# zwyang6/ExCEL

Hardware: AMD Instinct MI355X
Metric: images/sec (CAM+PAR refine, 448x448) (higher is better)
Workload: dtype bf16x3 (fp32 as bf16 hi+lo, fp32 accumulate)

## Files before the change

### excel_amd/_lib.py

```python
import ctypes as C
import os

_HERE = os.path.dirname(os.path.abspath(__file__))
LIB_PATH = os.path.join(_HERE, "csrc", "libexcel_hip.so")

c_f = C.c_void_p
c_i = C.c_int
c_ll = C.c_longlong
c_sz = C.c_size_t


class VitConfig(C.Structure):
    _fields_ = [("width", c_i), ("layers", c_i), ("heads", c_i), ("patch", c_i), ("out_dim", c_i),
                ("n_surgery", c_i), ("pos_grid", c_i)]


class VitBlockWeights(C.Structure):
    _fields_ = [(n, C.c_void_p) for n in (
        "ln1_w", "ln1_b", "in_proj_w", "in_proj_b", "out_proj_w", "out_proj_b",
        "ln2_w", "ln2_b", "fc1_w", "fc1_b", "fc2_w", "fc2_b")]


class VitWeights(C.Structure):
    _fields_ = [(n, C.c_void_p) for n in (
        "conv1_w", "class_emb", "pos_emb", "ln_pre_w", "ln_pre_b", "ln_post_w", "ln_post_b", "proj")] + \
        [("blocks", C.POINTER(VitBlockWeights))]


class DecoderConfig(C.Structure):
    _fields_ = [(n, c_i) for n in ("vit_layers", "vit_width", "embed", "dec_layers", "heads", "num_classes")]


class FuseLayerWeights(C.Structure):
    _fields_ = [(n, C.c_void_p) for n in ("proj_w", "proj_b", "proj2_w", "proj2_b")]


class DecoderBlockWeights(C.Structure):
    _fields_ = VitBlockWeights._fields_


class DecoderWeights(C.Structure):
    _fields_ = [("fuse", C.POINTER(FuseLayerWeights)), ("fuse_w", C.c_void_p), ("fuse_b", C.c_void_p),
                ("blocks", C.POINTER(DecoderBlockWeights)), ("pred_w", C.c_void_p), ("pred_b", C.c_void_p)]


class TextConfig(C.Structure):
    _fields_ = [(n, c_i) for n in ("vocab_size", "context_length", "width", "layers", "heads", "embed_dim")]


class TextWeights(C.Structure):
    _fields_ = [(n, C.c_void_p) for n in ("token_embedding", "positional_embedding", "ln_final_w", "ln_final_b", "text_projection")] + \
        [("blocks", C.POINTER(DecoderBlockWeights))]


class RaggedInfo(C.Structure):
    _fields_ = [("B", C.c_int32), ("total_tiles", C.c_int32), ("total_pix", C.c_int64), ("total_label_pix", C.c_int64),
                ("max_plane_pix", C.c_int64), ("table_ints", C.c_int64)]


class AugParams(C.Structure):
    _fields_ = [("ratio", C.c_double), ("flip", C.c_int32), ("h_pad", C.c_int32), ("w_pad", C.c_int32),
                ("cand_h", C.c_int32 * 10), ("cand_w", C.c_int32 * 10)]


class TrainAugInfo(C.Structure):
    _fields_ = [("B", C.c_int32), ("S", C.c_int32), ("max_h", C.c_int32), ("max_w2", C.c_int32), ("table_ints", C.c_int64),
                ("workspace_bytes", C.c_int64), ("total_label_pix", C.c_int64)]


SIGNATURES = {
    "excel_last_error": (C.c_char_p, []),
    "excel_abi_version": (c_i, []),
    "excel_build_id": (C.c_char_p, []),
    "excel_gemm_f32": (c_i, [c_f, c_f, c_f, c_f, c_f, c_i, c_i, c_i, c_i, c_i, c_i, c_i, c_i, c_i, c_i,
                             c_ll, c_ll, c_ll, c_ll, c_f]),
    "excel_split_bf16": (c_i, [c_f, c_f, c_ll, c_i, c_f]),
    "excel_gemm_bf16x3": (c_i, [c_f, c_f, c_f, c_f, c_f, c_i, c_i, c_i, c_i, c_i, c_f]),
    "excel_split_f16": (c_i, [c_f, c_f, c_ll, c_i, c_f]),
    "excel_gemm_f16x3": (c_i, [c_f, c_f, c_f, c_f, c_f, c_i, c_i, c_i, c_i, c_i, c_f]),
    "excel_pack_f16": (c_i, [c_f, c_f, c_ll, c_i, c_f, c_f]),
    "excel_gemm_f16x2": (c_i, [c_f, c_f, c_f, c_f, c_f, c_f, c_i, c_i, c_i, c_i, c_i, c_f]),
    "excel_gemm_plan": (c_i, [c_i, c_i, c_i, c_i, c_i, c_i, c_i, c_i, c_i, C.POINTER(C.c_int32)]),
    "excel_attn_plan": (c_i, [c_i, c_i, c_i, c_i, c_i, c_i, C.POINTER(C.c_int32)]),
    "excel_layernorm": (c_i, [c_f, c_f, c_f, c_f, c_i, c_i, C.c_float, c_f]),
    "excel_vit_create": (c_i, [C.POINTER(VitConfig), C.POINTER(VitWeights), C.POINTER(C.c_void_p)]),
    "excel_vit_destroy": (None, [C.c_void_p]),
    "excel_vit_workspace_bytes": (c_sz, [C.c_void_p, c_i, c_i]),
    "excel_vit_set_gemm_mode": (c_i, [C.c_void_p, c_i]),
    "excel_vit_get_gemm_mode": (c_i, [C.c_void_p]),
    "excel_vit_weights_fp16_exact": (c_i, [C.c_void_p]),
    "excel_vit_forward": (c_i, [C.c_void_p, c_f, c_i, c_i, c_f, c_sz, c_f, c_f, c_f, c_i, c_f, c_i, c_f, c_f]),
    "excel_vit_forward_ex": (c_i, [C.c_void_p, c_f, c_i, c_i, c_f, c_sz, c_f, c_f, c_f, c_i, c_f, c_i, c_f, c_f, c_i, c_f]),
    "excel_feature_affinity_workspace_bytes": (c_sz, [c_i, c_i, c_i]),
    "excel_feature_affinity": (c_i, [c_f, c_i, c_i, c_i, C.c_float, C.c_float, c_i, c_f, c_f, c_f]),
    "excel_feature_affinity_grouped_workspace_bytes": (c_sz, [c_i, c_i, c_i, c_i]),
    "excel_feature_affinity_grouped": (c_i, [c_f, c_i, c_i, c_i, c_i, c_i, C.c_float, C.c_float, c_i, c_f, c_f, c_f]),
    "excel_attn_select_workspace_bytes": (c_sz, [c_i, c_i]),
    "excel_attn_select_mean": (c_i, [c_f, c_i, c_i, c_i, c_i, c_i, c_f, c_f, c_f, c_f]),
    "excel_decoder_create": (c_i, [C.POINTER(DecoderConfig), C.POINTER(DecoderWeights), C.POINTER(C.c_void_p)]),
    "excel_decoder_destroy": (None, [C.c_void_p]),
    "excel_decoder_workspace_bytes": (c_sz, [C.c_void_p, c_i, c_i]),
    "excel_decoder_forward": (c_i, [C.c_void_p, c_f, c_i, c_i, c_f, c_sz, c_f, c_f, c_f]),
    "excel_text_create": (c_i, [C.POINTER(TextConfig), C.POINTER(TextWeights), C.POINTER(C.c_void_p)]),
    "excel_text_destroy": (None, [C.c_void_p]),
    "excel_text_workspace_bytes": (c_sz, [C.c_void_p, c_i]),
    "excel_text_encode": (c_i, [C.c_void_p, c_f, c_i, c_f, c_f, c_sz, c_f]),
    "excel_prompt_ensemble": (c_i, [c_f, c_i, c_i, c_f, c_f]),
    "excel_decoder_train_workspace_bytes": (c_sz, [C.c_void_p, c_i, c_i]),
    "excel_decoder_forward_train": (c_i, [C.c_void_p, c_f, c_i, c_i, c_f, c_sz, c_f, c_f, C.c_float, C.c_uint, c_f]),
    "excel_decoder_train_attn_fts": (c_i, [C.c_void_p, c_i, c_i, c_f, c_sz, c_f, c_f]),
    "excel_decoder_backward": (c_i, [C.c_void_p, c_f, c_i, c_i, c_f, c_sz, c_f, c_f, C.POINTER(DecoderWeights), C.c_float, C.c_uint, c_f]),
    "excel_adamw_step": (c_i, [c_f, c_f, c_f, c_f, c_ll, C.c_float, C.c_float, C.c_float, C.c_float, C.c_float, c_i, c_f]),
    "excel_train_losses_workspace_bytes": (c_sz, [c_i, c_i, c_i, c_i]),
    "excel_train_losses": (c_i, [c_f, c_f, c_f, c_f, c_i, c_i, c_i, c_i, c_i, c_i, c_i, c_i, C.c_float, C.c_float, c_f, c_f, c_f, c_f, c_f]),
    "excel_lam_to_label": (c_i, [c_f, c_f, c_f, c_i, c_i, c_i, c_i, C.c_float, C.c_float, C.c_float, c_i, c_i, c_f, c_f, c_f]),
    "excel_normalize_img_u8": (c_i, [c_f, c_i, c_i, c_i, C.POINTER(C.c_double), C.POINTER(C.c_double), c_f, c_f]),
    "excel_denormalize_img": (c_i, [c_f, c_i, c_i, c_i, C.POINTER(C.c_float), C.POINTER(C.c_float), c_f, c_f, c_f]),
    "excel_seg_scale_accumulate": (c_i, [c_f, c_f, c_i, c_i, c_i, c_i, c_i, c_i, c_i, c_i, C.c_float, c_f]),
    "excel_cam_workspace_bytes": (c_sz, [c_i, c_i, c_i]),
    "excel_patch_text_cam_workspace_bytes": (c_sz, [c_i, c_i, c_i, c_i]),
    "excel_patch_text_cam": (c_i, [c_f, c_f, c_i, c_i, c_i, c_i, c_i, C.c_float, c_i, c_f, c_f, c_f, c_f, c_f]),
    "excel_clip_feature_surgery": (c_i, [c_f, c_f, c_i, c_i, c_i, c_i, c_i, C.c_float, c_f, c_f, c_f, c_f]),
    "excel_dcrf_workspace_bytes": (c_sz, [c_i, c_i, c_i]),
    "excel_dcrf_inference": (c_i, [c_f, c_f, c_i, c_i, c_i, c_i, c_i, C.c_float, C.c_float, C.c_float, C.c_float, C.c_float, c_f, c_f, c_f]),
    "excel_dcrf_ragged_workspace_bytes": (c_i, [c_ll, c_i, C.POINTER(c_sz)]),
    "excel_dcrf_inference_ragged": (c_i, [c_f, c_f, c_i, c_f, C.POINTER(RaggedInfo), c_i, c_i, C.c_float, C.c_float, C.c_float, C.c_float, C.c_float,
                                          c_f, c_f, c_f, c_f]),
    "excel_dcrf_lam_ragged_workspace_bytes": (c_i, [C.POINTER(C.c_int32), C.POINTER(C.c_int32), c_i, C.POINTER(c_sz)]),
    "excel_dcrf_lam_ragged": (c_i, [c_f, c_f, c_f, C.POINTER(C.c_int32), c_f, c_f, C.POINTER(RaggedInfo), c_i, c_i, c_i, C.c_float, C.c_float,
                                    C.c_float, C.c_float, C.c_float, c_f, c_f, c_f, c_f]),
    "excel_attn_layer_mean": (c_i, [c_f, c_i, c_i, c_i, c_i, c_i, c_f, c_f]),
    "excel_trans_mat_workspace_bytes": (c_sz, [c_i, c_i]),
    "excel_compute_trans_mat": (c_i, [c_f, c_i, c_i, c_f, c_f, c_f]),
    "excel_cls_compact": (c_i, [c_f, c_i, c_i, c_i, c_f, c_f, c_f, c_f]),
    "excel_scoremap_box_mask": (c_i, [c_f, c_f, c_f, c_i, c_i, c_i, c_i, C.c_double, c_f, c_f, c_f]),
    "excel_refine_workspace_bytes": (c_sz, [c_i, c_i, c_i]),
    "excel_refine_cams_with_aff": (c_i, [c_f, c_f, c_f, c_f, c_i, c_i, c_i, c_i, C.c_double, c_f, c_f, c_f]),
    "excel_cam_upsample_bkg": (c_i, [c_f, c_f, c_i, c_i, c_i, c_i, c_i, c_f, c_f, c_i, c_f]),
    "excel_par_workspace_bytes": (c_sz, [c_i, c_i, c_i, c_i, c_i]),
    "excel_par_forward": (c_i, [c_f, c_i, c_i, c_f, c_f, c_i, c_i, c_i, c_i, C.POINTER(C.c_int32), c_i, c_i,
                                C.c_float, C.c_float, c_f, c_f, c_i, c_f]),
    "excel_ragged_plan": (c_i, [C.POINTER(C.c_int32), c_i, C.POINTER(RaggedInfo), C.POINTER(C.c_int32)]),
    "excel_normalize_resize_u8_ragged": (c_i, [c_f, c_f, c_i, c_i, C.POINTER(C.c_double), C.POINTER(C.c_double), c_f, c_f]),
    "excel_normalize_resize_u8_ragged_mirror": (c_i, [c_f, c_f, c_i, c_i, C.POINTER(C.c_double), C.POINTER(C.c_double), c_f, c_f]),
    "excel_cam_upsample_bkg_ragged": (c_i, [c_f, c_f, c_f, C.POINTER(RaggedInfo), c_i, c_i, c_f, c_f, c_i, c_f]),
    "excel_par_ragged_workspace_bytes": (c_sz, [c_ll, c_i]),
    "excel_par_forward_ragged": (c_i, [c_f, c_i, c_i, c_f, c_f, c_f, C.POINTER(RaggedInfo), c_i, C.POINTER(C.c_int32), c_i, c_i,
                                       C.c_float, C.c_float, c_f, c_f, c_f]),
    "excel_argmax_label_ragged": (c_i, [c_f, c_f, c_f, c_f, C.POINTER(RaggedInfo), c_i, c_i, c_f, c_f]),
    "excel_seg_msc_fuse_ragged": (c_i, [C.POINTER(C.c_void_p), C.POINTER(C.c_int32), C.POINTER(C.c_int32), c_i, c_i, c_f, C.POINTER(RaggedInfo),
                                        c_f, c_f, c_f]),
    "excel_seg_resize_argmax_ragged": (c_i, [c_f, c_f, C.POINTER(RaggedInfo), c_f, C.POINTER(RaggedInfo), c_i, c_f, c_f]),
    "excel_seg_resize_argmax_uniform": (c_i, [c_f, c_i, c_i, c_i, c_i, c_f, C.POINTER(RaggedInfo), c_f, c_f]),
    "excel_seg_softmax_resize": (c_i, [c_f, c_i, c_i, c_i, c_i, c_i, c_f, c_f]),
    "excel_seg_softmax_resize_ragged": (c_i, [c_f, c_f, C.POINTER(RaggedInfo), c_f, C.POINTER(RaggedInfo), c_i, c_f, c_f]),
    "excel_cam_overlay_ragged": (c_i, [c_f, c_f, c_i, c_f, c_f, c_f, C.POINTER(RaggedInfo), c_i, c_f, c_f, c_f]),
    "excel_cam_overlay": (c_i, [c_f, c_f, c_i, c_i, c_i, c_i, c_f, c_f, c_f]),
    "excel_train_panels_plan": (c_i, [c_i, c_i, c_i, c_i, c_i, C.POINTER(C.c_int64)]),
    "excel_train_panels": (c_i, [c_f, c_f, c_f, c_f, c_f, c_f, c_f, c_i, c_i, c_i, c_i, c_i, c_i, c_i, C.POINTER(C.c_float), C.POINTER(C.c_float),
                                 c_f, c_f, c_f, c_sz, c_f]),
    "excel_png_labels_bound_bytes": (c_sz, [c_i, c_i]),
    "excel_png_labels_workspace_bytes": (c_sz, [c_i, c_i]),
    "excel_png_encode_labels_ragged": (c_i, [c_f, c_f, C.POINTER(RaggedInfo), C.POINTER(C.c_int32), c_f, c_f, c_sz, c_f, c_f, c_sz, c_f]),
    "excel_train_aug_plan": (c_i, [C.POINTER(C.c_int32), C.POINTER(AugParams), c_i, c_i, C.POINTER(TrainAugInfo), C.POINTER(C.c_int32)]),
    "excel_train_augment_workspace_bytes": (c_sz, [C.POINTER(TrainAugInfo)]),
    "excel_train_augment": (c_i, [c_f, c_f, c_f, C.POINTER(TrainAugInfo), C.POINTER(C.c_double), C.POINTER(C.c_double), c_f, c_f, c_f, c_f, c_f]),
    "excel_train_augment_image": (c_i, [c_f, c_f, C.POINTER(TrainAugInfo), C.POINTER(C.c_double), C.POINTER(C.c_double), c_f, c_f, c_f, c_f]),
    "excel_argmax_label": (c_i, [c_f, c_f, c_f, c_i, c_i, c_i, c_ll, c_f, c_f, c_f]),
    "excel_confusion_accumulate": (c_i, [c_f, c_f, c_ll, c_i, c_f, c_f]),
    "excel_attr_aggregate": (c_i, [c_f, c_f, c_i, c_i, c_i, c_i, C.c_double, c_f, c_f]),
    "excel_bilinear_resize": (c_i, [c_f, c_f, c_ll, c_i, c_i, c_i, c_i, c_i, c_f]),
    "excel_pos_embed_resize": (c_i, [c_f, c_i, c_i, c_i, c_f, c_f]),
    "excel_flip_max_normalize": (c_i, [c_f, c_f, c_i, c_i, c_i, c_f]),
    "excel_lam_scale_accumulate": (c_i, [c_f, c_f, c_i, c_i, c_i, c_i, c_i, c_i, c_f]),
    "excel_plane_minmax_normalize": (c_i, [c_f, c_ll, c_ll, c_f]),
    "excel_prof_enable": (c_i, [c_i]),
    "excel_prof_set_mask": (c_i, [C.c_ulonglong]),
    "excel_prof_set_sampling": (c_i, [c_i]),
    "excel_prof_num_categories": (c_i, []),
    "excel_prof_category_name": (C.c_char_p, [c_i]),
    "excel_prof_collect": (c_i, [C.POINTER(C.c_double), C.POINTER(C.c_longlong), C.POINTER(C.c_double)]),
}

_lib = None


def lib():
    global _lib
    if _lib is not None:
        return _lib
    import torch
    if not os.path.exists(LIB_PATH):
        raise RuntimeError(
            f"excel_amd: {LIB_PATH} is missing - the HIP extension is the only compute path. "
            "Build it with `python -m excel_amd.build` (or __graft_entry__.build()).")
    handle = C.CDLL(LIB_PATH)
    for name, (res, args) in SIGNATURES.items():
        fn = getattr(handle, name)
        fn.restype = res
        fn.argtypes = args
    _lib = handle
    return _lib


def build_id():
    return lib().excel_build_id().decode()


def check(rc, what):
    if rc != 0:
        msg = lib().excel_last_error()
        raise RuntimeError(f"{what} failed (rc={rc}): {msg.decode() if msg else '?'}")
```

### excel_amd/csrc/abi.hip

```cpp
#include "../../include/excel_hip.h"
#include "common.h"
#include "excel_internal.h"

#include <stdarg.h>
#include <map>
#include <vector>

static thread_local char g_err[512] = "";

void excel_set_error(const char* fmt, ...) {
    va_list ap;
    va_start(ap, fmt);
    vsnprintf(g_err, sizeof(g_err), fmt, ap);
    va_end(ap);
}

extern "C" const char* excel_last_error(void) { return g_err; }
extern "C" int excel_abi_version(void) { return 4; }
#ifndef EXCEL_BUILD_ID
#define EXCEL_BUILD_ID "unstamped"
#endif
extern "C" const char* excel_build_id(void) { return EXCEL_BUILD_ID; }

bool g_excel_prof_on = false;
thread_local int g_excel_prof_gemm_cat = -1;
unsigned long long g_excel_prof_mask = ~0ull;
int g_excel_prof_every = 1;
unsigned g_excel_prof_seen[PROF_NCAT];
namespace {
struct ProfRec { int cat; hipEvent_t a, b; };
std::vector<ProfRec> g_prof_recs;
std::vector<hipEvent_t> g_prof_pool;
double g_prof_work[PROF_NCAT];
const char* PROF_NAMES[PROF_NCAT] = {"gemm_nt", "gemm_nn", "gemm_bf16x3", "attn_rowpass", "attn_accum", "layernorm", "embed", "token_norm",
                                     "cam_epilogue", "sinkhorn", "bbox_mask", "matvec", "cam_upsample", "par_affinity",
                                     "par_iterate", "argmax", "confusion", "other", "cam_proj", "cam_fused"};
hipEvent_t prof_event() {
    if (!g_prof_pool.empty()) { hipEvent_t e = g_prof_pool.back(); g_prof_pool.pop_back(); return e; }
    hipEvent_t e; (void)hipEventCreate(&e); return e;
}
}
void excel_prof_begin(int cat, hipStream_t st, double work) {
    ProfRec r{cat, prof_event(), prof_event()};
    (void)hipEventRecord(r.a, st);
    g_prof_recs.push_back(r);
    g_prof_work[cat] += work;
}
void excel_prof_end(int cat, hipStream_t st) {
    for (size_t i = g_prof_recs.size(); i-- > 0;)
        if (g_prof_recs[i].cat == cat) { (void)hipEventRecord(g_prof_recs[i].b, st); return; }
}
extern "C" int excel_prof_enable(int on) {
    g_excel_prof_on = on != 0;
    return EXCEL_OK;
}
extern "C" int excel_prof_set_mask(unsigned long long mask) {
    g_excel_prof_mask = mask;
    return EXCEL_OK;
}
extern "C" int excel_prof_set_sampling(int every) {
    g_excel_prof_every = every > 0 ? every : 1;
    for (int c = 0; c < PROF_NCAT; ++c) g_excel_prof_seen[c] = 0;
    return EXCEL_OK;
}
extern "C" int excel_prof_num_categories(void) { return PROF_NCAT; }
extern "C" const char* excel_prof_category_name(int cat) { return (cat >= 0 && cat < PROF_NCAT) ? PROF_NAMES[cat] : ""; }
extern "C" int excel_prof_collect(double* ms, long long* launches, double* work) {
    for (int c = 0; c < PROF_NCAT; ++c) { ms[c] = 0.0; launches[c] = 0; work[c] = g_prof_work[c]; g_prof_work[c] = 0.0; }
    for (auto& r : g_prof_recs) {
        float t = 0.f;
        if (hipEventSynchronize(r.b) == hipSuccess && hipEventElapsedTime(&t, r.a, r.b) == hipSuccess) {
            ms[r.cat] += t;
            launches[r.cat] += 1;
        }
        g_prof_pool.push_back(r.a);
        g_prof_pool.push_back(r.b);
    }
    g_prof_recs.clear();
    return EXCEL_OK;
}

#define ST(s) ((hipStream_t)(s))
#define TRY(x)                  \
    do {                        \
        int rc__ = (x);         \
        if (rc__) return rc__;  \
    } while (0)

static inline size_t align_up(size_t v, size_t a) { return (v + a - 1) / a * a; }

static GemmArgs gemm_args(const float* A, const float* B, float* C, const float* bias, const float* res, int M, int N, int K,
                          int lda, int ldb, int ldc, int ldr, int act) {
    GemmArgs g;
    memset(&g, 0, sizeof(g));
    g.A = A; g.B = B; g.C = C; g.bias = bias; g.res = res;
    g.M = M; g.N = N; g.K = K; g.Kld = (K + 3) / 4 * 4;
    g.lda = lda; g.ldb = ldb; g.ldc = ldc; g.ldr = ldr;
    g.act = act; g.out_mode = GEMM_OUT_PLAIN; g.alpha = 1.f; g.zdiv = 1;
    return g;
}

static GemmBfArgs gemm_bf_args(const void* A, const unsigned short* W, float* C, void* Cs, const float* bias, const float* res,
                               int M, int N, int K, int ldc, int ldr, int act, int out_mode) {
    GemmBfArgs g;
    memset(&g, 0, sizeof(g));
    g.A = (const unsigned short*)A; g.B = W; g.C = C; g.Cs = (unsigned short*)Cs; g.bias = bias; g.res = res;
    g.M = M; g.N = N; g.K = K; g.lda = 2 * K; g.ldb = 2 * K; g.ldc = ldc; g.ldr = ldr; g.act = act; g.out_mode = out_mode;
    return g;
}

__global__ void transpose_kernel(const float* __restrict__ in, float* __restrict__ out, int R, int Cc) {
    __shared__ float t[32][33];
    const int tx = threadIdx.x & 31, ty = threadIdx.x >> 5;
    const int r0 = blockIdx.y * 32, c0 = blockIdx.x * 32;
    for (int k = ty; k < 32; k += 8)
        if (r0 + k < R && c0 + tx < Cc) t[k][tx] = in[(long long)(r0 + k) * Cc + c0 + tx];
    __syncthreads();
    for (int k = ty; k < 32; k += 8)
        if (c0 + k < Cc && r0 + tx < R) out[(long long)(c0 + k) * R + r0 + tx] = t[tx][k];
}

__global__ void pos_resize_kernel(const float* __restrict__ pos, float* __restrict__ out, int side, int g, int D) {
    const long long i = (long long)blockIdx.x * 256 + threadIdx.x;
    const long long total = (long long)(g * g + 1) * D;
    if (i >= total) return;
    const int d = (int)(i % D);
    const int n = (int)(i / D);
    if (n == 0) { out[i] = pos[d]; return; }
    const int y = (n - 1) / g, x = (n - 1) % g;
    const float sc = (float)side / (float)g;
    float fy = fmaxf(sc * ((float)y + 0.5f) - 0.5f, 0.f), fx = fmaxf(sc * ((float)x + 0.5f) - 0.5f, 0.f);
    const int y0 = min((int)fy, side - 1), x0 = min((int)fx, side - 1);
    const int y1 = min(y0 + 1, side - 1), x1 = min(x0 + 1, side - 1);
    const float ly = fy - (float)y0, lx = fx - (float)x0;
    auto at = [&](int yy, int xx) { return pos[(long long)(1 + yy * side + xx) * D + d]; };
    out[i] = (1.f - ly) * ((1.f - lx) * at(y0, x0) + lx * at(y0, x1)) + ly * ((1.f - lx) * at(y1, x0) + lx * at(y1, x1));
}

__global__ void attn_layer_mean_kernel(const float* __restrict__ attn, int B, int N, int first, int nl, float* __restrict__ out) {
    const long long P = N - 1;
    const long long i = (long long)blockIdx.x * 256 + threadIdx.x;
    if (i >= (long long)B * P * P) return;
    const int c = (int)(i % P), r = (int)((i / P) % P);
    const long long b = i / (P * P);
    float s = 0.f;
    for (int l = 0; l < nl; ++l) s += attn[(((long long)(first + l) * B + b) * N + (r + 1)) * N + (c + 1)];
    out[i] = s / (float)nl;
}

extern "C" int excel_gemm_f32(const float* A, const float* Bm, float* C, const float* bias, const float* residual, int M, int N,
                              int K, int lda, int ldb, int ldc, int ldr, int b_kmajor, int act, int batch, long long sA,
                              long long sB, long long sC, long long sR, void* stream) {
    GemmArgs g = gemm_args(A, Bm, C, bias, residual, M, N, K, lda, ldb, ldc, ldr, act);
    EXCEL_CHECK_ARG((K % 4) == 0 || !b_kmajor, "excel_gemm_f32: K must be a multiple of 4 in NT mode (K=%d)", K);
    if (!b_kmajor) {
        EXCEL_CHECK_ARG((K % 4) == 0, "excel_gemm_f32: K must be a multiple of 4 (pad A with zeros) (K=%d)", K);
    }
    g.sA = sA; g.sB = sB; g.sC = sC; g.sR = sR;
    return excel_launch_gemm(g, b_kmajor != 0, batch, ST(stream));
}

extern "C" int excel_split_bf16(const float* in, void* out, long long rows, int K, void* stream) {
    EXCEL_CHECK_ARG(in && out && rows > 0 && K > 0, "split_bf16: bad argument");
    return excel_launch_split_bf16(in, out, rows, K, ST(stream));
}

extern "C" int excel_gemm_bf16x3(const void* A_split, const void* W_split, float* C, const float* bias, const float* residual,
                                 int M, int N, int K, int act, int split_out, void* stream) {
    EXCEL_CHECK_ARG(A_split && W_split && C, "gemm_bf16x3: null argument");
    GemmBfArgs g = gemm_bf_args(A_split, (const unsigned short*)W_split, C, C, bias, residual, M, N, K, N, N, act,
                                split_out ? GEMM_OUT_SPLIT_BF16 : GEMM_OUT_PLAIN);
// ... 337 lines not shown
    return excel_launch_feature_affinity(feats, B, C, P, beta, gamma, mode, out, workspace, ST(stream));
}

extern "C" size_t excel_feature_affinity_grouped_workspace_bytes(int B, int C, int P, int group) {
    return excel_feature_affinity_grouped_ws_bytes(B, C, P, group);
}

extern "C" int excel_feature_affinity_grouped(const float* feats, int B, int C, int P, int group, int member_stride, float beta, float gamma,
                                              int mode, float* out, void* workspace, void* stream) {
    return excel_launch_feature_affinity_grouped(feats, B, C, P, group, member_stride, beta, gamma, mode, out, workspace, ST(stream));
}

extern "C" size_t excel_attn_select_workspace_bytes(int B, int n_layers) { return excel_attn_select_ws_bytes(B, n_layers); }

extern "C" int excel_attn_select_mean(const float* attn, int Lw, int B, int N, int first_layer, int n_layers, const float* seg_attn,
                                      float* w_out, void* workspace, void* stream) {
    return excel_launch_attn_select_mean(attn, Lw, B, N, first_layer, n_layers, seg_attn, w_out, workspace, ST(stream));
}

#define EXCEL_VIT_FWD_ARGS excel_vit_t h, const float* img, int B, int S, void* workspace, size_t workspace_bytes, float* image_features, \
    float* x_raw, float* w_aff, int aff_layers, float* attn_out, int n_attn_out, float* feats_out, const float* ex_attn, int flags, void* stream
static int vit_forward_bf16(EXCEL_VIT_FWD_ARGS) {
#include "vit_forward_body.inc"
}
static int vit_forward_f16(EXCEL_VIT_FWD_ARGS) {
    using excel_f16::excel_launch_gemm; using excel_f16::excel_launch_gemm_bf16x3; using excel_f16::excel_launch_split_bf16;
    using excel_f16::excel_launch_vt_from_planes; using excel_f16::excel_launch_layernorm; using excel_f16::excel_launch_assemble_ln_pre;
    using excel_f16::excel_launch_token_axis_normalize; using excel_f16::excel_launch_im2col; using excel_f16::excel_launch_attn_rowpass;
    using excel_f16::excel_launch_attn_accum; using excel_f16::excel_launch_attn_strip;
#include "vit_forward_body.inc"
}
static int vit_forward_impl(EXCEL_VIT_FWD_ARGS) {
    EXCEL_CHECK_ARG(h, "excel_vit_forward: null handle");
    return h->gemm_mode >= 2 ? vit_forward_f16(h, img, B, S, workspace, workspace_bytes, image_features, x_raw, w_aff, aff_layers, attn_out,
                                               n_attn_out, feats_out, ex_attn, flags, stream)
                             : vit_forward_bf16(h, img, B, S, workspace, workspace_bytes, image_features, x_raw, w_aff, aff_layers, attn_out,
                                                n_attn_out, feats_out, ex_attn, flags, stream);
}

extern "C" size_t excel_cam_workspace_bytes(int B, int N, int T) {
    return align_up((size_t)B * N * ((T + 3) / 4 * 4) * sizeof(float), 256);
}

extern "C" int excel_clip_feature_surgery(const float* image_features, const float* text, int B, int N, int C, int T, int F,
                                          float temperature, float* out_full, float* out_slice, void* workspace, void* stream) {
    EXCEL_CHECK_ARG(image_features && text && workspace && (out_full || out_slice), "clip_feature_surgery: null argument");
    EXCEL_CHECK_ARG((C % 4) == 0, "clip_feature_surgery: C must be a multiple of 4");
    const int ldT = (T + 3) / 4 * 4;
    float* S = (float*)workspace;
    GemmArgs ga = gemm_args(image_features, text, S, nullptr, nullptr, B * N, T, C, C, C, ldT, 0, GEMM_ACT_NONE);
    TRY(excel_launch_gemm(ga, true, 1, ST(stream)));
    return excel_launch_cam_epilogue(S, out_full, out_slice, B, N, T, ldT, F, temperature, ST(stream));
}

struct PtcWs { float *sim, *part, *colsq; unsigned short* ts; size_t total; };
static PtcWs ptc_ws_layout(int B, int N, int C, int T, char* base) {
    PtcWs w;
    size_t off = 0;
    auto take = [&](size_t bytes) { char* p = base + off; off += align_up(bytes, 256); return p; };
    w.sim = (float*)take(excel_patch_text_cam_ws_floats(B, N, C, T, 0) * sizeof(float));
    w.ts = (unsigned short*)take((size_t)T * C * sizeof(float));
    w.part = (float*)take(excel_patch_text_cam_ws_floats(B, N, C, T, 1) * sizeof(float));
    w.colsq = (float*)take(excel_patch_text_cam_ws_floats(B, N, C, T, 2) * sizeof(float));
    w.total = off;
    return w;
}
extern "C" size_t excel_patch_text_cam_workspace_bytes(int B, int N, int C, int T) { return ptc_ws_layout(B, N, C, T, nullptr).total; }

extern "C" int excel_patch_text_cam(const float* x_raw, const float* text, int B, int N, int C, int T, int F, float temperature, int mode,
                                    float* out_full, float* out_slice, float* image_features, void* workspace, void* stream) {
    EXCEL_CHECK_ARG(x_raw && text && workspace && (out_full || out_slice), "patch_text_cam: null argument");
    EXCEL_CHECK_ARG(mode == 0 || mode == 1 || mode == 2, "patch_text_cam: mode must be 0 (exact fp32), 1 (bf16x3) or 2 (f16x3)");
    EXCEL_CHECK_ARG(B > 0 && N > 0 && C > 0 && T > 0, "patch_text_cam: bad shape");
    const int ldT = (T + 3) / 4 * 4;
    const PtcWs w = ptc_ws_layout(B, N, C, T, (char*)workspace);
    if (mode == 2)
        return excel_f16::excel_launch_patch_text_cam(x_raw, text, w.ts, w.sim, w.part, w.colsq, out_full, out_slice, image_features, B, N, C, T, F,
                                                      ldT, temperature, 1, ST(stream));
    return excel_launch_patch_text_cam(x_raw, text, mode == 1 ? w.ts : nullptr, w.sim, w.part, w.colsq, out_full, out_slice, image_features, B, N, C,
                                       T, F, ldT, temperature, mode, ST(stream));
}

extern "C" int excel_attn_layer_mean(const float* attn, int Lw, int B, int N, int first_layer, int n_layers, float* w_aff, void* stream) {
    EXCEL_CHECK_ARG(attn && w_aff && first_layer >= 0 && n_layers >= 1 && first_layer + n_layers <= Lw, "attn_layer_mean: bad layer range");
    const long long n = (long long)B * (N - 1) * (N - 1);
    hipLaunchKernelGGL(attn_layer_mean_kernel, dim3((unsigned)cdivl(n, 256)), dim3(256), 0, ST(stream), attn, B, N, first_layer, n_layers, w_aff);
    EXCEL_CHECK_LAUNCH("attn_layer_mean");
    return EXCEL_OK;
}

extern "C" size_t excel_trans_mat_workspace_bytes(int B, int P) {
    return 2 * align_up((size_t)B * P * P * sizeof(float), 256) + align_up((size_t)B * P * sizeof(float), 256);
}

extern "C" int excel_compute_trans_mat(const float* w_aff, int B, int P, float* trans_out, void* workspace, void* stream) {
    EXCEL_CHECK_ARG(w_aff && trans_out && workspace, "compute_trans_mat: null argument");
    EXCEL_CHECK_ARG((P % 4) == 0, "compute_trans_mat: P must be a multiple of 4 (P=%d)", P);
    char* base = (char*)workspace;
    const size_t mat = align_up((size_t)B * P * P * sizeof(float), 256);
    float* T = (float*)base;
    float* Tsym = (float*)(base + mat);
    float* cs = (float*)(base + 2 * mat);
    TRY(excel_launch_trans_mat_sym(w_aff, T, Tsym, cs, B, P, ST(stream)));
    GemmArgs ga = gemm_args(Tsym, Tsym, trans_out, nullptr, nullptr, P, P, P, P, P, P, 0, GEMM_ACT_NONE);
    ga.sA = ga.sB = ga.sC = (long long)P * P;
    return excel_launch_gemm(ga, true, B, ST(stream));
}

extern "C" int excel_cls_compact(const float* onehot, int B, int F, int Smax, int32_t* cls_idx, int32_t* ncls, int32_t* nchan,
                                 void* stream) {
    EXCEL_CHECK_ARG(onehot && cls_idx && ncls && Smax >= 1, "cls_compact: bad argument");
    return excel_launch_cls_compact(onehot, B, F, Smax, cls_idx, ncls, nchan, ST(stream));
}

extern "C" int excel_scoremap_box_mask(const float* attr, const int32_t* cls_idx, const int32_t* ncls, int B, int g, int F, int Smax,
                                       double caa_thre, float* v_out, uint8_t* mask_out, void* stream) {
    EXCEL_CHECK_ARG(attr && cls_idx && ncls && v_out, "scoremap_box_mask: null argument");
    return excel_launch_bbox_mask(attr, cls_idx, ncls, B, g, F, Smax, caa_thre, v_out, mask_out, ST(stream));
}

extern "C" size_t excel_refine_workspace_bytes(int B, int P, int Smax) {
    return 2 * align_up((size_t)B * P * P * sizeof(float), 256) + align_up((size_t)B * P * sizeof(float), 256) +
           2 * align_up((size_t)B * Smax * P * sizeof(float), 256);
}

extern "C" int excel_refine_cams_with_aff(const float* attr, const float* w_aff, const int32_t* cls_idx, const int32_t* ncls, int B,
                                          int g, int F, int Smax, double caa_thre, float* refined, void* workspace, void* stream) {
    EXCEL_CHECK_ARG(attr && w_aff && cls_idx && ncls && refined && workspace, "refine_cams_with_aff: null argument");
    const int P = g * g;
    char* base = (char*)workspace;
    const size_t mat = align_up((size_t)B * P * P * sizeof(float), 256);
    const size_t vec = align_up((size_t)B * Smax * P * sizeof(float), 256);
    float* T = (float*)base;
    float* Tsym = (float*)(base + mat);
    float* cs = (float*)(base + 2 * mat);
    float* v = (float*)(base + 2 * mat + align_up((size_t)B * P * sizeof(float), 256));
    float* u = (float*)((char*)v + vec);
    hipStream_t st = ST(stream);
    TRY(excel_launch_trans_mat_sym(w_aff, T, Tsym, cs, B, P, st));
    TRY(excel_launch_bbox_mask(attr, cls_idx, ncls, B, g, F, Smax, caa_thre, v, nullptr, st));
    TRY(excel_launch_matvec(Tsym, v, ncls, u, B, P, Smax, st));
    TRY(excel_launch_matvec(Tsym, u, ncls, refined, B, P, Smax, st));
    return EXCEL_OK;
}

extern "C" int excel_cam_upsample_bkg(const float* refined, const int32_t* ncls, int B, int g, int Smax, int H, int W, float* cams,
                                      void* workspace, int flags, void* stream) {
    EXCEL_CHECK_ARG(refined && ncls && cams && workspace, "cam_upsample_bkg: null argument");
    return excel_launch_cam_upsample_bkg(refined, ncls, (float*)workspace, cams, B, g, Smax, H, W, (flags & EXCEL_CAMS_ZERO_UNUSED) ? 1 : 0, ST(stream));
}

extern "C" int excel_ragged_plan(const int32_t* hw, int B, excel_ragged_info* info, int32_t* table) {
    EXCEL_CHECK_ARG(hw && info && B >= 1, "ragged_plan: bad argument");
    long long pix = 0, lab = 0, tiles = 0, max_plane = 0;
    for (int b = 0; b < B; ++b) {
        const long long H = hw[2 * b], W = hw[2 * b + 1];
        EXCEL_CHECK_ARG(H >= 1 && W >= 1, "ragged_plan: image %d has size %lld x %lld", b, H, W);
        const long long Wp = (W + 3) / 4 * 4, plane = H * Wp, nt = ((W + 63) / 64) * ((H + 15) / 16);
        if (table) {
            int32_t* rec = table + EXCEL_RAG_REC * b;
            rec[0] = (int32_t)H; rec[1] = (int32_t)W; rec[2] = (int32_t)pix; rec[3] = (int32_t)tiles; rec[4] = (int32_t)lab; rec[5] = rec[6] = rec[7] = 0;
            for (long long t = 0; t < nt; ++t) table[EXCEL_RAG_REC * (B + 1) + tiles + t] = b;
        }
        pix += plane; lab += H * W; tiles += nt;
        if (plane > max_plane) max_plane = plane;
        EXCEL_CHECK_ARG(pix < (1LL << 31) && 3 * lab < (1LL << 31) && tiles < (1LL << 31), "ragged_plan: batch too large for 32-bit offsets");
    }
    if (table) {
        int32_t* rec = table + EXCEL_RAG_REC * B;
        rec[0] = rec[1] = 0; rec[2] = (int32_t)pix; rec[3] = (int32_t)tiles; rec[4] = (int32_t)lab; rec[5] = rec[6] = rec[7] = 0;
    }
    info->B = B; info->total_tiles = (int32_t)tiles; info->total_pix = pix; info->total_label_pix = lab; info->max_plane_pix = max_plane;
    info->table_ints = EXCEL_RAG_REC * (long long)(B + 1) + tiles;
    return EXCEL_OK;
}

static TileGeo ragged_geo(const int32_t* table, int B) {
    TileGeo g;
    g.tab = table; g.B = B; g.H = g.W = 0;
    return g;
}
static TileGeo uniform_geo(int B, int H, int W) {
    TileGeo g;
    g.tab = nullptr; g.B = B; g.H = H; g.W = W;
    return g;
}

extern "C" int excel_normalize_resize_u8_ragged(const uint8_t* hwc, const int32_t* table, int B, int S, const double* mean3, const double* std3,
                                                float* out, void* stream) {
    EXCEL_CHECK_ARG(hwc && table && out && mean3 && std3 && B > 0 && S > 0, "normalize_resize_u8_ragged: bad argument");
    return excel_launch_normalize_resize_u8_ragged(hwc, out, ragged_geo(table, B), S, mean3, std3, ST(stream));
}

extern "C" int excel_normalize_resize_u8_ragged_mirror(const uint8_t* hwc, const int32_t* table, int B, int S, const double* mean3,
                                                       const double* std3, float* out, void* stream) {
    EXCEL_CHECK_ARG(hwc && table && out && mean3 && std3 && B > 0 && S > 0, "normalize_resize_u8_ragged_mirror: bad argument");
    return excel_launch_normalize_resize_u8_ragged_mirror(hwc, out, ragged_geo(table, B), S, mean3, std3, ST(stream));
}

extern "C" int excel_cam_upsample_bkg_ragged(const float* refined, const int32_t* ncls, const int32_t* table, const excel_ragged_info* info, int g,
                                             int Smax, float* cams, void* workspace, int flags, void* stream) {
    EXCEL_CHECK_ARG(refined && ncls && table && info && cams && workspace, "cam_upsample_bkg_ragged: null argument");
    EXCEL_CHECK_ARG((((uintptr_t)cams) & 15) == 0, "cam_upsample_bkg_ragged: cams must be 16-byte aligned");
    return excel_launch_cam_upsample_bkg_ragged(refined, ncls, (float*)workspace, cams, g, Smax, ragged_geo(table, info->B), info->total_tiles,
                                                (flags & EXCEL_CAMS_ZERO_UNUSED) ? 1 : 0, ST(stream));
}

int excel_aug_plan(const int32_t* hw, const excel_aug_params* prm, int B, int S, excel_train_aug_info* info, int32_t* table);
int excel_launch_train_augment(const unsigned char* hwc, const unsigned char* labels, const int* table, const excel_train_aug_info& info,
                               const double* mean, const double* stdv, float* img, unsigned char* label, int* img_box, void* workspace,
                               hipStream_t st);
int excel_launch_train_augment_image(const unsigned char* hwc, const int* table, const excel_train_aug_info& info, const double* mean,
                                     const double* stdv, float* img, int* img_box, void* workspace, hipStream_t st);
extern "C" int excel_train_aug_plan(const int32_t* hw, const excel_aug_params* params, int B, int S, excel_train_aug_info* info, int32_t* table) {
    return excel_aug_plan(hw, params, B, S, info, table);
}

extern "C" size_t excel_train_augment_workspace_bytes(const excel_train_aug_info* info) {
    return info ? (size_t)info->workspace_bytes : 0;
}

extern "C" int excel_train_augment(const uint8_t* hwc, const uint8_t* labels, const int32_t* table, const excel_train_aug_info* info,
                                   const double* mean3, const double* std3, float* img, uint8_t* label, int32_t* img_box, void* workspace,
                                   void* stream) {
    EXCEL_CHECK_ARG(hwc && labels && table && info && mean3 && std3 && img && label && img_box && workspace, "train_augment: null argument");
    EXCEL_CHECK_ARG(info->B >= 1 && info->S >= 1 && info->max_h >= 1 && info->max_w2 >= 1 && info->workspace_bytes > 0,
                    "train_augment: info was not filled by excel_train_aug_plan");
    return excel_launch_train_augment(hwc, labels, table, *info, mean3, std3, img, label, img_box, workspace, ST(stream));
}

extern "C" int excel_train_augment_image(const uint8_t* hwc, const int32_t* table, const excel_train_aug_info* info, const double* mean3,
                                         const double* std3, float* img, int32_t* img_box, void* workspace, void* stream) {
    EXCEL_CHECK_ARG(hwc && table && info && mean3 && std3 && img && img_box && workspace, "train_augment_image: null argument");
    EXCEL_CHECK_ARG(info->B >= 1 && info->S >= 1 && info->max_h >= 1 && info->max_w2 >= 1 && info->workspace_bytes > 0,
                    "train_augment_image: info was not filled by excel_train_aug_plan");
    return excel_launch_train_augment_image(hwc, table, *info, mean3, std3, img, img_box, workspace, ST(stream));
}

extern "C" size_t excel_par_workspace_bytes(int B, int Cmax, int H, int W, int ndil) {
    const size_t hw = (size_t)H * W;
    return align_up((size_t)B * 8 * ndil * hw * sizeof(float), 256) + align_up((size_t)B * Cmax * hw * sizeof(float), 256) +
           align_up((size_t)B * 3 * hw * sizeof(float), 256);
}

template <class Step>
static int par_jacobi(const float* masks, float* out, float* pp, int n_iter, Step step) {
    const float* cur = masks;
    for (int it = 0; it < n_iter; ++it) {
        float* dst = (((n_iter - 1 - it) & 1) == 0) ? out : pp;
        TRY(step(cur, dst));
        cur = dst;
    }
    return EXCEL_OK;
}

extern "C" int excel_par_forward(const float* imgs, int h, int w, const float* masks, const int32_t* nchan, int B, int Cmax, int H,
                                 int W, const int32_t* dilations, int ndil, int n_iter, float w1, float w2, float* out,
                                 void* workspace, int flags, void* stream) {
    EXCEL_CHECK_ARG(imgs && masks && out && workspace && dilations, "par_forward: null argument");
    EXCEL_CHECK_ARG(n_iter >= 0 && ndil >= 1 && ndil <= 8, "par_forward: bad n_iter/ndil");
    EXCEL_CHECK_ARG(B > 0 && Cmax > 0 && H > 0 && W > 0 && h > 0 && w > 0, "par_forward: bad shape");
    const size_t hw = (size_t)H * W;
    char* base = (char*)workspace;
    float* aff = (float*)base;
    float* pp = (float*)(base + align_up((size_t)B * 8 * ndil * hw * sizeof(float), 256));
    float* guide = (float*)((char*)pp + align_up((size_t)B * Cmax * hw * sizeof(float), 256));
    hipStream_t st = ST(stream);
    const float* gimg = imgs;
    if (h != H || w != W) {
        TRY(excel_launch_bilinear_ac(imgs, guide, B * 3, h, w, H, W, st));
        gimg = guide;
    }
    const TileGeo geo = uniform_geo(B, H, W);
    const bool recompute = !(flags & EXCEL_PAR_STREAM_AFFINITIES) && n_iter > 0 && (W % 4) == 0 && (((uintptr_t)pp & 15) == 0) &&
                           excel_par_guide_supported(gimg, aff, masks, out, Cmax, (long long)hw, W, dilations, ndil);
    TRY(excel_launch_par_affinity(gimg, aff, geo, 0, dilations, ndil, w1, w2, st, recompute ? 1 : 0));
    if (n_iter == 0) {
        hipMemcpyAsync(out, masks, sizeof(float) * (size_t)B * Cmax * hw, hipMemcpyDeviceToDevice, st);
        return EXCEL_OK;
    }
    if (recompute)
        return par_jacobi(masks, out, pp, n_iter, [&](const float* cur, float* dst) {
            return excel_launch_par_iterate_guide(gimg, aff, cur, dst, nchan, Cmax, geo, 0, dilations, ndil, w1, w2, st);
        });
    return par_jacobi(masks, out, pp, n_iter, [&](const float* cur, float* dst) {
        return excel_launch_par_iterate(aff, cur, dst, nchan, B, Cmax, H, W, dilations, ndil, st);
    });
}

extern "C" size_t excel_par_ragged_workspace_bytes(long long total_pix, int Cmax) {
    return align_up((size_t)5 * total_pix * sizeof(float), 256) + align_up((size_t)Cmax * total_pix * sizeof(float), 256) +
           align_up((size_t)3 * total_pix * sizeof(float), 256);
}

extern "C" int excel_par_forward_ragged(const float* imgs, int h, int w, const float* masks, const int32_t* nchan, const int32_t* table,
                                        const excel_ragged_info* info, int Cmax, const int32_t* dilations, int ndil, int n_iter, float w1,
                                        float w2, float* out, void* workspace, void* stream) {
    EXCEL_CHECK_ARG(imgs && masks && out && workspace && dilations && table && info, "par_forward_ragged: null argument");
    EXCEL_CHECK_ARG(n_iter >= 1 && Cmax > 0 && h > 0 && w > 0 && info->B > 0, "par_forward_ragged: bad n_iter / shape");
    const size_t tp = (size_t)info->total_pix;
    char* base = (char*)workspace;
    float* stats = (float*)base;
    float* pp = (float*)(base + align_up(5 * tp * sizeof(float), 256));
    float* guide = (float*)((char*)pp + align_up((size_t)Cmax * tp * sizeof(float), 256));
    hipStream_t st = ST(stream);
    const TileGeo geo = ragged_geo(table, info->B);
    EXCEL_CHECK_ARG(excel_par_guide_supported(guide, stats, masks, out, Cmax, info->max_plane_pix, 4, dilations, ndil) && (((uintptr_t)pp & 15) == 0),
                    "par_forward_ragged: needs dilations [1,2,4,8,12,24], 16-byte aligned buffers and max(Cmax,5) * H * Wp * 4 < 2^31 per image "
                    "(Wp = W rounded up to 4)");
    TRY(excel_launch_bilinear_ac_ragged(imgs, guide, h, w, geo, info->total_tiles, st));
    TRY(excel_launch_par_affinity(guide, stats, geo, info->total_tiles, dilations, ndil, w1, w2, st, 1));
    return par_jacobi(masks, out, pp, n_iter, [&](const float* cur, float* dst) {
        return excel_launch_par_iterate_guide(guide, stats, cur, dst, nchan, Cmax, geo, info->total_tiles, dilations, ndil, w1, w2, st);
    });
}

extern "C" int excel_argmax_label_ragged(const float* cams, const int32_t* nchan, const int32_t* cls_idx, const int32_t* table,
                                         const excel_ragged_info* info, int Smax, int Cmax, uint8_t* labels_u8, void* stream) {
    EXCEL_CHECK_ARG(cams && table && info && labels_u8, "argmax_label_ragged: null argument");
    return excel_launch_argmax_label_ragged(cams, nchan, cls_idx, Smax, Cmax, ragged_geo(table, info->B), info->total_tiles, labels_u8, ST(stream));
}

extern "C" int excel_argmax_label(const float* cams, const int32_t* nchan, const int32_t* cls_idx, int B, int Smax, int Cmax,
                                  long long HW, uint8_t* labels_u8, int64_t* labels_i64, void* stream) {
    EXCEL_CHECK_ARG(cams && (labels_u8 || labels_i64), "argmax_label: null argument");
    return excel_launch_argmax_label(cams, nchan, cls_idx, B, Smax, Cmax, HW, labels_u8, (long long*)labels_i64, ST(stream));
}

extern "C" int excel_confusion_accumulate(const uint8_t* gt, const uint8_t* pred, long long n, int num_classes, int64_t* hist,
                                          void* stream) {
    EXCEL_CHECK_ARG(gt && pred && hist && n >= 0, "confusion_accumulate: null argument");
    if (n == 0) return EXCEL_OK;
    return excel_launch_confusion(gt, pred, n, num_classes, (unsigned long long*)hist, ST(stream));
}

extern "C" int excel_attr_aggregate(const float* text, const float* bank, int F, int T, int C, int K, double topK, float* out,
                                    void* stream) {
    EXCEL_CHECK_ARG(text && bank && out, "attr_aggregate: null argument");
    const int drop = (int)((1.0 - topK) * (double)K);
    return excel_launch_attr_aggregate(text, bank, F, T, C, K, drop, out, ST(stream));
}

extern "C" int excel_bilinear_resize(const float* in, float* out, long long planes, int h, int w, int H, int W, int align_corners,
                                     void* stream) {
    EXCEL_CHECK_ARG(in && out && planes > 0 && h > 0 && w > 0 && H > 0 && W > 0, "bilinear_resize: bad argument");
    return excel_launch_bilinear_resize(in, out, planes, h, w, H, W, align_corners, ST(stream));
}

extern "C" int excel_pos_embed_resize(const float* pos, int side, int g, int D, float* out, void* stream) {
    EXCEL_CHECK_ARG(pos && out && side > 0 && g > 0, "pos_embed_resize: bad argument");
    hipLaunchKernelGGL(pos_resize_kernel, dim3((unsigned)cdivl((long long)(g * g + 1) * D, 256)), dim3(256), 0, ST(stream), pos, out, side, g, D);
    EXCEL_CHECK_LAUNCH("pos_resize");
    return EXCEL_OK;
}

extern "C" int excel_flip_max_normalize(const float* attr, float* out, int B, int g, int F, void* stream) {
    EXCEL_CHECK_ARG(attr && out, "flip_max_normalize: null argument");
    return excel_launch_flip_max_normalize(attr, out, B, g, F, ST(stream));
}

extern "C" int excel_lam_scale_accumulate(const float* maps, float* acc, int B, int g, int F, int H, int W, int init, void* stream) {
    EXCEL_CHECK_ARG(maps && acc && B > 0 && g > 0, "lam_scale_accumulate: bad argument");
    return excel_launch_lam_scale_accumulate(maps, acc, B, g, F, H, W, init, ST(stream));
}

extern "C" int excel_plane_minmax_normalize(float* lam, long long planes, long long HW, void* stream) {
    EXCEL_CHECK_ARG(lam && planes > 0 && HW > 0, "plane_minmax_normalize: bad argument");
    return excel_launch_plane_minmax_normalize(lam, planes, HW, ST(stream));
}
```

### excel_amd/csrc/common.h

```cpp
#pragma once
#include <hip/hip_runtime.h>
#include <stdint.h>
#include <stdio.h>
#include <string.h>

#define EXCEL_OK 0
#define EXCEL_ERR_ARG (-1)
#define EXCEL_ERR_LAUNCH (-2)
#define EXCEL_ERR_ALLOC (-3)

void excel_set_error(const char* fmt, ...);

#define EXCEL_CHECK_ARG(cond, ...)                         \
    do {                                                   \
        if (!(cond)) {                                     \
            excel_set_error(__VA_ARGS__);                  \
            return EXCEL_ERR_ARG;                          \
        }                                                  \
    } while (0)

#define EXCEL_CHECK_LAUNCH(name)                                                   \
    do {                                                                           \
        hipError_t e__ = hipGetLastError();                                        \
        if (e__ != hipSuccess) {                                                   \
            excel_set_error("%s: launch failed: %s", name, hipGetErrorString(e__)); \
            return EXCEL_ERR_LAUNCH;                                               \
        }                                                                          \
    } while (0)

typedef float f32x4 __attribute__((ext_vector_type(4)));
typedef float f32x16 __attribute__((ext_vector_type(16)));

static inline int cdiv(int a, int b) { return (a + b - 1) / b; }
static inline long long cdivl(long long a, long long b) { return (a + b - 1) / b; }

#define WAVE 64

#ifdef EXCEL_DEV
#define EXCEL_DBG(x) (x)
#else
#define EXCEL_DBG(x) 0
#endif

__device__ __forceinline__ void wave_halves(float x, float& lo, float& hi) {
    const unsigned u = __float_as_uint(x);
    const auto r = __builtin_amdgcn_permlane32_swap(u, u, false, false);
    lo = __uint_as_float(r[0]);
    hi = __uint_as_float(r[1]);
}
__device__ __forceinline__ float wave_sum(float v) {
    float lo, hi;
    wave_halves(v, lo, hi);
    v = lo + hi;
#pragma unroll
    for (int o = 16; o > 0; o >>= 1) v += __shfl_xor(v, o, 64);
    return v;
}
__device__ __forceinline__ float wave_max(float v) {
    float lo, hi;
    wave_halves(v, lo, hi);
    v = fmaxf(lo, hi);
#pragma unroll
    for (int o = 16; o > 0; o >>= 1) v = fmaxf(v, __shfl_xor(v, o, 64));
    return v;
}
__device__ __forceinline__ float wave_min(float v) {
    float lo, hi;
    wave_halves(v, lo, hi);
    v = fminf(lo, hi);
#pragma unroll
    for (int o = 16; o > 0; o >>= 1) v = fminf(v, __shfl_xor(v, o, 64));
    return v;
}

__device__ __forceinline__ int c32_row(int reg, int lane) { return (reg & 3) + 8 * (reg >> 2) + 4 * (lane >> 5); }

__device__ __forceinline__ int xcd_remap(int id, int n) {
    const int q = n >> 3, r = n & 7;
    const int xcd = id & 7, loc = id >> 3;
    const int base = (xcd < r) ? xcd * (q + 1) : r * (q + 1) + (xcd - r) * q;
    return base + loc;
}

#define EXCEL_RAG_REC 8
struct TileGeo {
    const int* tab;
    int B;
    int H, W;
};
struct Tile {
    int b, x0, y0, H, W, Wp;
    long long base;
    long long HW;
    long long lab;
};
__device__ __forceinline__ Tile tile_of_ragged(const TileGeo& g, int tile) {
    Tile t;
    const int* __restrict__ tab = g.tab;
    t.b = tab[EXCEL_RAG_REC * (g.B + 1) + tile];
    const int* rec = tab + EXCEL_RAG_REC * t.b;
    t.H = rec[0]; t.W = rec[1];
    t.Wp = (t.W + 3) & ~3;
    t.base = rec[2];
    t.lab = rec[4];
    const int loc = tile - rec[3];
    const int ntx = (t.W + 63) >> 6;
    const int ty = loc / ntx;
    t.x0 = (loc - ty * ntx) * 64;
    t.y0 = ty * 16;
    t.HW = (long long)t.H * t.Wp;
    return t;
}
template <bool RAGGED>
__device__ __forceinline__ Tile tile_of(const TileGeo& g) {
    Tile t;
    if (RAGGED) {
        t = tile_of_ragged(g, blockIdx.x);
    } else {
        t.b = blockIdx.z; t.x0 = blockIdx.x * 64; t.y0 = blockIdx.y * 16;
        t.H = g.H; t.W = g.W; t.Wp = g.W;
        t.HW = (long long)g.H * g.W;
        t.base = (long long)t.b * t.HW;
        t.lab = t.base;
    }
    return t;
}
__device__ __forceinline__ int ragged_image_of_pixel(const int* __restrict__ tab, int B, long long n) {
    int lo = 0, hi = B - 1;
    while (lo < hi) {
        const int mid = (lo + hi + 1) >> 1;
        if ((long long)tab[EXCEL_RAG_REC * mid + 4] <= n) lo = mid; else hi = mid - 1;
    }
    return lo;
}

enum ExcelProfCat {
    PROF_GEMM_NT = 0, PROF_GEMM_NN, PROF_GEMM_BF16X3, PROF_ATTN_ROWPASS, PROF_ATTN_ACCUM, PROF_LAYERNORM, PROF_EMBED, PROF_TOKEN_NORM,
    PROF_CAM_EPILOGUE, PROF_SINKHORN, PROF_BBOX, PROF_MATVEC, PROF_UPSAMPLE, PROF_PAR_AFFINITY, PROF_PAR_ITERATE,
    PROF_ARGMAX, PROF_CONFUSION, PROF_OTHER, PROF_CAM_PROJ, PROF_CAM_FUSED, PROF_NCAT
};
extern thread_local int g_excel_prof_gemm_cat;
extern bool g_excel_prof_on;
extern unsigned long long g_excel_prof_mask;
extern int g_excel_prof_every;
extern unsigned g_excel_prof_seen[];
void excel_prof_begin(int cat, hipStream_t st, double work);
void excel_prof_end(int cat, hipStream_t st);
struct ProfScope {
    int cat; hipStream_t st; bool on;
    ProfScope(int c, hipStream_t s, double work = 0.0)
        : cat(c), st(s), on(g_excel_prof_on && ((g_excel_prof_mask >> c) & 1) && (g_excel_prof_seen[c]++ % g_excel_prof_every) == 0) { if (on) excel_prof_begin(cat, st, work); }
    ~ProfScope() { if (on) excel_prof_end(cat, st); }
};


#ifdef EXCEL_SPLIT_F16
typedef _Float16 split_t;
#define EXCEL_MFMA16(a, b, c, x, y, z) __builtin_amdgcn_mfma_f32_32x32x16_f16(a, b, c, x, y, z)
#define EXCEL_MFMA32(a, b, c) __builtin_amdgcn_mfma_f32_16x16x32_f16(a, b, c, 0, 0, 0)
#define EXCEL_SPLIT_NAME "f16"
#else
typedef __bf16 split_t;
#define EXCEL_MFMA16(a, b, c, x, y, z) __builtin_amdgcn_mfma_f32_32x32x16_bf16(a, b, c, x, y, z)
#define EXCEL_MFMA32(a, b, c) __builtin_amdgcn_mfma_f32_16x16x32_bf16(a, b, c, 0, 0, 0)
#define EXCEL_SPLIT_NAME "bf16"
#endif
typedef split_t splitx8 __attribute__((ext_vector_type(8)));
typedef split_t splitx4 __attribute__((ext_vector_type(4)));
__device__ __forceinline__ split_t split_hi(float x) { return (split_t)x; }
__device__ __forceinline__ void split_pair(float a, float b, unsigned& hi2, unsigned& lo2) {
#ifdef EXCEL_SPLIT_F16
    typedef float f2_ __attribute__((ext_vector_type(2)));
    typedef _Float16 h2_ __attribute__((ext_vector_type(2)));
    const f2_ v = {a, b};
    const h2_ h = __builtin_convertvector(v, h2_);
    hi2 = __builtin_bit_cast(unsigned, h);
    lo2 = __builtin_bit_cast(unsigned, __builtin_convertvector(v - __builtin_convertvector(h, f2_), h2_));
#else
    typedef float f2_ __attribute__((ext_vector_type(2)));
    typedef __bf16 b2_ __attribute__((ext_vector_type(2)));
    const f2_ v = {a, b};
    hi2 = __builtin_bit_cast(unsigned, __builtin_convertvector(v, b2_));
    const f2_ back = {__uint_as_float(hi2 << 16), __uint_as_float(hi2 & 0xffff0000u)};
    lo2 = __builtin_bit_cast(unsigned, __builtin_convertvector(v - back, b2_));
#endif
}
__device__ __forceinline__ void split_pair_bounded(float a, float b, unsigned& hi2, unsigned& lo2) {
#ifdef EXCEL_SPLIT_F16
    typedef _Float16 h2_ __attribute__((ext_vector_type(2)));
    const float ha = __uint_as_float(__float_as_uint(a) & 0xFFFFE000u), hb = __uint_as_float(__float_as_uint(b) & 0xFFFFE000u);
    hi2 = __builtin_bit_cast(unsigned, __builtin_amdgcn_cvt_pkrtz(ha, hb));
    const h2_ l = {(_Float16)(a - ha), (_Float16)(b - hb)};
    lo2 = __builtin_bit_cast(unsigned, l);
#else
    typedef float f2_ __attribute__((ext_vector_type(2)));
    typedef __bf16 b2_ __attribute__((ext_vector_type(2)));
    const unsigned ua = __float_as_uint(a), ub = __float_as_uint(b);
    hi2 = (ua >> 16) | (ub & 0xFFFF0000u);
    const f2_ d = {a - __uint_as_float(ua & 0xFFFF0000u), b - __uint_as_float(ub & 0xFFFF0000u)};
    lo2 = __builtin_bit_cast(unsigned, __builtin_convertvector(d, b2_));
#endif
}
typedef float f32x2 __attribute__((ext_vector_type(2)));
template <int NV>
__device__ __forceinline__ void quickgelu_tiles(f32x4* v) {
    f32x2 t[2 * NV];
#pragma unroll
    for (int i = 0; i < 2 * NV; ++i) t[i] = f32x2{v[i >> 1][2 * (i & 1)], v[i >> 1][2 * (i & 1) + 1]} * f32x2{-1.702f, -1.702f};
#pragma unroll
    for (int i = 0; i < 2 * NV; ++i) t[i] = t[i] * f32x2{1.4426950408889634f, 1.4426950408889634f};
#pragma unroll
    for (int i = 0; i < 2 * NV; ++i) t[i] = f32x2{__builtin_amdgcn_exp2f(t[i][0]), __builtin_amdgcn_exp2f(t[i][1])};
#pragma unroll
    for (int i = 0; i < 2 * NV; ++i) t[i] = t[i] + f32x2{1.f, 1.f};
#pragma unroll
    for (int i = 0; i < 2 * NV; ++i) t[i] = f32x2{__builtin_amdgcn_rcpf(t[i][0]), __builtin_amdgcn_rcpf(t[i][1])};
#pragma unroll
    for (int i = 0; i < 2 * NV; ++i) {
        const f32x2 o = f32x2{v[i >> 1][2 * (i & 1)], v[i >> 1][2 * (i & 1) + 1]} * t[i];
        v[i >> 1][2 * (i & 1)] = o[0];
        v[i >> 1][2 * (i & 1) + 1] = o[1];
    }
}
__device__ __forceinline__ unsigned lds_addr(const void* p) { return (unsigned)(unsigned long long)(const __attribute__((address_space(3))) void*)p; }
__device__ __forceinline__ splitx8 lds_read16(unsigned addr) {
    f32x4 v;
    asm volatile("ds_read_b128 %0, %1" : "=v"(v) : "v"(addr) : "memory");
    return __builtin_bit_cast(splitx8, v);
}
__device__ __forceinline__ float2 lds_read8(unsigned addr) {
    float2 v;
    asm volatile("ds_read_b64 %0, %1" : "=v"(v) : "v"(addr) : "memory");
    return v;
}
__device__ __forceinline__ void lds_write8(unsigned addr, float2 v) { asm volatile("ds_write_b64 %0, %1" ::"v"(addr), "v"(v) : "memory"); }
__device__ __forceinline__ splitx4 lds_read8h(unsigned addr) {
    f32x2 v;
    asm volatile("ds_read_b64 %0, %1" : "=v"(v) : "v"(addr) : "memory");
    return __builtin_bit_cast(splitx4, v);
}
template <int OFF>
__device__ __forceinline__ splitx4 lds_read8h_tr(unsigned addr) {
    static_assert(OFF >= 0 && OFF < 65536, "ds_read_b64_tr_b16 immediate offset");
    f32x2 v;
    asm volatile("ds_read_b64_tr_b16 %0, %1 offset:%2" : "=v"(v) : "v"(addr), "n"(OFF) : "memory");
    return __builtin_bit_cast(splitx4, v);
}
__device__ __forceinline__ void lds_wait8(splitx8 (&a)[4], splitx8 (&b)[4]) {
    asm volatile("s_waitcnt lgkmcnt(0)" : "+v"(a[0]), "+v"(a[1]), "+v"(a[2]), "+v"(a[3]), "+v"(b[0]), "+v"(b[1]), "+v"(b[2]), "+v"(b[3])::"memory");
}


__host__ __device__ __forceinline__ long long split_off(int k, int plane) { return (long long)(k >> 5) * 64 + plane * 32 + (k & 31); }
```

### excel_amd/csrc/excel_internal.h

```cpp
#pragma once
#include <hip/hip_runtime.h>

enum { GEMM_ACT_NONE = 0, GEMM_ACT_QUICKGELU = 1, GEMM_ACT_RELU = 2 };
enum { GEMM_OUT_PLAIN = 0, GEMM_OUT_QKV_HEADMAJOR = 1, GEMM_OUT_SPLIT_BF16 = 2 };

struct GemmArgs {
    const float* A;
    const float* B;
    float* C;
    const float* bias;
    const float* res;
    int M, N, K;
    int Kld;
    int lda, ldb, ldc, ldr;
    long long sA, sB, sC, sR, sBias;
    int zdiv;
    long long sA2, sB2, sC2;
    int act;
    int out_mode;
    int tokN, heads, hd;
    float alpha;
};


struct GemmBfArgs {
    const unsigned short* A;
    const unsigned short* B;
    float* C;
    unsigned short* Cs;
    const float* bias;
    const float* res;
    int M, N, K;
    int lda, ldb, ldc, ldr;
    int act, out_mode;
    int tokN, heads, hd;
    unsigned short* qkv_split;
    int dbg;
    int batch;
    long long sA, sB, sC, sCs;
    int mix_tall, mix_short;
    int mix_first;
    int w_lo_zero;
    const unsigned short* Bh;
    int ldbh;
};

struct GemmShape {
    int M, N, K, lda, ldb, ldc, ldr, hd, out_mode, has_residual, batch;
    int f16;
    int w_lo_zero;
    int half_ok;
};
enum { GEMM_8WAVE = 0, GEMM_8WAVE_MIXED = 1, GEMM_W4 = 2, GEMM_W4_MIX = 3 };
struct GemmPlan {
    int kernel;
    int tile;
    int nt_m;
    int x2;
    int tall, shrt, second;
    int grid_x, grid_y, block;
};
constexpr int GEMM_W4_BN = 256;
GemmPlan gemm_plan(const GemmShape& s, int n_cu);
enum { ATTN_STRIP = 0, ATTN_TWOPASS_SPLIT = 1, ATTN_TWOPASS_F32 = 2 };
constexpr int ATTN_STRIP_MAX_TILES = 40;
struct AttnPlan {
    int path;
    int ntiles;
    int ntw, nw, nw_full;
    int rp_ntypes;
    int rp_grid[3];
    int grid[3], block;
    int split_c;
};
AttnPlan attn_plan(int B, int H, int N, int gemm_mode, int surgery, int want_w);
inline bool gemm_half_ok(bool aligned, int N, int K, int ldbh) {
    return aligned && ldbh >= K && (ldbh & 7) == 0 && (long long)N * ldbh * 2 < 0x7fffffffLL;
}


int excel_launch_trans_mat_sym(const float* W, float* T, float* Tsym, float* cs, int B, int P, hipStream_t st);
int excel_launch_cls_compact(const float* onehot, int B, int F, int Smax, int* cls_idx, int* ncls, int* nchan, hipStream_t st);
int excel_launch_bbox_mask(const float* attr, const int* cls_idx, const int* ncls, int B, int g, int F, int Smax, double thre,
                           float* v_out, unsigned char* mask_out, hipStream_t st);
int excel_launch_matvec(const float* T, const float* v, const int* ncls, float* u, int B, int P, int Smax, hipStream_t st);
int excel_launch_cam_upsample_bkg(const float* r, const int* ncls, float* rn, float* cams, int B, int g, int Smax, int H, int W,
                                  int zero_unused, hipStream_t st);
struct TileGeo;
int excel_launch_par_affinity(const float* img, float* aff, const TileGeo& geo, int total_tiles, const int* dil, int ndil, float w1, float w2,
                              hipStream_t st, int compact = 0);
int excel_par_guide_supported(const void* guide, const void* stats, const void* in, const void* out, int Cmax, long long max_plane, int Wp,
                              const int* dil, int ndil);
int excel_launch_par_iterate_guide(const float* guide, const float* stats, const float* in, float* out, const int* nchan, int Cmax,
                                   const TileGeo& geo, int total_tiles, const int* dil, int ndil, float w1, float w2, hipStream_t st);
int excel_launch_par_iterate(const float* aff, const float* in, float* out, const int* nchan, int B, int Cmax, int H, int W,
                             const int* dil, int ndil, hipStream_t st);
int excel_launch_bilinear_ac_ragged(const float* in, float* out, int h, int w, const TileGeo& geo, int total_tiles, hipStream_t st);
int excel_launch_argmax_label_ragged(const float* cams, const int* nchan, const int* cls_idx, int Smax, int Cmax, const TileGeo& geo,
                                     int total_tiles, unsigned char* lab8, hipStream_t st);
int excel_launch_cam_upsample_bkg_ragged(const float* r, const int* ncls, float* rn, float* cams, int g, int Smax, const TileGeo& geo,
                                         int total_tiles, int zero_unused, hipStream_t st);
int excel_launch_normalize_resize_u8_ragged(const unsigned char* hwc, float* out, const TileGeo& geo, int S, const double* mean, const double* stdv,
                                            hipStream_t st);
int excel_launch_normalize_resize_u8_ragged_mirror(const unsigned char* hwc, float* out, const TileGeo& geo, int S, const double* mean,
                                                   const double* stdv, hipStream_t st);
int excel_launch_bilinear_ac(const float* in, float* out, int planes, int h, int w, int H, int W, hipStream_t st);
int excel_launch_argmax_label(const float* cams, const int* nchan, const int* cls_idx, int B, int Smax, int Cmax, long long HW,
                              unsigned char* lab8, long long* lab64, hipStream_t st);
int excel_launch_confusion(const unsigned char* gt, const unsigned char* pred, long long n, int nc, unsigned long long* hist,
                           hipStream_t st);
int excel_launch_attr_aggregate(const float* text, const float* bank, int F, int T, int C, int K, int drop, float* out,
                                hipStream_t st);
int excel_launch_bilinear_resize(const float* in, float* out, long long planes, int h, int w, int H, int W, int align_corners,
                                 hipStream_t st);
int excel_launch_flip_max_normalize(const float* attr, float* out, int B, int g, int F, hipStream_t st);
int excel_launch_lam_scale_accumulate(const float* maps, float* acc, int B, int g, int F, int H, int W, int init, hipStream_t st);
int excel_launch_plane_minmax_normalize(float* lam, long long planes, long long HW, hipStream_t st);
int excel_launch_seg_scale_accumulate(const float* segs, float* acc, int B, int nc, int h, int w, int H, int W, int flip_mean, int init,
                                      float scale, hipStream_t st);
int excel_launch_denormalize(const float* img, unsigned char* out8, float* outf, int B, long long HW, const float* mean, const float* stdv,
                             hipStream_t st);
int excel_launch_normalize_u8(const unsigned char* hwc, float* out, int B, long long HW, const double* mean, const double* stdv, hipStream_t st);
int excel_launch_lam_to_label(const float* cam, const float* cls, const int* box, int B, int F, int H, int W, float bkg, float high, float low,
                              int ignore_mid, int ignore, float* valid, unsigned char* lab, hipStream_t st);
size_t excel_train_losses_ws_bytes(int B, int nc, int H, int W);
int excel_launch_train_losses(const float* seg, const float* attn_pred, const unsigned char* pseudo, const unsigned char* aff_labels, int B, int nc,
                              int g_h, int g_w, int H, int W, int radius, int ignore, float w_seg, float w_diver, float* losses, float* d_seg,
                              float* d_attn_pred, void* ws, hipStream_t st);
size_t excel_feature_affinity_ws_bytes(int B, int C, int P);
int excel_launch_feature_affinity(const float* feats, int B, int C, int P, float beta, float gamma, int mode, float* out, void* ws,
                                  hipStream_t st);
size_t excel_feature_affinity_grouped_ws_bytes(int B, int C, int P, int group);
int excel_launch_feature_affinity_grouped(const float* feats, int B, int C, int P, int group, int member_stride, float beta, float gamma,
                                          int mode, float* out, void* ws, hipStream_t st);
size_t excel_attn_select_ws_bytes(int B, int n_layers);
int excel_launch_attn_select_mean(const float* attn, int Lw, int B, int N, int first_layer, int n_layers, const float* seg_attn,
                                  float* out, void* ws, hipStream_t st);

namespace excel_bf16 {
#include "excel_split_api.inc"
}
namespace excel_f16 {
#include "excel_split_api.inc"
}
#ifdef EXCEL_SPLIT_F16
#define EXCEL_SPLIT_NS excel_f16
#else
#define EXCEL_SPLIT_NS excel_bf16
#endif
using namespace excel_bf16;

struct BilinearTap { int y0, y1, x0, x1; float ly, lx; };
__device__ __forceinline__ BilinearTap bilinear_tap(int x, int y, int h, int w, int H, int W, int align_corners) {
    float fy, fx;
    if (align_corners) {
        fy = ((H > 1) ? (float)(h - 1) / (float)(H - 1) : 0.f) * (float)y;
        fx = ((W > 1) ? (float)(w - 1) / (float)(W - 1) : 0.f) * (float)x;
    } else {
        fy = fmaxf(__fsub_rn(__fmul_rn((float)h / (float)H, (float)y + 0.5f), 0.5f), 0.f);
        fx = fmaxf(__fsub_rn(__fmul_rn((float)w / (float)W, (float)x + 0.5f), 0.5f), 0.f);
    }
    BilinearTap t;
    t.y0 = min((int)fy, h - 1); t.x0 = min((int)fx, w - 1);
    t.y1 = min(t.y0 + 1, h - 1); t.x1 = min(t.x0 + 1, w - 1);
    t.ly = fy - (float)t.y0; t.lx = fx - (float)t.x0;
    return t;
}
__device__ __forceinline__ float bilinear_blend(const BilinearTap& t, float p00, float p01, float p10, float p11) {
    const float top = fmaf(t.lx, p01, __fmul_rn(1.f - t.lx, p00));
    const float bot = fmaf(t.lx, p11, __fmul_rn(1.f - t.lx, p10));
    return fmaf(t.ly, bot, __fmul_rn(1.f - t.ly, top));
}
```

### excel_amd/csrc/par.hip

```cpp
#include <stdlib.h>
#include <type_traits>
#include <utility>
#include "common.h"
#include "excel_internal.h"

struct ParDil {
    int d[8];
    float pos_sm[64];
};

#define PAR_LOG2E_3 0.48089834696298783f
#ifndef PAR_MASK_DEPTH
#define PAR_MASK_DEPTH 1
#endif

template <int ND, bool RAGGED>
__global__ __launch_bounds__(256) void par_affinity_kernel(const float* __restrict__ img, float* __restrict__ aff, ParDil dl, TileGeo geo,
                                                           float w1, int COMPACT) {
    constexpr int NT = 8 * ND;
    int b, H, W, Wp, x, y;
    long long base, HW;
    const int wave = __builtin_amdgcn_readfirstlane((int)(threadIdx.x >> 6));
    if (RAGGED) {
        const Tile t = tile_of<true>(geo);
        b = t.b; H = t.H; W = t.W; Wp = t.Wp; base = t.base; HW = t.HW;
        x = t.x0 + (threadIdx.x & 63);
        y = t.y0 + blockIdx.y * 4 + wave;
    } else {
        b = blockIdx.z; H = geo.H; W = geo.W; Wp = geo.W; HW = (long long)H * W; base = (long long)b * HW;
        x = blockIdx.x * 64 + (threadIdx.x & 63);
        y = blockIdx.y * 4 + wave;
    }
    if (y >= H) return;
    const bool in_x = x < W;
    const int xc = min(x, W - 1);
    int xo[ND][2];
#pragma unroll
    for (int di = 0; di < ND; ++di) { xo[di][0] = max(xc - dl.d[di], 0); xo[di][1] = min(xc + dl.d[di], W - 1); }
    float acc[NT];
#pragma unroll
    for (int t = 0; t < NT; ++t) acc[t] = 0.f;
    const long long pix = (long long)y * Wp + x;
    float* st = aff + 5 * base + pix;
#pragma unroll 1
    for (int c = 0; c < 3; ++c) {
        const float* ch = img + 3 * base + c * HW;
        const float* row0 = ch + (long long)y * Wp;
        const float ctr = row0[xc];
        float nb[NT];
        float sum = 0.f;
#pragma unroll
        for (int di = 0; di < ND; ++di) {
            const int d = dl.d[di];
            const float* rup = ch + (long long)max(y - d, 0) * Wp;
            const float* rdn = ch + (long long)min(y + d, H - 1) * Wp;
            nb[di * 8 + 0] = rup[xo[di][0]]; nb[di * 8 + 1] = rup[xc]; nb[di * 8 + 2] = rup[xo[di][1]];
            nb[di * 8 + 3] = row0[xo[di][0]]; nb[di * 8 + 4] = row0[xo[di][1]];
            nb[di * 8 + 5] = rdn[xo[di][0]]; nb[di * 8 + 6] = rdn[xc]; nb[di * 8 + 7] = rdn[xo[di][1]];
#pragma unroll
            for (int k = 0; k < 8; ++k) sum += nb[di * 8 + k];
        }
        const float mean = sum / (float)NT;
        float var = 0.f;
#pragma unroll
        for (int t = 0; t < NT; ++t) { const float dv = nb[t] - mean; var = fmaf(dv, dv, var); }
        const float den = sqrtf(var / (float)(NT - 1)) + 1e-8f;
        const float k = 1.f / (den * w1);
        const float k2 = __fmul_rn(k * k, PAR_LOG2E_3);
        if (COMPACT && in_x) st[c * HW] = k2;
#pragma unroll
        for (int t = 0; t < NT; ++t) {
            const float dv = nb[t] - ctr;
            acc[t] = fmaf(-(dv * dv), k2, acc[t]);
        }
    }
    float m = -INFINITY;
#pragma unroll
    for (int t = 0; t < NT; ++t) m = fmaxf(m, acc[t]);
    float s = 0.f;
#pragma unroll
    for (int t = 0; t < NT; ++t) { acc[t] = __builtin_amdgcn_exp2f(__fsub_rn(acc[t], m)); s += acc[t]; }
    const float inv_s = 1.f / s;
    if (!in_x) return;
    if (COMPACT) {
        st[3 * HW] = m;
        st[4 * HW] = inv_s;
        return;
    }
    float* out = aff + (long long)NT * base + pix;
#pragma unroll
    for (int t = 0; t < NT; ++t) out[(long long)t * HW] = fmaf(acc[t], inv_s, dl.pos_sm[t]);
}

#define PAR_CCH 8
__global__ __launch_bounds__(256) void par_iterate_stream_kernel(const float* __restrict__ aff, const float* __restrict__ in,
                                                                 float* __restrict__ out, const int* __restrict__ nchan, ParDil dl,
                                                                 int ndil, int Cmax, int H, int W) {
    const int b = blockIdx.z;
    const int x = blockIdx.x * 64 + (threadIdx.x & 63);
    const int y = blockIdx.y * 4 + (threadIdx.x >> 6);
    if (x >= W || y >= H) return;
    const int nch = nchan ? min(nchan[b], Cmax) : Cmax;
    const long long HW = (long long)H * W;
    const float* a = aff + (long long)b * 8 * ndil * HW + (long long)y * W + x;
    const float* ib = in + (long long)b * Cmax * HW;
    float* ob = out + (long long)b * Cmax * HW + (long long)y * W + x;
    const int dils[8] = {dl.d[0], dl.d[1], dl.d[2], dl.d[3], dl.d[4], dl.d[5], dl.d[6], dl.d[7]};
    for (int c0 = 0; c0 < nch; c0 += PAR_CCH) {
        float acc[PAR_CCH];
#pragma unroll
        for (int c = 0; c < PAR_CCH; ++c) acc[c] = 0.f;
#pragma unroll 1
        for (int di = 0; di < ndil; ++di) {
            int d = dils[0];
#pragma unroll
            for (int q = 1; q < 8; ++q) d = (di == q) ? dils[q] : d;
#pragma unroll
            for (int k = 0; k < 8; ++k) {
                const int dy = (k < 3) ? -1 : (k < 5 ? 0 : 1);
                const int dx = (k == 0 || k == 3 || k == 5) ? -1 : ((k == 1 || k == 6) ? 0 : 1);
                const int yy = min(max(y + dy * d, 0), H - 1);
                const int xx = min(max(x + dx * d, 0), W - 1);
                const float wgt = a[(long long)(di * 8 + k) * HW];
                const float* src = ib + (long long)yy * W + xx;
#pragma unroll
                for (int c = 0; c < PAR_CCH; ++c)
                    if (c0 + c < nch) acc[c] = fmaf(src[(long long)(c0 + c) * HW], wgt, acc[c]);
            }
        }
#pragma unroll
        for (int c = 0; c < PAR_CCH; ++c)
            if (c0 + c < nch) ob[(long long)(c0 + c) * HW] = acc[c];
    }
}

#define PG_TP 128
template <int DI> struct ParD { static constexpr int v = DI == 0 ? 1 : DI == 1 ? 2 : DI == 2 ? 4 : DI == 3 ? 8 : DI == 4 ? 12 : 24; };
template <class F, int... I> __device__ __forceinline__ void static_for_seq(F&& f, std::integer_sequence<int, I...>) { (f(std::integral_constant<int, I>{}), ...); }
template <int N, class F> __device__ __forceinline__ void static_for(F&& f) { static_for_seq(f, std::make_integer_sequence<int, N>{}); }
template <int OFF> __device__ __forceinline__ f32x2 lds_read8_imm(unsigned base) {
    static_assert(OFF >= 0 && OFF < 65536 && (OFF & 7) == 0, "ds_read_b64 immediate offset");
    f32x2 v;
    asm volatile("ds_read_b64 %0, %1 offset:%2" : "=v"(v) : "v"(base), "n"(OFF) : "memory");
    return v;
}

template <bool RAGGED>
__global__ __launch_bounds__(512, 4) void par_iterate_guide_kernel(const float* __restrict__ guide, const float* __restrict__ stats,
                                                                    const float* __restrict__ in, float* __restrict__ out,
                                                                    const int* __restrict__ nchan, ParDil dl, int Cmax, TileGeo geo, int dbg) {
    constexpr int ND = 6, HALO = 24, TR = 16 + 2 * HALO, TP = PG_TP, NG = 3 * ND;
    __shared__ __attribute__((aligned(1024))) float tile[2 * TR * TP];
    Tile tg;
    if (RAGGED) {
        tg = tile_of_ragged(geo, (EXCEL_DBG(dbg) & 32) ? (int)blockIdx.x : xcd_remap(blockIdx.x, gridDim.x));
    } else {
        tg = tile_of<false>(geo);
        if (!(EXCEL_DBG(dbg) & 32)) {
            const int nx = gridDim.x, ny = gridDim.y, per = nx * ny;
            const int id = xcd_remap(blockIdx.x + nx * (blockIdx.y + ny * blockIdx.z), per * (int)gridDim.z);
            const int bb = id / per, rem = id - bb * per, tyy = rem / nx;
            tg.b = bb; tg.x0 = (rem - tyy * nx) * 64; tg.y0 = tyy * 16; tg.base = (long long)bb * tg.HW; tg.lab = tg.base;
        }
    }
    const int b = tg.b, x0 = tg.x0, y0 = tg.y0, H = tg.H, W = tg.W, Wp = tg.Wp;
    const long long HW = tg.HW;
    const int tid = threadIdx.x, lane = tid & 63, tx = tid & 31, ty = tid >> 5;
    const int wave = __builtin_amdgcn_readfirstlane(tid >> 6);
    const int px = x0 + 2 * tx, py = y0 + ty;
    const int nch = nchan ? min(nchan[b], Cmax) : Cmax;
    const long long pix = (long long)min(py, H - 1) * Wp + min(px, Wp - 2);
    const float* st_b = stats + 5 * tg.base + pix;

    typedef __attribute__((address_space(3))) unsigned char* lds_bptr;
    const __amdgpu_buffer_rsrc_t rs_g = __builtin_amdgcn_make_buffer_rsrc((void*)(guide + 3 * tg.base), 0, (int)(3 * HW * 4), 0x00020000);
    const __amdgpu_buffer_rsrc_t rs_m = __builtin_amdgcn_make_buffer_rsrc((void*)(in + (long long)Cmax * tg.base), 0, (int)((long long)Cmax * HW * 4), 0x00020000);
    const int xoffA = min(max(x0 - HALO + lane, 0), W - 1) * 4, xoffB = min(max(x0 - HALO + 64 + lane, 0), W - 1) * 4;
    const unsigned tile_b = lds_addr(tile);
    constexpr int RPW = TR / 8;
#ifdef PAR_ALL_INTERIOR
    const bool interior = true;
#else
    const bool interior = x0 - HALO >= 0 && x0 + 64 + HALO <= W;
#endif
    const int x4off = min(x0 - HALO + 4 * (lane & 31), Wp - 4) * 4;
    auto stage = [&](int p, int buf) {
        const bool is_g = p < 3;
        const int plane_off = (is_g ? p : p - 3) * (int)(HW * 4);
        unsigned dst = tile_b + (buf * TR + wave * RPW) * (TP * 4);
        asm volatile("" : "+s"(dst));
        if ((EXCEL_DBG(dbg) & 8) && (wave == 0 || wave == 7)) return;
        if (interior) {
            int half = lane >> 5;
            asm volatile("" : "+v"(half));
#pragma unroll
            for (int j = 0; j < RPW / 2; ++j) {
                const int gy = min(max(y0 - HALO + wave * RPW + 2 * j + half, 0), H - 1);
                const int voff = gy * Wp * 4 + x4off;
                if (is_g) __builtin_amdgcn_raw_ptr_buffer_load_lds(rs_g, (lds_bptr)(unsigned long long)(dst + j * (2 * TP * 4)), 16, voff, plane_off, 0, 0);
                else __builtin_amdgcn_raw_ptr_buffer_load_lds(rs_m, (lds_bptr)(unsigned long long)(dst + j * (2 * TP * 4)), 16, voff, plane_off, 0, 0);
            }
            return;
        }
#pragma unroll 4
        for (int rr = 0; rr < RPW; ++rr) {
            const int gy = min(max(y0 - HALO + wave * RPW + rr, 0), H - 1);
            const int soff = plane_off + gy * Wp * 4;
            if (is_g) {
                __builtin_amdgcn_raw_ptr_buffer_load_lds(rs_g, (lds_bptr)(unsigned long long)(dst + rr * (TP * 4)), 4, xoffA, soff, 0, 0);
                __builtin_amdgcn_raw_ptr_buffer_load_lds(rs_g, (lds_bptr)(unsigned long long)(dst + rr * (TP * 4) + 256), 4, xoffB, soff, 0, 0);
            } else {
                __builtin_amdgcn_raw_ptr_buffer_load_lds(rs_m, (lds_bptr)(unsigned long long)(dst + rr * (TP * 4)), 4, xoffA, soff, 0, 0);
                __builtin_amdgcn_raw_ptr_buffer_load_lds(rs_m, (lds_bptr)(unsigned long long)(dst + rr * (TP * 4) + 256), 4, xoffB, soff, 0, 0);
            }
        }
    };

    f32x2 wall[ND][8];
#pragma unroll
    for (int di = 0; di < ND; ++di)
#pragma unroll
        for (int k = 0; k < 8; ++k) wall[di][k] = f32x2{0.f, 0.f};

    const unsigned org = tile_b + (ty * TP + 2 * tx) * 4;
    auto taps = [&](auto depth_c, int buf, auto&& fn, auto&& pin) {
        constexpr int DEPTH = decltype(depth_c)::value, NS = DEPTH + 1;
        unsigned base = org + buf * (TR * TP * 4);
        asm volatile("" : "+v"(base));
        f32x2 sl[NS][3];
        auto nreads = [](int G) constexpr { return (G % 3 != 1 || G / 3 == 0) ? 3 : 2; };
        auto issue = [&](auto g) {
            constexpr int G = decltype(g)::value, r = G % 3, d = ParD<G / 3>::v, s = G % NS;
            constexpr int row = (HALO + (r - 1) * d) * TP * 4, cl = (d == 1) ? HALO - 2 : HALO - d, cr = (d == 1) ? HALO + 2 : HALO + d;
            sl[s][0] = lds_read8_imm<row + cl * 4>(base);
            if constexpr (r != 1 || d == 1) sl[s][1] = lds_read8_imm<row + HALO * 4>(base);
            sl[s][2] = lds_read8_imm<row + cr * 4>(base);
        };
        static_for<DEPTH>([&](auto g) { issue(g); });
        static_for<NG>([&](auto g) {
            constexpr int G = decltype(g)::value, di = G / 3, r = G % 3, d = ParD<di>::v, s = G % NS;
            constexpr bool mid = (r != 1 || d == 1);
            if constexpr (G + DEPTH < NG) issue(std::integral_constant<int, G + DEPTH>{});
            constexpr int last = (G + DEPTH < NG) ? G + DEPTH : NG - 1;
            constexpr int nxt = [&]() constexpr { int n = 0; for (int q = G + 1; q <= last; ++q) n += nreads(q); return n; }();
            static_assert(nxt <= 15, "lgkmcnt is a 4-bit counter");
            if constexpr (mid) asm volatile("s_waitcnt lgkmcnt(%3)" : "+v"(sl[s][0]), "+v"(sl[s][1]), "+v"(sl[s][2]) : "n"(nxt) : "memory");
            else asm volatile("s_waitcnt lgkmcnt(%2)" : "+v"(sl[s][0]), "+v"(sl[s][2]) : "n"(nxt) : "memory");
            constexpr int k0 = (r == 0) ? 0 : (r == 1 ? 3 : 5);
            const f32x2 L = sl[s][0], R = sl[s][2];
            if constexpr (d == 1) {
                const f32x2 M = sl[s][1];
                fn(di, k0, f32x2{L[1], M[0]});
                if constexpr (r != 1) fn(di, k0 + 1, M);
                fn(di, k0 + (r != 1 ? 2 : 1), f32x2{M[1], R[0]});
            } else {
                fn(di, k0, L);
                if constexpr (r != 1) fn(di, k0 + 1, sl[s][1]);
                fn(di, k0 + (r != 1 ? 2 : 1), R);
            }
            pin();
            __builtin_amdgcn_sched_barrier(0);
        });
    };

    auto far_taps = [&](const float* plane) -> f32x2 {
        f32x2 sum = {0.f, 0.f};
        const int yu = max(py - 24, 0), yd = min(py + 24, H - 1), ym = min(py, H - 1);
        const int xl = max(min(px, Wp - 2) - 24, 0), xr = min(min(px, Wp - 2) + 24, Wp - 2), xm = min(px, Wp - 2);
        const int ys[8] = {yu, yu, yu, ym, ym, yd, yd, yd}, xs[8] = {xl, xm, xr, xl, xr, xl, xm, xr};
#pragma unroll
        for (int k = 0; k < 8; ++k) {
            const float2 v = *reinterpret_cast<const float2*>(plane + (long long)ys[k] * Wp + (xs[k] & ~1));
            sum += f32x2{v.x, v.y};
        }
        return sum;
    };
    const int np = 3 + nch;
    auto stat_load = [&](int plane) -> f32x2 { return *reinterpret_cast<const f32x2*>(st_b + (long long)plane * HW); };
    f32x2 st_nxt = stat_load(0), st_nx2 = f32x2{0.f, 0.f};
    __builtin_amdgcn_sched_barrier(0);
    stage(0, 0);
#pragma unroll 1
    for (int p = 0; p < 3; ++p) {
        asm volatile("s_waitcnt vmcnt(0)" : "+v"(st_nxt) :: "memory");
        __builtin_amdgcn_s_barrier();
        const f32x2 nk2 = -st_nxt;
        st_nxt = stat_load(p + 1);
        if (p == 2) st_nx2 = stat_load(4);
        f32x2 ctr;
        asm volatile("ds_read_b64 %0, %1 offset:%2" : "=v"(ctr) : "v"(org + (p & 1) * (TR * TP * 4)), "n"((HALO * TP + HALO) * 4) : "memory");
        __builtin_amdgcn_sched_barrier(0);
        stage(p + 1, (p + 1) & 1);
        asm volatile("s_waitcnt lgkmcnt(0)" : "+v"(ctr) :: "memory");
        if (EXCEL_DBG(dbg) & 1) continue;
        f32x2 nctr = -ctr;
        if (EXCEL_DBG(dbg) & 16) nctr += 1e-30f * far_taps(guide + 3 * tg.base + (long long)p * HW);
        asm volatile("" : "+v"(nctr));
        taps(std::integral_constant<int, 1>{}, p & 1, [&](int di, int k, const f32x2 nb) {
            const f32x2 dv = nb + nctr;
            wall[di][k] = __builtin_elementwise_fma(dv * dv, nk2, wall[di][k]);
        }, [] {});
    }
    if (!(EXCEL_DBG(dbg) & 2)) {
        f32x2 nm2 = -st_nxt;
        asm volatile("" : "+v"(nm2));
        const f32x2 is2 = st_nx2;
#pragma unroll
        for (int di = 0; di < ND; ++di)
#pragma unroll
            for (int k = 0; k < 8; ++k) {
                const f32x2 z = wall[di][k] + nm2;
                const f32x2 e = {__builtin_amdgcn_exp2f(z[0]), __builtin_amdgcn_exp2f(z[1])};
                const float ps = dl.pos_sm[di * 8 + k];
                wall[di][k] = __builtin_elementwise_fma(e, is2, f32x2{ps, ps});
            }
    }
    const bool valid = px < W && py < H;
    float* out_px = out + (long long)Cmax * tg.base + (long long)py * Wp + px;
#ifndef PAR_STORE_WAIT
#define PAR_STORE_WAIT 1
#endif
    const bool wstore = PAR_STORE_WAIT && __builtin_amdgcn_ballot_w64(valid) != 0 && !EXCEL_DBG(dbg);
    for (int p = 3; p < np; ++p) {
        if (p > 3 && wstore) asm volatile("s_waitcnt vmcnt(1)" ::: "memory");
        else asm volatile("s_waitcnt vmcnt(0)" ::: "memory");
        __builtin_amdgcn_s_barrier();
        if (p + 1 < np) stage(p + 1, (p + 1) & 1);
        if (EXCEL_DBG(dbg) & 4) continue;
        f32x2 acc = {0.f, 0.f};
        if (EXCEL_DBG(dbg) & 16) acc = 1e-30f * far_taps(in + (long long)Cmax * tg.base + (long long)(p - 3) * HW);
        taps(std::integral_constant<int, PAR_MASK_DEPTH>{}, p & 1, [&](int di, int k, const f32x2 nb) { acc = __builtin_elementwise_fma(nb, wall[di][k], acc); },
             [&] { asm volatile("" : "+v"(acc)); });
        if (valid) *reinterpret_cast<f32x2*>(out_px + (long long)(p - 3) * HW) = acc;
    }
}

template <bool RAGGED>
__global__ __launch_bounds__(512, 4) void par_stats_tile_kernel(const float* __restrict__ guide, float* __restrict__ stats, TileGeo geo, float w1) {
    constexpr int ND = 6, HALO = 24, TR = 16 + 2 * HALO, TP = PG_TP, NG = 3 * ND, NT = 8 * ND;
    __shared__ __attribute__((aligned(1024))) float tile[2 * TR * TP];
    const Tile tg = tile_of<RAGGED>(geo);
    const int x0 = tg.x0, y0 = tg.y0, H = tg.H, W = tg.W, Wp = tg.Wp;
    const long long HW = tg.HW;
    const int tid = threadIdx.x, lane = tid & 63, tx = tid & 31, ty = tid >> 5;
    const int wave = __builtin_amdgcn_readfirstlane(tid >> 6);
    const int px = x0 + 2 * tx, py = y0 + ty;

    typedef __attribute__((address_space(3))) unsigned char* lds_bptr;
    const __amdgpu_buffer_rsrc_t rs_g = __builtin_amdgcn_make_buffer_rsrc((void*)(guide + 3 * tg.base), 0, (int)(3 * HW * 4), 0x00020000);
    const int xoffA = min(max(x0 - HALO + lane, 0), W - 1) * 4, xoffB = min(max(x0 - HALO + 64 + lane, 0), W - 1) * 4;
    const unsigned tile_b = lds_addr(tile);
    constexpr int RPW = TR / 8;
    const bool interior = x0 - HALO >= 0 && x0 + 64 + HALO <= W;
    const int x4off = min(x0 - HALO + 4 * (lane & 31), Wp - 4) * 4;
    auto stage = [&](int p, int buf) {
        const int plane_off = p * (int)(HW * 4);
        unsigned dst = tile_b + (buf * TR + wave * RPW) * (TP * 4);
        asm volatile("" : "+s"(dst));
        if (interior) {
            int half = lane >> 5;
            asm volatile("" : "+v"(half));
#pragma unroll
            for (int j = 0; j < RPW / 2; ++j) {
                const int gy = min(max(y0 - HALO + wave * RPW + 2 * j + half, 0), H - 1);
                __builtin_amdgcn_raw_ptr_buffer_load_lds(rs_g, (lds_bptr)(unsigned long long)(dst + j * (2 * TP * 4)), 16, gy * Wp * 4 + x4off, plane_off, 0, 0);
            }
            return;
        }
#pragma unroll 4
        for (int rr = 0; rr < RPW; ++rr) {
            const int gy = min(max(y0 - HALO + wave * RPW + rr, 0), H - 1);
            const int soff = plane_off + gy * Wp * 4;
            __builtin_amdgcn_raw_ptr_buffer_load_lds(rs_g, (lds_bptr)(unsigned long long)(dst + rr * (TP * 4)), 4, xoffA, soff, 0, 0);
            __builtin_amdgcn_raw_ptr_buffer_load_lds(rs_g, (lds_bptr)(unsigned long long)(dst + rr * (TP * 4) + 256), 4, xoffB, soff, 0, 0);
        }
    };

    f32x2 acc[ND][8];
#pragma unroll
    for (int di = 0; di < ND; ++di)
#pragma unroll
        for (int k = 0; k < 8; ++k) acc[di][k] = f32x2{0.f, 0.f};

    const unsigned org = tile_b + (ty * TP + 2 * tx) * 4;
    auto taps = [&](int buf, auto&& fn, auto&& pin) {
        unsigned base = org + buf * (TR * TP * 4);
        asm volatile("" : "+v"(base));
        f32x2 sl[2][3];
        auto issue = [&](auto g) {
            constexpr int G = decltype(g)::value, r = G % 3, d = ParD<G / 3>::v, s = G & 1;
            constexpr int row = (HALO + (r - 1) * d) * TP * 4, cl = (d == 1) ? HALO - 2 : HALO - d, cr = (d == 1) ? HALO + 2 : HALO + d;
            sl[s][0] = lds_read8_imm<row + cl * 4>(base);
            if constexpr (r != 1 || d == 1) sl[s][1] = lds_read8_imm<row + HALO * 4>(base);
            sl[s][2] = lds_read8_imm<row + cr * 4>(base);
        };
        issue(std::integral_constant<int, 0>{});
        static_for<NG>([&](auto g) {
            constexpr int G = decltype(g)::value, di = G / 3, r = G % 3, d = ParD<di>::v, s = G & 1;
            constexpr bool mid = (r != 1 || d == 1);
            if constexpr (G + 1 < NG) {
                issue(std::integral_constant<int, G + 1>{});
                constexpr int nxt = ((G + 1) % 3 != 1 || ParD<(G + 1) / 3>::v == 1) ? 3 : 2;
                if constexpr (mid) asm volatile("s_waitcnt lgkmcnt(%3)" : "+v"(sl[s][0]), "+v"(sl[s][1]), "+v"(sl[s][2]) : "n"(nxt) : "memory");
                else asm volatile("s_waitcnt lgkmcnt(%2)" : "+v"(sl[s][0]), "+v"(sl[s][2]) : "n"(nxt) : "memory");
            } else {
                asm volatile("s_waitcnt lgkmcnt(0)" : "+v"(sl[s][0]), "+v"(sl[s][1]), "+v"(sl[s][2])::"memory");
            }
            constexpr int k0 = (r == 0) ? 0 : (r == 1 ? 3 : 5);
            const f32x2 L = sl[s][0], R = sl[s][2];
            if constexpr (d == 1) {
                const f32x2 M = sl[s][1];
                fn(di, k0, f32x2{L[1], M[0]});
                if constexpr (r != 1) fn(di, k0 + 1, M);
                fn(di, k0 + (r != 1 ? 2 : 1), f32x2{M[1], R[0]});
            } else {
                fn(di, k0, L);
                if constexpr (r != 1) fn(di, k0 + 1, sl[s][1]);
                fn(di, k0 + (r != 1 ? 2 : 1), R);
            }
            pin();
            __builtin_amdgcn_sched_barrier(0);
        });
    };

    const bool valid = px < W && py < H;
    float* st_px = stats + 5 * tg.base + (long long)py * Wp + px;
    stage(0, 0);
#pragma unroll 1
    for (int p = 0; p < 3; ++p) {
        asm volatile("s_waitcnt vmcnt(0)" ::: "memory");
        __builtin_amdgcn_s_barrier();
        if (p + 1 < 3) stage(p + 1, (p + 1) & 1);
        f32x2 ctr;
        asm volatile("ds_read_b64 %0, %1 offset:%2\n\ts_waitcnt lgkmcnt(0)" : "=v"(ctr) : "v"(org + (p & 1) * (TR * TP * 4)), "n"((HALO * TP + HALO) * 4) : "memory");
        f32x2 sum = {0.f, 0.f};
        taps(p & 1, [&](int, int, const f32x2 nb) { sum += nb; }, [&] { asm volatile("" : "+v"(sum)); });
        const f32x2 mean = {sum[0] / (float)NT, sum[1] / (float)NT};
        f32x2 nmean = -mean;
        asm volatile("" : "+v"(nmean));
        f32x2 var = {0.f, 0.f};
        taps(p & 1, [&](int, int, const f32x2 nb) { const f32x2 dv = nb + nmean; var = __builtin_elementwise_fma(dv, dv, var); },
             [&] { asm volatile("" : "+v"(var)); });
        f32x2 k2;
#pragma unroll
        for (int q = 0; q < 2; ++q) {
            const float den = sqrtf(var[q] / (float)(NT - 1)) + 1e-8f;
            const float k = 1.f / (den * w1);
            k2[q] = __fmul_rn(k * k, PAR_LOG2E_3);
        }
        if (valid) *reinterpret_cast<f32x2*>(st_px + (long long)p * HW) = k2;
        f32x2 nk2 = -k2, nctr = -ctr;
        asm volatile("" : "+v"(nctr));
        taps(p & 1, [&](int di, int k, const f32x2 nb) {
            const f32x2 dv = nb + nctr;
            acc[di][k] = __builtin_elementwise_fma(dv * dv, nk2, acc[di][k]);
        }, [] {});
    }
    f32x2 m = {-INFINITY, -INFINITY};
#pragma unroll
    for (int di = 0; di < ND; ++di)
#pragma unroll
        for (int k = 0; k < 8; ++k) { m[0] = fmaxf(m[0], acc[di][k][0]); m[1] = fmaxf(m[1], acc[di][k][1]); }
    f32x2 nm = -m;
    asm volatile("" : "+v"(nm));
    f32x2 ssum = {0.f, 0.f};
#pragma unroll
    for (int di = 0; di < ND; ++di)
#pragma unroll
        for (int k = 0; k < 8; ++k) {
            const f32x2 z = acc[di][k] + nm;
            ssum += f32x2{__builtin_amdgcn_exp2f(z[0]), __builtin_amdgcn_exp2f(z[1])};
        }
    if (valid) {
        *reinterpret_cast<f32x2*>(st_px + 3 * HW) = m;
        *reinterpret_cast<f32x2*>(st_px + 4 * HW) = f32x2{1.f / ssum[0], 1.f / ssum[1]};
    }
}

__device__ __forceinline__ float bilinear_ac_px(const float* __restrict__ p, int h, int w, int H, int W, int x, int y) {
    const float sy = (H > 1) ? (float)(h - 1) / (float)(H - 1) : 0.f;
    const float sx = (W > 1) ? (float)(w - 1) / (float)(W - 1) : 0.f;
    const float fy = sy * (float)y, fx = sx * (float)x;
    const int y0 = min((int)fy, h - 1), x0 = min((int)fx, w - 1);
    const int y1 = min(y0 + 1, h - 1), x1 = min(x0 + 1, w - 1);
    const float ly = fy - (float)y0, lx = fx - (float)x0;
    const float top = fmaf(lx, p[y0 * w + x1], __fmul_rn(1.f - lx, p[y0 * w + x0]));
// ... 41 lines not shown
    const int b = blockIdx.y;
    const long long i = (long long)blockIdx.x * 256 + threadIdx.x;
    if (i >= HW) return;
    const int nch = nchan ? min(nchan[b], Cmax) : Cmax;
    const int key = argmax_key(cams + (long long)b * Cmax * HW + i, HW, nch, cls_idx ? cls_idx + (long long)b * Smax : nullptr);
    if (lab8) lab8[(long long)b * HW + i] = (unsigned char)key;
    if (lab64) lab64[(long long)b * HW + i] = key;
}

__global__ __launch_bounds__(256) void argmax_label_ragged_kernel(const float* __restrict__ cams, const int* __restrict__ nchan,
                                                                  const int* __restrict__ cls_idx, int Smax, int Cmax, TileGeo geo,
                                                                  unsigned char* __restrict__ lab8) {
    const Tile t = tile_of<true>(geo);
    const int x = t.x0 + (threadIdx.x & 63);
    if (x >= t.W) return;
    const int nch = nchan ? min(nchan[t.b], Cmax) : Cmax;
    const int* cls_row = cls_idx ? cls_idx + (long long)t.b * Smax : nullptr;
    const float* cb = cams + (long long)Cmax * t.base;
#pragma unroll
    for (int r = 0; r < 4; ++r) {
        const int y = t.y0 + (threadIdx.x >> 6) + 4 * r;
        if (y < t.H) lab8[t.lab + (long long)y * t.W + x] = (unsigned char)argmax_key(cb + (long long)y * t.Wp + x, t.HW, nch, cls_row);
    }
}

#define CONF_MAXBINS 8192
__global__ __launch_bounds__(256) void confusion_kernel(const unsigned char* __restrict__ gt, const unsigned char* __restrict__ pred,
                                                        long long n, int nc, unsigned long long* __restrict__ hist, int head) {
    __shared__ unsigned int lh[CONF_MAXBINS];
    const int bins = nc * nc;
    for (int i = threadIdx.x; i < bins; i += 256) lh[i] = 0;
    __syncthreads();
    if (head > 0 && blockIdx.x == 0 && threadIdx.x < head && threadIdx.x < n) {
        const int g = gt[threadIdx.x], p = pred[threadIdx.x];
        if (g < nc && p < nc) atomicAdd(&lh[g * nc + p], 1u);
    }
    if (head >= 0) {
        gt += head; pred += head; n -= head;
        if (n < 0) n = 0;
    }
    const long long stride = (long long)gridDim.x * 256 * 16;
    for (long long base = ((long long)blockIdx.x * 256 + threadIdx.x) * 16; base < n; base += stride) {
        if (head >= 0 && base + 16 <= n) {
            const uint4 g4 = *reinterpret_cast<const uint4*>(gt + base);
            const uint4 p4 = *reinterpret_cast<const uint4*>(pred + base);
            const unsigned int gw[4] = {g4.x, g4.y, g4.z, g4.w}, pw[4] = {p4.x, p4.y, p4.z, p4.w};
#pragma unroll
            for (int k = 0; k < 16; ++k) {
                const int g = (gw[k >> 2] >> (8 * (k & 3))) & 255, p = (pw[k >> 2] >> (8 * (k & 3))) & 255;
                if (g < nc && p < nc) atomicAdd(&lh[g * nc + p], 1u);
            }
        } else {
            const long long end = (base + 16 < n) ? base + 16 : n;
            for (long long j = base; j < end; ++j) {
                const int g = gt[j], p = pred[j];
                if (g < nc && p < nc) atomicAdd(&lh[g * nc + p], 1u);
            }
        }
    }
    __syncthreads();
    for (int i = threadIdx.x; i < bins; i += 256)
        if (lh[i]) atomicAdd(&hist[i], (unsigned long long)lh[i]);
}

static int make_dil(const int* dil, int ndil, float w1, float w2, ParDil* out) {
    EXCEL_CHECK_ARG(ndil >= 1 && ndil <= 8, "PAR: 1..8 dilations supported (got %d)", ndil);
    const int nt = 8 * ndil;
    double pos[64], mean = 0.0;
    for (int i = 0; i < 8; ++i) out->d[i] = 0;
    for (int i = 0; i < ndil; ++i) {
        EXCEL_CHECK_ARG(dil[i] >= 1, "PAR: dilations must be >= 1 (got %d)", dil[i]);
        out->d[i] = dil[i];
        for (int k = 0; k < 8; ++k) {
            const bool diag = (k == 0 || k == 2 || k == 5 || k == 7);
            pos[i * 8 + k] = (double)(float)((diag ? (float)sqrt(2.0) : 1.f) * (float)dil[i]);
            mean += pos[i * 8 + k];
        }
    }
    mean /= nt;
    double var = 0.0;
    for (int t = 0; t < nt; ++t) var += (pos[t] - mean) * (pos[t] - mean);
    const double sd = (nt > 1) ? sqrt(var / (nt - 1)) : 0.0;
    double z[64], zm = -1e300, zs = 0.0;
    for (int t = 0; t < nt; ++t) {
        const double a = pos[t] / (sd + 1e-8) / (double)w1;
        z[t] = -(a * a);
        if (z[t] > zm) zm = z[t];
    }
    for (int t = 0; t < nt; ++t) { z[t] = exp(z[t] - zm); zs += z[t]; }
    for (int t = 0; t < 64; ++t) out->pos_sm[t] = (t < nt) ? (float)((double)w2 * (z[t] / zs)) : 0.f;
    return EXCEL_OK;
}

#define ND_SWITCH(nd, CALL)                 \
    switch (nd) {                           \
        case 1: CALL(1); break;             \
        case 2: CALL(2); break;             \
        case 3: CALL(3); break;             \
        case 4: CALL(4); break;             \
        case 5: CALL(5); break;             \
        case 6: CALL(6); break;             \
        case 7: CALL(7); break;             \
        default: CALL(8); break;            \
    }

static bool par_dil_ok(const int* dil, int ndil) {
    static const int want[6] = {1, 2, 4, 8, 12, 24};
    if (ndil != 6) return false;
    for (int i = 0; i < 6; ++i)
        if (dil[i] != want[i]) return false;
    return true;
}
int excel_launch_par_affinity(const float* img, float* aff, const TileGeo& geo, int total_tiles, const int* dil, int ndil, float w1, float w2,
                              hipStream_t st, int compact) {
    ProfScope prof__(PROF_PAR_AFFINITY, st);
    ParDil dl;
    int rc = make_dil(dil, ndil, w1, w2, &dl);
    if (rc) return rc;
    const bool tiled = compact && par_dil_ok(dil, ndil) && ((((uintptr_t)img | (uintptr_t)aff) & 15) == 0) &&
                       (geo.tab ? true : (geo.W % 4 == 0 && geo.W >= 8 && 5LL * geo.H * geo.W * 4 < (1LL << 31)));
    if (geo.tab) {
        EXCEL_CHECK_ARG(compact && ndil == 6, "par_affinity: ragged batches use the compact statistics of the 6-dilation kernel");
        if (tiled) hipLaunchKernelGGL((par_stats_tile_kernel<true>), dim3(total_tiles), dim3(512), 0, st, img, aff, geo, w1);
        else hipLaunchKernelGGL((par_affinity_kernel<6, true>), dim3(total_tiles, 4), dim3(256), 0, st, img, aff, dl, geo, w1, 1);
    } else if (tiled) {
        hipLaunchKernelGGL((par_stats_tile_kernel<false>), dim3(cdiv(geo.W, 64), cdiv(geo.H, 16), geo.B), dim3(512), 0, st, img, aff, geo, w1);
    } else {
#define CALL(N) hipLaunchKernelGGL((par_affinity_kernel<N, false>), dim3(cdiv(geo.W, 64), cdiv(geo.H, 4), geo.B), dim3(256), 0, st, img, aff, dl, geo, w1, compact ? 1 : 0)
        ND_SWITCH(ndil, CALL)
#undef CALL
    }
    EXCEL_CHECK_LAUNCH("par_affinity");
    return EXCEL_OK;
}

int excel_launch_par_iterate(const float* aff, const float* in, float* out, const int* nchan, int B, int Cmax, int H, int W,
                             const int* dil, int ndil, hipStream_t st) {
    ProfScope prof__(PROF_PAR_ITERATE, st);
    ParDil dl;
    int rc = make_dil(dil, ndil, 0.3f, 0.01f, &dl);
    if (rc) return rc;
    hipLaunchKernelGGL(par_iterate_stream_kernel, dim3(cdiv(W, 64), cdiv(H, 4), B), dim3(256), 0, st, aff, in, out, nchan, dl, ndil, Cmax, H, W);
    EXCEL_CHECK_LAUNCH("par_iterate");
    return EXCEL_OK;
}

int excel_par_guide_supported(const void* guide, const void* stats, const void* in, const void* out, int Cmax, long long max_plane, int Wp,
                              const int* dil, int ndil) {
    const bool vec = (Wp % 4) == 0 && Wp >= 4 && ((((uintptr_t)guide | (uintptr_t)stats | (uintptr_t)in | (uintptr_t)out) & 15) == 0);
    const long long planes = Cmax > 5 ? Cmax : 5;
    return (vec && par_dil_ok(dil, ndil) && planes * max_plane * 4 < (1LL << 31)) ? 1 : 0;
}

int excel_launch_par_iterate_guide(const float* guide, const float* stats, const float* in, float* out, const int* nchan, int Cmax,
                                   const TileGeo& geo, int total_tiles, const int* dil, int ndil, float w1, float w2, hipStream_t st) {
    EXCEL_CHECK_ARG(par_dil_ok(dil, ndil), "par_iterate_guide: unsupported dilation set");
    ProfScope prof__(PROF_PAR_ITERATE, st);
    ParDil dl;
    int rc = make_dil(dil, ndil, w1, w2, &dl);
    if (rc) return rc;
    int dbg = 0;
#ifdef EXCEL_DEV
    static const int env_dbg = getenv("EXCEL_PAR_DBG") ? atoi(getenv("EXCEL_PAR_DBG")) : 0;
    dbg = env_dbg;
#endif
    if (geo.tab)
        hipLaunchKernelGGL((par_iterate_guide_kernel<true>), dim3(total_tiles), dim3(512), 0, st, guide, stats, in, out, nchan, dl, Cmax, geo, dbg);
    else
        hipLaunchKernelGGL((par_iterate_guide_kernel<false>), dim3(cdiv(geo.W, 64), cdiv(geo.H, 16), geo.B), dim3(512), 0, st, guide, stats,
                           in, out, nchan, dl, Cmax, geo, dbg);
    EXCEL_CHECK_LAUNCH("par_iterate_guide");
    return EXCEL_OK;
}

int excel_launch_bilinear_ac(const float* in, float* out, int planes, int h, int w, int H, int W, hipStream_t st) {
    ProfScope prof__(PROF_OTHER, st);
    const long long n = (long long)planes * H * W;
    hipLaunchKernelGGL(bilinear_ac_kernel, dim3((unsigned)cdivl(n, 256)), dim3(256), 0, st, in, out, planes, h, w, H, W);
    EXCEL_CHECK_LAUNCH("bilinear_ac");
    return EXCEL_OK;
}

int excel_launch_bilinear_ac_ragged(const float* in, float* out, int h, int w, const TileGeo& geo, int total_tiles, hipStream_t st) {
    ProfScope prof__(PROF_OTHER, st);
    hipLaunchKernelGGL(bilinear_ac_ragged_kernel, dim3(total_tiles, 3), dim3(256), 0, st, in, out, h, w, geo);
    EXCEL_CHECK_LAUNCH("bilinear_ac_ragged");
    return EXCEL_OK;
}

int excel_launch_argmax_label(const float* cams, const int* nchan, const int* cls_idx, int B, int Smax, int Cmax, long long HW,
                              unsigned char* lab8, long long* lab64, hipStream_t st) {
    ProfScope prof__(PROF_ARGMAX, st);
    hipLaunchKernelGGL(argmax_label_kernel, dim3((unsigned)cdivl(HW, 256), B), dim3(256), 0, st, cams, nchan, cls_idx, Smax, Cmax, HW, lab8, lab64);
    EXCEL_CHECK_LAUNCH("argmax_label");
    return EXCEL_OK;
}

int excel_launch_argmax_label_ragged(const float* cams, const int* nchan, const int* cls_idx, int Smax, int Cmax, const TileGeo& geo,
                                     int total_tiles, unsigned char* lab8, hipStream_t st) {
    ProfScope prof__(PROF_ARGMAX, st);
    hipLaunchKernelGGL(argmax_label_ragged_kernel, dim3(total_tiles), dim3(256), 0, st, cams, nchan, cls_idx, Smax, Cmax, geo, lab8);
    EXCEL_CHECK_LAUNCH("argmax_label_ragged");
    return EXCEL_OK;
}

int excel_launch_confusion(const unsigned char* gt, const unsigned char* pred, long long n, int nc, unsigned long long* hist,
                           hipStream_t st) {
    ProfScope prof__(PROF_CONFUSION, st);
    EXCEL_CHECK_ARG(nc >= 1 && nc * nc <= CONF_MAXBINS, "confusion: num_classes %d too large", nc);
    const int mg = (int)((16 - ((uintptr_t)gt & 15)) & 15), mp = (int)((16 - ((uintptr_t)pred & 15)) & 15);
    const int head = (mg == mp) ? mg : -1;
    const int blocks = (int)((cdivl(n, 256 * 16) < 2048) ? cdivl(n, 256 * 16) : 2048);
    hipLaunchKernelGGL(confusion_kernel, dim3(blocks > 0 ? blocks : 1), dim3(256), 0, st, gt, pred, n, nc, hist, head);
    EXCEL_CHECK_LAUNCH("confusion");
    return EXCEL_OK;
}
```

### excel_amd/ops.py

```python
import ctypes as C
import os

import torch

from . import _lib
from ._lib import check, lib

PAR_DILATIONS = (1, 2, 4, 8, 12, 24)


def _p(t, dtype=torch.float32):
    if t is None:
        return None
    if not t.is_cuda:
        raise RuntimeError("excel_amd ops need GPU tensors (the HIP library is the only compute path)")
    if t.dtype != dtype:
        raise TypeError(f"expected {dtype}, got {t.dtype}")
    if not t.is_contiguous():
        raise ValueError("tensor must be contiguous")
    return C.c_void_p(t.data_ptr())


def _stream():
    return C.c_void_p(torch.cuda.current_stream().cuda_stream)
# ... 548 lines not shown

def seg_softmax_resize_ragged(planes, src_plan, dst_plan, nc):
    if src_plan.B != dst_plan.B:
        raise ValueError(f"seg_softmax_resize_ragged: plans of {src_plan.B} and {dst_plan.B} images")
    if planes.numel() != nc * src_plan.total_pix:
        raise ValueError(f"seg_softmax_resize_ragged: planes must hold nc * total_pix = {nc * src_plan.total_pix} floats")
    prob = torch.empty((nc * dst_plan.total_label_pix,), dtype=torch.float32, device=planes.device)
    check(lib().excel_seg_softmax_resize_ragged(_p(planes), _p(src_plan.table, torch.int32), C.byref(src_plan.info), _p(dst_plan.table, torch.int32),
                                                C.byref(dst_plan.info), int(nc), _p(prob), _stream()), "excel_seg_softmax_resize_ragged")
    return prob


def clip_feature_surgery(image_features, text_features, num_fg=None, t=2.0, want_full=True):
    image_features = f32c(image_features)
    text_features = f32c(text_features)
    B, N, Cc = image_features.shape
    T = text_features.shape[0]
    dev = image_features.device
    full = torch.empty((B, N, T), dtype=torch.float32, device=dev) if want_full else None
    F_ = T if num_fg is None else num_fg
    sl = torch.empty((B, N - 1, F_), dtype=torch.float32, device=dev) if num_fg is not None else None
    ws = _ws(lib().excel_cam_workspace_bytes(B, N, T), dev)
    check(lib().excel_clip_feature_surgery(_p(image_features), _p(text_features), B, N, Cc, T, F_, float(t), _p(full), _p(sl),
                                           _p(ws, torch.uint8), _stream()), "excel_clip_feature_surgery")
    return full, sl


def patch_text_cam(x_raw, text_features, num_fg=None, t=2.0, want_full=False, want_features=False, mode="bf16x3"):
    x_raw = f32c(x_raw)
    text_features = f32c(text_features)
    B, N, Cc = x_raw.shape
    T = text_features.shape[0]
    dev = x_raw.device
    full = torch.empty((B, N, T), dtype=torch.float32, device=dev) if want_full else None
    F_ = T if num_fg is None else num_fg
    sl = torch.empty((B, N - 1, F_), dtype=torch.float32, device=dev) if num_fg is not None else None
    feats = torch.empty_like(x_raw) if want_features else None
    if full is None and sl is None:
        raise ValueError("patch_text_cam: nothing to compute (want_full=False and num_fg=None)")
    ws = _ws(lib().excel_patch_text_cam_workspace_bytes(B, N, Cc, T), dev)
    check(lib().excel_patch_text_cam(_p(x_raw), _p(text_features), B, N, Cc, T, F_, float(t), GEMM_MODES["f16x3" if mode == "f16x2" else mode], _p(full), _p(sl),
                                     _p(feats), _p(ws, torch.uint8), _stream()), "excel_patch_text_cam")
    return full, sl, feats


def attn_layer_mean(attn, n_layers=6):
    attn = f32c(attn)
    Lw, B, N, _ = attn.shape
    n = min(n_layers, Lw)
    out = torch.empty((B, N - 1, N - 1), dtype=torch.float32, device=attn.device)
    check(lib().excel_attn_layer_mean(_p(attn), Lw, B, N, Lw - n, n, _p(out), _stream()), "excel_attn_layer_mean")
    return out


def attn_select_mean(attn, seg_attn, n_layers=6):
    attn = f32c(attn)
    seg_attn = f32c(seg_attn)
    Lw, B, N, _ = attn.shape
    n = min(n_layers, Lw)
    if tuple(seg_attn.shape) != (B, N - 1, N - 1):
        raise ValueError(f"seg_attn must be [B,P,P] = {(B, N - 1, N - 1)}, got {tuple(seg_attn.shape)}")
    out = torch.empty((B, N - 1, N - 1), dtype=torch.float32, device=attn.device)
    ws = _ws(lib().excel_attn_select_workspace_bytes(B, n), attn.device)
    check(lib().excel_attn_select_mean(_p(attn), Lw, B, N, Lw - n, n, _p(seg_attn), _p(out), _p(ws, torch.uint8), _stream()),
          "excel_attn_select_mean")
    return out


def feature_affinity(feats, mode, beta=1.0, gamma=3.0):
    feats = f32c(feats)
    feats = feats.reshape(feats.shape[0], feats.shape[1], -1)
    B, Cc, P = feats.shape
    out = torch.empty((B, P, P), dtype=torch.float32, device=feats.device)
    ws = _ws(lib().excel_feature_affinity_workspace_bytes(B, Cc, P), feats.device)
    check(lib().excel_feature_affinity(_p(feats), B, Cc, P, float(beta), float(gamma), {"sigmoid": 0, "mask_softmax": 1}[mode],
                                       _p(out), _p(ws, torch.uint8), _stream()), "excel_feature_affinity")
    return out


def feature_affinity_grouped(feats, mode, group, member_stride=1, beta=1.0, gamma=3.0, out=None):
    feats = f32c(feats)
    feats = feats.reshape(feats.shape[0], feats.shape[1], -1)
    B, Cc, P = feats.shape
    out = _out(out, (B, P, P), torch.float32, feats.device)
    ws = _ws(lib().excel_feature_affinity_grouped_workspace_bytes(B, Cc, P, int(group)), feats.device)
    check(lib().excel_feature_affinity_grouped(_p(feats), B, Cc, P, int(group), int(member_stride), float(beta), float(gamma),
                                               {"sigmoid": 0, "mask_softmax": 1}[mode], _p(out), _p(ws, torch.uint8), _stream()),
          "excel_feature_affinity_grouped")
    return out


def compute_trans_mat(w_aff):
    single = w_aff.dim() == 2
    w = f32c(w_aff[None] if single else w_aff)
    B, P, _ = w.shape
    out = torch.empty_like(w)
    ws = _ws(lib().excel_trans_mat_workspace_bytes(B, P), w.device)
    check(lib().excel_compute_trans_mat(_p(w), B, P, _p(out), _p(ws, torch.uint8), _stream()), "excel_compute_trans_mat")
    return out[0] if single else out


def cls_compact(onehot, smax, want_nchan=False):
    onehot = f32c(onehot)
    B, F_ = onehot.shape
    idx = torch.empty((B, smax), dtype=torch.int32, device=onehot.device)
    n = torch.empty((B,), dtype=torch.int32, device=onehot.device)
    nch = torch.empty((B,), dtype=torch.int32, device=onehot.device) if want_nchan else None
    check(lib().excel_cls_compact(_p(onehot), B, F_, smax, _p(idx, torch.int32), _p(n, torch.int32), _p(nch, torch.int32),
                                  _stream()), "excel_cls_compact")
    return (idx, n, nch) if want_nchan else (idx, n)


def scoremap_box_mask(attr, cls_idx, ncls, g, caa_thre=0.79, want_mask=False):
    attr = f32c(attr)
    B, P, F_ = attr.shape
    smax = cls_idx.shape[1]
    v = torch.zeros((B, smax, P), dtype=torch.float32, device=attr.device)
    m = torch.zeros((B, smax, P), dtype=torch.uint8, device=attr.device) if want_mask else None
    check(lib().excel_scoremap_box_mask(_p(attr), _p(cls_idx, torch.int32), _p(ncls, torch.int32), B, g, F_, smax, float(caa_thre),
                                        _p(v), _p(m, torch.uint8), _stream()), "excel_scoremap_box_mask")
    return v, m


def refine_cams_with_aff_batched(attr, w_aff, cls_idx, ncls, g, caa_thre=0.79):
    attr = f32c(attr)
    w_aff = f32c(w_aff)
    B, P, F_ = attr.shape
    smax = cls_idx.shape[1]
    out = torch.zeros((B, smax, P), dtype=torch.float32, device=attr.device)
    ws = _ws(lib().excel_refine_workspace_bytes(B, P, smax), attr.device)
    check(lib().excel_refine_cams_with_aff(_p(attr), _p(w_aff), _p(cls_idx, torch.int32), _p(ncls, torch.int32), B, g, F_, smax,
                                           float(caa_thre), _p(out), _p(ws, torch.uint8), _stream()), "excel_refine_cams_with_aff")
    return out


def _out(out, shape, dtype, device, zero=False):
    if out is not None:
        if tuple(out.shape) != tuple(shape) or out.dtype != dtype or not out.is_contiguous():
            raise ValueError(f"out= must be a contiguous {dtype} tensor of shape {tuple(shape)}, got {out.dtype} {tuple(out.shape)}")
        return out
    return (torch.zeros if zero else torch.empty)(shape, dtype=dtype, device=device)


def cam_upsample_bkg(refined, ncls, g, H, W, out=None, zero_unused=True):
    refined = f32c(refined)
    B, smax, P = refined.shape
    cams = _out(out, (B, smax + 1, H, W), torch.float32, refined.device)
    ws = _ws(B * smax * P * 4, refined.device)
    check(lib().excel_cam_upsample_bkg(_p(refined), _p(ncls, torch.int32), B, g, smax, H, W, _p(cams), _p(ws, torch.uint8),
                                       1 if zero_unused else 0, _stream()), "excel_cam_upsample_bkg")
    return cams


def par_forward(imgs, masks, dilations=PAR_DILATIONS, num_iter=20, nchan=None, w1=0.3, w2=0.01, stream_affinities=False, out=None, ws=None):
    imgs = f32c(imgs)
    masks = f32c(masks)
    B, Cmax, H, W = masks.shape
    assert imgs.shape[0] == B and imgs.shape[1] == 3
    h, w = imgs.shape[-2:]
    out = _out(out, masks.shape, torch.float32, masks.device, zero=nchan is not None)
    dil = (C.c_int32 * len(dilations))(*dilations)
    need = lib().excel_par_workspace_bytes(B, Cmax, H, W, len(dilations))
    if ws is None or ws.numel() < need:
        ws = _ws(need, masks.device)
    check(lib().excel_par_forward(_p(imgs), h, w, _p(masks), _p(nchan, torch.int32), B, Cmax, H, W, dil, len(dilations), num_iter,
                                  w1, w2, _p(out), _p(ws, torch.uint8), 1 if stream_affinities else 0, _stream()), "excel_par_forward")
    return out


class RaggedPlan:

    def __init__(self, hw, device):
        import numpy as np
        hw = np.ascontiguousarray(np.asarray(hw, np.int32).reshape(-1, 2))
        self.hw = hw
        self.B = int(hw.shape[0])
        self.info = _lib.RaggedInfo()
        ptr = hw.ctypes.data_as(C.POINTER(C.c_int32))
        check(lib().excel_ragged_plan(ptr, self.B, C.byref(self.info), None), "excel_ragged_plan")
        table = np.empty(int(self.info.table_ints), np.int32)
        check(lib().excel_ragged_plan(ptr, self.B, C.byref(self.info), table.ctypes.data_as(C.POINTER(C.c_int32))), "excel_ragged_plan")
        self.table_host = table
        rec = table[:8 * (self.B + 1)].reshape(self.B + 1, 8)
        self.poff = rec[:, 2].astype(np.int64)
        self.loff = rec[:, 4].astype(np.int64)
        self.total_pix = int(self.info.total_pix)
        self.total_label_pix = int(self.info.total_label_pix)
        self.total_tiles = int(self.info.total_tiles)
        self.table = torch.from_numpy(table).to(device, non_blocking=True) if device is not None else None

    def planes(self, packed, b, K):
        H, W = int(self.hw[b, 0]), int(self.hw[b, 1])
        Wp = (W + 3) // 4 * 4
        o = K * int(self.poff[b])
        return packed[o:o + K * H * Wp].view(K, H, Wp)[:, :, :W]

    def label(self, packed_u8, b):
        H, W = int(self.hw[b, 0]), int(self.hw[b, 1])
        o = int(self.loff[b])
        return packed_u8[o:o + H * W].view(H, W)


def normalize_resize_u8_ragged(hwc_packed, plan, S, mean=(123.675, 116.28, 103.53), std=(58.395, 57.12, 57.375), out=None):
    if hwc_packed.dtype != torch.uint8 or hwc_packed.numel() != 3 * plan.total_label_pix:
        raise ValueError(f"hwc_packed must hold {3 * plan.total_label_pix} uint8 values")
    out = _out(out, (plan.B, 3, S, S), torch.float32, hwc_packed.device)
    m, s = (C.c_double * 3)(*mean), (C.c_double * 3)(*std)
    check(lib().excel_normalize_resize_u8_ragged(_p(hwc_packed, torch.uint8), _p(plan.table, torch.int32), plan.B, S, m, s, _p(out), _stream()),
          "excel_normalize_resize_u8_ragged")
    return out


def normalize_resize_u8_ragged_mirror(hwc_packed, plan, S, mean=(123.675, 116.28, 103.53), std=(58.395, 57.12, 57.375), out=None):
    if hwc_packed.dtype != torch.uint8 or hwc_packed.numel() != 3 * plan.total_label_pix:
        raise ValueError(f"hwc_packed must hold {3 * plan.total_label_pix} uint8 values")
    out = _out(out, (2 * plan.B, 3, S, S), torch.float32, hwc_packed.device)
    m, s = (C.c_double * 3)(*mean), (C.c_double * 3)(*std)
    check(lib().excel_normalize_resize_u8_ragged_mirror(_p(hwc_packed, torch.uint8), _p(plan.table, torch.int32), plan.B, S, m, s, _p(out),
                                                        _stream()), "excel_normalize_resize_u8_ragged_mirror")
    return out


CAM_OVERLAY_MODES = {"max": 0, "per_class": 1}
_CAM_TABLES = {}


def cam_overlay_tables(alpha, device, mean=(123.675, 116.28, 103.53), std=(58.395, 57.12, 57.375)):
    key = (float(alpha), tuple(mean), tuple(std), str(device))
    t = _CAM_TABLES.get(key)
    if t is None:
        from .utils import imutils
        t = _CAM_TABLES[key] = torch.from_numpy(imutils.cam_overlay_tables(alpha, mean, std)).to(device)
    return t


def _pinned_upload(a, dtype, device):
    import numpy as np
    h = torch.from_numpy(np.ascontiguousarray(a)).to(dtype).pin_memory()
    return h.to(device, non_blocking=True)


def cam_overlay_ragged(hwc_packed, cams, plan, Cmax, ncls, mode="max", alpha=None, mean=(123.675, 116.28, 103.53),
                       std=(58.395, 57.12, 57.375)):
    import numpy as np
    if mode not in CAM_OVERLAY_MODES:
        raise ValueError(f"mode must be one of {sorted(CAM_OVERLAY_MODES)}, got {mode!r}")
    if alpha is None:
        alpha = 0.5 if mode == "max" else 0.6
    ncls = np.asarray(ncls, np.int64).reshape(-1)
    if ncls.shape[0] != plan.B or (ncls < 0).any() or (ncls > Cmax - 1).any():
        raise ValueError(f"ncls: need {plan.B} values in [0, Cmax - 1 = {Cmax - 1}], got {ncls.tolist()}")
    if hwc_packed.dtype != torch.uint8 or hwc_packed.numel() != 3 * plan.total_label_pix:
        raise ValueError(f"hwc_packed must hold {3 * plan.total_label_pix} uint8 values")
    if cams.numel() < Cmax * plan.total_pix:
        raise ValueError(f"cams must hold Cmax * total_pix = {Cmax * plan.total_pix} floats, got {cams.numel()}")
    dev = hwc_packed.device
    hw = plan.hw.astype(np.int64)
    if mode == "max":
        off = 3 * plan.loff[:plan.B]
        nbytes = 3 * plan.total_label_pix
    else:
        sizes = 3 * ncls * hw[:, 0] * hw[:, 1]
        off = np.concatenate([[0], np.cumsum(sizes)])[:plan.B]
        nbytes = int(sizes.sum())
    out = torch.empty(max(int(nbytes), 1), dtype=torch.uint8, device=dev)[:int(nbytes)]
    if nbytes == 0:
        return out, off
    n_dev = _pinned_upload(ncls, torch.int32, dev)
    off_dev = _pinned_upload(off, torch.int64, dev) if mode == "per_class" else None
    tabs = cam_overlay_tables(alpha, dev, mean, std)
    check(lib().excel_cam_overlay_ragged(_p(hwc_packed, torch.uint8), _p(cams[:Cmax * plan.total_pix]), Cmax, _p(n_dev, torch.int32),
                                         _p(off_dev, torch.int64), _p(plan.table, torch.int32), C.byref(plan.info), CAM_OVERLAY_MODES[mode],
                                         _p(tabs, torch.float64), _p(out, torch.uint8), _stream()), "excel_cam_overlay_ragged")
    return out, off


def cam_overlay(hwc, cams, mode="max", alpha=None, mean=(123.675, 116.28, 103.53), std=(58.395, 57.12, 57.375)):
    if mode not in CAM_OVERLAY_MODES:
        raise ValueError(f"mode must be one of {sorted(CAM_OVERLAY_MODES)}, got {mode!r}")
    if alpha is None:
        alpha = 0.5 if mode == "max" else 0.6
    cams = f32c(cams)
    k, H, W = cams.shape[0] - 1, cams.shape[1], cams.shape[2]
    if hwc.dtype != torch.uint8 or tuple(hwc.shape) != (H, W, 3):
        raise ValueError(f"hwc must be uint8 [{H},{W},3], got {hwc.dtype} {tuple(hwc.shape)}")
    if mode == "max" and k == 0:
        return None
    out = torch.empty((H, W, 3) if mode == "max" else (k, H, W, 3), dtype=torch.uint8, device=cams.device)
    if out.numel() == 0:
        return out
    tabs = cam_overlay_tables(alpha, cams.device, mean, std)
    check(lib().excel_cam_overlay(_p(hwc.contiguous(), torch.uint8), _p(cams), k, H, W, CAM_OVERLAY_MODES[mode], _p(tabs, torch.float64),
                                  _p(out, torch.uint8), _stream()), "excel_cam_overlay")
    return out


TRAIN_PANELS = ("img1", "cam1", "pseu_aff", "pseu_mid", "seg_gt", "seg_pred")
TB_MEAN, TB_STD = (0.485, 0.456, 0.406), (0.229, 0.224, 0.225)
_PANEL_TABLES = {}


def train_panels_plan(B, S, g, panels=TRAIN_PANELS, nrow=2):
    unknown = [n for n in panels if n not in TRAIN_PANELS]
    if unknown:
        raise ValueError(f"unknown panels {unknown}; known: {list(TRAIN_PANELS)}")
    mask = sum(1 << TRAIN_PANELS.index(n) for n in set(panels))
    out = (C.c_int64 * (3 * len(TRAIN_PANELS) + 1))()
    check(lib().excel_train_panels_plan(int(B), int(nrow), int(S), int(g), mask, out), "excel_train_panels_plan")
    plan = {n: (int(out[3 * k]), int(out[3 * k + 1]), int(out[3 * k + 2])) for k, n in enumerate(TRAIN_PANELS) if (mask >> k) & 1}
    return plan, int(out[3 * len(TRAIN_PANELS)])


class TrainPanels(dict):
    buffer = None
    plan = None

    def host(self):
        buf = self.buffer.cpu().numpy()
        return {n: buf[off:off + 3 * Hg * Wg].reshape(Hg, Wg, 3) for n, (Hg, Wg, off) in self.plan.items()}
# ... 60 lines not shown


_PNG_PALETTES = {}


def png_labels_bound_bytes(H, W):
    return int(lib().excel_png_labels_bound_bytes(int(H), int(W)))


def png_labels_arena_bytes(hw):
    return sum(png_labels_bound_bytes(h, w) for h, w in hw)


def _png_palette(palette, device):
    import numpy as np
    from .utils import imutils
    pal = imutils.colormap() if palette is None else np.asarray(palette)
    if pal.dtype != np.uint8 or pal.size != 768:
        raise ValueError(f"palette must hold 256 RGB uint8 entries, got {pal.dtype} {pal.shape}")
    key = (pal.tobytes(), str(device))
    t = _PNG_PALETTES.get(key)
    if t is None:
        if len(_PNG_PALETTES) > 16:
            _PNG_PALETTES.clear()
        t = _PNG_PALETTES[key] = torch.from_numpy(np.ascontiguousarray(pal).reshape(-1).copy()).to(device)
    return t


def png_encode_labels_ragged(labels_flat, plan, palette=None, out=None, ws=None):
    import numpy as np
    if plan is None:
        if labels_flat.dim() != 3:
            raise ValueError("plan=None needs a uniform [B,H,W] label tensor")
        Bn, H, W = labels_flat.shape
        plan = RaggedPlan([(H, W)] * Bn, labels_flat.device)
    if labels_flat.dtype != torch.uint8 or labels_flat.numel() != plan.total_label_pix:
        raise ValueError(f"labels must hold {plan.total_label_pix} uint8 values, got {labels_flat.dtype} x {labels_flat.numel()}")
    dev = labels_flat.device
    hw = np.ascontiguousarray(plan.hw, np.int32)
    need = png_labels_arena_bytes(hw)
    if out is None:
        out = torch.empty(need, dtype=torch.uint8, device=dev)
    elif out.dtype != torch.uint8 or out.dim() != 1 or not out.is_contiguous():
        raise ValueError("out= must be a flat contiguous uint8 tensor")
    ws_need = int(lib().excel_png_labels_workspace_bytes(plan.B, int(hw[:, 0].max())))
    if ws is None:
        ws = _ws(ws_need, dev)
    table = torch.empty((plan.B, 2), dtype=torch.int64, device=dev)
    check(lib().excel_png_encode_labels_ragged(_p(labels_flat.contiguous().view(-1), torch.uint8), _p(plan.table, torch.int32), C.byref(plan.info),
                                               hw.ctypes.data_as(C.POINTER(C.c_int32)), _p(_png_palette(palette, dev), torch.uint8),
                                               _p(out, torch.uint8), out.numel(), _p(table, torch.int64), _p(ws, torch.uint8), ws.numel(),
                                               _stream()), "excel_png_encode_labels_ragged")
    return out[:need], table


AUG_CANDIDATES = 10
AUG_PARAMS_DTYPE = None


def aug_params_dtype():
    import numpy as np
    global AUG_PARAMS_DTYPE
    if AUG_PARAMS_DTYPE is None:
        AUG_PARAMS_DTYPE = np.dtype([("ratio", "<f8"), ("flip", "<i4"), ("h_pad", "<i4"), ("w_pad", "<i4"),
                                     ("cand_h", "<i4", (AUG_CANDIDATES,)), ("cand_w", "<i4", (AUG_CANDIDATES,))], align=True)
        assert AUG_PARAMS_DTYPE.itemsize == C.sizeof(_lib.AugParams)
    return AUG_PARAMS_DTYPE


class TrainAugPlan:

    def __init__(self, hw, params, S, device):
        import numpy as np
        hw = np.ascontiguousarray(np.asarray(hw, np.int32).reshape(-1, 2))
        params = np.ascontiguousarray(params, dtype=aug_params_dtype())
        if params.shape != (hw.shape[0],):
            raise ValueError(f"params: {params.shape[0] if params.ndim else 0} records for {hw.shape[0]} images")
        self.B, self.S = int(hw.shape[0]), int(S)
        self.hw, self.params = hw, params
        self.info = _lib.TrainAugInfo()
        hp = hw.ctypes.data_as(C.POINTER(C.c_int32))
        pp = params.ctypes.data_as(C.POINTER(_lib.AugParams))
        check(lib().excel_train_aug_plan(hp, pp, self.B, self.S, C.byref(self.info), None), "excel_train_aug_plan")
        table = np.empty(int(self.info.table_ints), np.int32)
        check(lib().excel_train_aug_plan(hp, pp, self.B, self.S, C.byref(self.info), table.ctypes.data_as(C.POINTER(C.c_int32))),
              "excel_train_aug_plan")
        self.table_host = table
        self.workspace_bytes = int(lib().excel_train_augment_workspace_bytes(C.byref(self.info)))
        self.table = None
        if device is not None:
            self.table = torch.from_numpy(table).pin_memory().to(device, non_blocking=True)


def train_augment(images_u8, plan, labels_u8, params, crop_size, mean=(123.675, 116.28, 103.53), std=(58.395, 57.12, 57.375),
                  aug_plan=None):
    S = int(crop_size)
    if S <= 0:
        raise ValueError("crop_size must be positive")
    dev = images_u8.device
    if aug_plan is None:
        aug_plan = TrainAugPlan(plan.hw, params, S, dev)
    if aug_plan.S != S or aug_plan.B != plan.B or aug_plan.table is None:
        raise ValueError("aug_plan was built for another batch / crop size, or without a device table")
    n = int(aug_plan.info.total_label_pix)
    if images_u8.dtype != torch.uint8 or images_u8.numel() != 3 * n:
        raise ValueError(f"images_u8 must hold {3 * n} uint8 values")
    if labels_u8.dtype != torch.uint8 or labels_u8.numel() != n:
        raise ValueError(f"labels_u8 must hold {n} uint8 values")
    B = plan.B
    img = torch.empty((B, 3, S, S), dtype=torch.float32, device=dev)
    label = torch.empty((B, S, S), dtype=torch.uint8, device=dev)
    box = torch.empty((B, 4), dtype=torch.int32, device=dev)
    ws = _ws(aug_plan.workspace_bytes, dev)
    m, s = (C.c_double * 3)(*mean), (C.c_double * 3)(*std)
    check(lib().excel_train_augment(_p(images_u8, torch.uint8), _p(labels_u8, torch.uint8), _p(aug_plan.table, torch.int32),
                                    C.byref(aug_plan.info), m, s, _p(img), _p(label, torch.uint8), _p(box, torch.int32),
                                    _p(ws, torch.uint8), _stream()), "excel_train_augment")
    return img, label, box


def train_augment_image(images_u8, plan, params, crop_size, aug_plan=None, mean=(123.675, 116.28, 103.53), std=(58.395, 57.12, 57.375)):
    S = int(crop_size)
    if S <= 0:
        raise ValueError("crop_size must be positive")
    dev = images_u8.device
    if aug_plan is None:
        aug_plan = TrainAugPlan(plan.hw, params, S, dev)
    if aug_plan.S != S or aug_plan.B != plan.B or aug_plan.table is None:
        raise ValueError("aug_plan was built for another batch / crop size, or without a device table")
    n = int(aug_plan.info.total_label_pix)
    if images_u8.dtype != torch.uint8 or images_u8.numel() != 3 * n:
        raise ValueError(f"images_u8 must hold {3 * n} uint8 values")
    B = plan.B
    img = torch.empty((B, 3, S, S), dtype=torch.float32, device=dev)
    box = torch.empty((B, 4), dtype=torch.int32, device=dev)
    ws = _ws(aug_plan.workspace_bytes, dev)
    m, s = (C.c_double * 3)(*mean), (C.c_double * 3)(*std)
    check(lib().excel_train_augment_image(_p(images_u8, torch.uint8), _p(aug_plan.table, torch.int32), C.byref(aug_plan.info), m, s,
                                          _p(img), _p(box, torch.int32), _p(ws, torch.uint8), _stream()), "excel_train_augment_image")
    return img, box


def cam_upsample_bkg_ragged(refined, ncls, g, plan, out=None, zero_unused=True):
    refined = f32c(refined)
    B, smax, P = refined.shape
    assert B == plan.B
    cams = _out(out, ((smax + 1) * plan.total_pix,), torch.float32, refined.device)
    ws = _ws(B * smax * P * 4, refined.device)
    check(lib().excel_cam_upsample_bkg_ragged(_p(refined), _p(ncls, torch.int32), _p(plan.table, torch.int32), C.byref(plan.info), g, smax,
                                              _p(cams), _p(ws, torch.uint8), 1 if zero_unused else 0, _stream()), "excel_cam_upsample_bkg_ragged")
    return cams


def par_forward_ragged(imgs, masks, plan, Cmax, dilations=PAR_DILATIONS, num_iter=20, nchan=None, w1=0.3, w2=0.01, out=None, ws=None):
    imgs = f32c(imgs)
    assert imgs.shape[0] == plan.B and imgs.shape[1] == 3 and masks.numel() == Cmax * plan.total_pix
    h, w = imgs.shape[-2:]
    out = _out(out, masks.shape, torch.float32, masks.device, zero=True)
    dil = (C.c_int32 * len(dilations))(*dilations)
    need = lib().excel_par_ragged_workspace_bytes(plan.total_pix, Cmax)
    if ws is None or ws.numel() < need:
        ws = _ws(need, masks.device)
    check(lib().excel_par_forward_ragged(_p(imgs), h, w, _p(masks), _p(nchan, torch.int32), _p(plan.table, torch.int32), C.byref(plan.info), Cmax,
                                         dil, len(dilations), num_iter, w1, w2, _p(out), _p(ws, torch.uint8), _stream()), "excel_par_forward_ragged")
    return out


def argmax_label_ragged(cams, plan, Cmax, nchan=None, cls_idx=None, out=None):
    smax = cls_idx.shape[1] if cls_idx is not None else Cmax - 1
    lab = _out(out, (plan.total_label_pix,), torch.uint8, cams.device)
    check(lib().excel_argmax_label_ragged(_p(cams), _p(nchan, torch.int32), _p(cls_idx, torch.int32), _p(plan.table, torch.int32), C.byref(plan.info),
                                          smax, Cmax, _p(lab, torch.uint8), _stream()), "excel_argmax_label_ragged")
    return lab


def argmax_label(cams, nchan=None, cls_idx=None, want_i64=False):
    cams = f32c(cams)
    B, Cmax, H, W = cams.shape
    smax = cls_idx.shape[1] if cls_idx is not None else Cmax - 1
    l8 = torch.empty((B, H, W), dtype=torch.uint8, device=cams.device)
    l64 = torch.empty((B, H, W), dtype=torch.int64, device=cams.device) if want_i64 else None
    check(lib().excel_argmax_label(_p(cams), _p(nchan, torch.int32), _p(cls_idx, torch.int32), B, smax, Cmax, H * W,
                                   _p(l8, torch.uint8), _p(l64, torch.int64), _stream()), "excel_argmax_label")
    return (l8, l64) if want_i64 else l8


def confusion_accumulate(gt_u8, pred_u8, num_classes, hist=None):
    gt = gt_u8.contiguous().view(-1)
    pr = pred_u8.contiguous().view(-1)
    assert gt.numel() == pr.numel()
    if hist is None:
        hist = torch.zeros((num_classes, num_classes), dtype=torch.int64, device=gt.device)
    check(lib().excel_confusion_accumulate(_p(gt, torch.uint8), _p(pr, torch.uint8), gt.numel(), num_classes,
                                           _p(hist, torch.int64), _stream()), "excel_confusion_accumulate")
    return hist


def attr_aggregate(text_features, bank, num_fg, topK=0.9):
    text_features = f32c(text_features)
    bank = f32c(bank)
    T, Cc = text_features.shape
    K = bank.shape[1]
    out = torch.empty((Cc, T), dtype=torch.float32, device=text_features.device)
    check(lib().excel_attr_aggregate(_p(text_features), _p(bank), num_fg, T, Cc, K, float(topK), _p(out), _stream()),
          "excel_attr_aggregate")
    return out


def bilinear_resize(x, H, W, align_corners=False):
    x = f32c(x)
    h, w = x.shape[-2:]
    planes = x.numel() // (h * w)
    out = torch.empty(x.shape[:-2] + (H, W), dtype=torch.float32, device=x.device)
    check(lib().excel_bilinear_resize(_p(x), _p(out), planes, h, w, H, W, 1 if align_corners else 0, _stream()),
          "excel_bilinear_resize")
    return out


def pos_embed_resize(pos, g):
    pos = f32c(pos)
    side = int(round((pos.shape[0] - 1) ** 0.5))
    D = pos.shape[1]
    out = torch.empty((g * g + 1, D), dtype=torch.float32, device=pos.device)
    check(lib().excel_pos_embed_resize(_p(pos), side, g, D, _p(out), _stream()), "excel_pos_embed_resize")
    return out


def flip_max_normalize(attr, g):
    attr = f32c(attr)
    B2, P, F_ = attr.shape
    out = torch.empty((B2 // 2, P, F_), dtype=torch.float32, device=attr.device)
    check(lib().excel_flip_max_normalize(_p(attr), _p(out), B2 // 2, g, F_, _stream()), "excel_flip_max_normalize")
    return out


def lam_scale_accumulate(maps, acc, g, H, W, init):
    maps = f32c(maps)
    B2, P, F_ = maps.shape
    if acc is None:
        acc = torch.empty((B2 // 2, F_, H, W), dtype=torch.float32, device=maps.device)
        init = True
    check(lib().excel_lam_scale_accumulate(_p(maps), _p(acc), B2 // 2, g, F_, H, W, 1 if init else 0, _stream()),
          "excel_lam_scale_accumulate")
    return acc


def plane_minmax_normalize_(lam):
    H, W = lam.shape[-2:]
    check(lib().excel_plane_minmax_normalize(_p(lam), lam.numel() // (H * W), H * W, _stream()), "excel_plane_minmax_normalize")
    return lam


def prof_enable(on=True, categories=None, every=1):
    check(lib().excel_prof_set_sampling(int(every)), "excel_prof_set_sampling")
    mask = (1 << 64) - 1
    if categories is not None:
        names = [lib().excel_prof_category_name(i).decode() for i in range(lib().excel_prof_num_categories())]
        mask = 0
        for c in categories:
            mask |= 1 << names.index(c)
    check(lib().excel_prof_set_mask(mask), "excel_prof_set_mask")
    check(lib().excel_prof_enable(1 if on else 0), "excel_prof_enable")


def dcrf_inference(image_u8, prob, iters, pos_w, pos_xy_std, bi_w, bi_xy_std, bi_rgb_std, is_energy=False):
    prob = f32c(prob)
    if image_u8.dtype != torch.uint8 or not image_u8.is_contiguous():
        image_u8 = image_u8.to(torch.uint8).contiguous()
    Cn, H, W = prob.shape
    assert tuple(image_u8.shape) == (H, W, 3), (tuple(image_u8.shape), (H, W, 3))
    out = torch.empty_like(prob)
    ws = _ws(lib().excel_dcrf_workspace_bytes(H, W, Cn), prob.device)
    check(lib().excel_dcrf_inference(_p(image_u8, torch.uint8), _p(prob), 1 if is_energy else 0, H, W, Cn, int(iters), float(pos_w), float(pos_xy_std),
                                     float(bi_w), float(bi_xy_std), float(bi_rgb_std), _p(out), _p(ws, torch.uint8), _stream()), "excel_dcrf_inference")
    return out


_dcrf_budget_warned = False


def dcrf_ragged_workspace_bytes(hw, C_):
    total = sum(int(h) * int(w) for h, w in hw)
    out = C.c_size_t(0)
    check(lib().excel_dcrf_ragged_workspace_bytes(total, int(C_), C.byref(out)), "excel_dcrf_ragged_workspace_bytes")
    return int(out.value)


def dcrf_groups(hw, C_, budget_bytes):
    sizes = [(int(h), int(w)) for h, w in hw]
    runs, start = [], 0
    for b in range(1, len(sizes) + 1):
        if b == len(sizes):
            runs.append((start, b))
            break
        try:
            fits = dcrf_ragged_workspace_bytes(sizes[start:b + 1], C_) <= budget_bytes
        except RuntimeError:
            fits = False
        if not fits:
            runs.append((start, b))
            start = b
    return runs


def dcrf_inference_ragged(images_u8, plan, unary, C_, iters, pos_w, pos_xy_std, bi_w, bi_xy_std, bi_rgb_std, is_energy=False, want_labels=True,
                          want_q=False, budget_bytes=None):
    if not (want_labels or want_q):
        raise ValueError("dcrf_inference_ragged: ask for labels, q or both")
    n = plan.total_label_pix
    if images_u8.dtype != torch.uint8 or images_u8.numel() != 3 * n:
        raise ValueError(f"dcrf_inference_ragged: images_u8 must hold {3 * n} uint8 values")
    if unary.dtype != torch.float32 or unary.numel() != C_ * n:
        raise ValueError(f"dcrf_inference_ragged: unary must hold C * total_label_pix = {C_ * n} float32 values")
    images_u8, unary = images_u8.view(-1), unary.view(-1)
    dev = unary.device
    labels = torch.empty((n,), dtype=torch.uint8, device=dev) if want_labels else None
    q = torch.empty((C_ * n,), dtype=torch.float32, device=dev) if want_q else None
# ... 112 lines not shown
```

### include/excel_hip.h

```cpp
#ifndef EXCEL_HIP_H
#define EXCEL_HIP_H
#include <stddef.h>
#include <stdint.h>

#ifdef __cplusplus
extern "C" {
#endif

const char* excel_last_error(void);
int excel_abi_version(void);
const char* excel_build_id(void);


int excel_gemm_f32(const float* A, const float* Bm, float* C, const float* bias, const float* residual,
                   int M, int N, int K, int lda, int ldb, int ldc, int ldr, int b_kmajor, int act,
                   int batch, long long sA, long long sB, long long sC, long long sR, void* stream);

int excel_split_bf16(const float* in, void* out, long long rows, int K, void* stream);
int excel_gemm_bf16x3(const void* A_split, const void* W_split, float* C, const float* bias, const float* residual,
                      int M, int N, int K, int act, int split_out, void* stream);
int excel_split_f16(const float* in, void* out, long long rows, int K, void* stream);
int excel_gemm_f16x3(const void* A_split, const void* W_split, float* C, const float* bias, const float* residual,
                     int M, int N, int K, int act, int split_out, void* stream);
int excel_pack_f16(const float* in, void* out, long long rows, int K, unsigned long long* inexact_dev, void* stream);
// ... 8 lines not shown
int excel_layernorm(const float* x, const float* w, const float* b, float* y, int rows, int D, float eps, void* stream);


typedef struct {
    int width, layers, heads, patch, out_dim;
    int n_surgery;
    int pos_grid;
} excel_vit_config;

typedef struct {
    const float *ln1_w, *ln1_b;
    const float *in_proj_w, *in_proj_b;
    const float *out_proj_w, *out_proj_b;
    const float *ln2_w, *ln2_b;
    const float *fc1_w, *fc1_b;
    const float *fc2_w, *fc2_b;
} excel_vit_block_weights;

typedef struct {
    const float* conv1_w;
    const float* class_emb;
    const float* pos_emb;
    const float *ln_pre_w, *ln_pre_b, *ln_post_w, *ln_post_b;
    const float* proj;
    const excel_vit_block_weights* blocks;
} excel_vit_weights;

typedef struct excel_vit* excel_vit_t;

int excel_vit_create(const excel_vit_config* cfg, const excel_vit_weights* w, excel_vit_t* out);
void excel_vit_destroy(excel_vit_t h);

int excel_vit_set_gemm_mode(excel_vit_t h, int mode);
int excel_vit_get_gemm_mode(excel_vit_t h);
int excel_vit_weights_fp16_exact(excel_vit_t h);

size_t excel_vit_workspace_bytes(excel_vit_t h, int B, int S);

int excel_vit_forward(excel_vit_t h, const float* img, int B, int S, void* workspace, size_t workspace_bytes,
                      float* image_features, float* x_raw, float* w_aff, int aff_layers,
                      float* attn_out, int n_attn_out, float* feats_out, void* stream);

#define EXCEL_VIT_FEATS_AS_REFERENCE 1
int excel_vit_forward_ex(excel_vit_t h, const float* img, int B, int S, void* workspace, size_t workspace_bytes,
                         float* image_features, float* x_raw, float* w_aff, int aff_layers,
                         float* attn_out, int n_attn_out, float* feats_out, const float* ex_attn, int flags, void* stream);

size_t excel_feature_affinity_workspace_bytes(int B, int C, int P);
int excel_feature_affinity(const float* feats, int B, int C, int P, float beta, float gamma, int mode, float* out,
                           void* workspace, void* stream);

size_t excel_feature_affinity_grouped_workspace_bytes(int B, int C, int P, int group);
int excel_feature_affinity_grouped(const float* feats, int B, int C, int P, int group, int member_stride, float beta, float gamma,
                                   int mode, float* out, void* workspace, void* stream);

typedef struct excel_decoder* excel_decoder_t;
typedef struct { int vit_layers, vit_width, embed, dec_layers, heads, num_classes; } excel_decoder_config;
typedef struct { const float *proj_w, *proj_b, *proj2_w, *proj2_b; } excel_fuse_layer_weights;
typedef struct {
    const float *ln1_w, *ln1_b, *in_proj_w, *in_proj_b, *out_proj_w, *out_proj_b, *ln2_w, *ln2_b, *fc1_w, *fc1_b, *fc2_w, *fc2_b;
} excel_decoder_block_weights;
typedef struct {
    const excel_fuse_layer_weights* fuse;
    const float *fuse_w, *fuse_b;
    const excel_decoder_block_weights* blocks;
    const float *pred_w, *pred_b;
} excel_decoder_weights;
int excel_decoder_create(const excel_decoder_config* cfg, const excel_decoder_weights* w, excel_decoder_t* out);
void excel_decoder_destroy(excel_decoder_t h);
size_t excel_decoder_workspace_bytes(excel_decoder_t h, int B, int g);
int excel_decoder_forward(excel_decoder_t h, const float* all_feats, int B, int g, void* workspace, size_t workspace_bytes,
                          float* attn_fts_out, float* seg_out, void* stream);

typedef struct excel_text* excel_text_t;
typedef struct { int vocab_size, context_length, width, layers, heads, embed_dim; } excel_text_config;
typedef struct {
    const float *token_embedding, *positional_embedding, *ln_final_w, *ln_final_b, *text_projection;
    const excel_decoder_block_weights* blocks;
} excel_text_weights;
int excel_text_create(const excel_text_config* cfg, const excel_text_weights* w, excel_text_t* out);
void excel_text_destroy(excel_text_t h);
size_t excel_text_workspace_bytes(excel_text_t h, int B);
int excel_text_encode(excel_text_t h, const int32_t* tokens, int B, float* out, void* workspace, size_t workspace_bytes, void* stream);
int excel_prompt_ensemble(const float* emb, int n, int E, float* out, void* stream);

size_t excel_train_losses_workspace_bytes(int B, int nc, int H, int W);
int excel_train_losses(const float* seg, const float* attn_pred, const unsigned char* pseudo, const unsigned char* aff_labels, int B, int nc,
                       int g_h, int g_w, int H, int W, int radius, int ignore_index, float w_seg, float w_diver, float* losses,
                       float* d_seg, float* d_attn_pred, void* workspace, void* stream);

size_t excel_decoder_train_workspace_bytes(excel_decoder_t h, int B, int g);
int excel_decoder_forward_train(excel_decoder_t h, const float* all_feats, int B, int g, void* workspace, size_t workspace_bytes,
                                float* seg_out, float* attn_pred_out, float dropout_p, unsigned dropout_seed, void* stream);
int excel_decoder_train_attn_fts(excel_decoder_t h, int B, int g, const void* workspace, size_t workspace_bytes, float* attn_fts_out,
                                 void* stream);
int excel_decoder_backward(excel_decoder_t h, const float* all_feats, int B, int g, void* workspace, size_t workspace_bytes,
                           const float* d_seg, const float* d_attn_pred, const excel_decoder_weights* grads, float dropout_p,
                           unsigned dropout_seed, void* stream);
int excel_adamw_step(float* param, const float* grad, float* exp_avg, float* exp_avg_sq, long long n, float lr, float beta1, float beta2,
                     float eps, float weight_decay, int step, void* stream);

int excel_lam_to_label(const float* cam, const float* cls_label, const int32_t* img_box, int B, int F, int H, int W, float bkg_thre,
                       float high_thre, float low_thre, int ignore_mid, int ignore_index, float* valid_cam, unsigned char* label,
                       void* stream);

int excel_normalize_img_u8(const unsigned char* hwc, int B, int H, int W, const double* mean3, const double* std3, float* out, void* stream);

int excel_denormalize_img(const float* img, int B, int H, int W, const float* mean3, const float* std3, unsigned char* out_u8,
                          float* out_f32, void* stream);

int excel_seg_scale_accumulate(const float* segs, float* acc, int B, int nc, int h, int w, int H, int W, int flip_mean, int init,
                               float scale, void* stream);


size_t excel_cam_workspace_bytes(int B, int N, int T);
int excel_clip_feature_surgery(const float* image_features, const float* text, int B, int N, int C, int T, int F,
                               float temperature, float* out_full, float* out_slice, void* workspace, void* stream);

size_t excel_patch_text_cam_workspace_bytes(int B, int N, int C, int T);
int excel_patch_text_cam(const float* x_raw, const float* text, int B, int N, int C, int T, int F, float temperature, int mode,
                         float* out_full, float* out_slice, float* image_features, void* workspace, void* stream);


size_t excel_dcrf_workspace_bytes(int H, int W, int C);
int excel_dcrf_inference(const unsigned char* rgb_hwc, const float* prob, int prob_is_energy, int H, int W, int C, int iters, float pos_w,
                         float pos_xy_std, float bi_w, float bi_xy_std, float bi_rgb_std, float* q_out, void* workspace, void* stream);



int excel_attn_layer_mean(const float* attn, int Lw, int B, int N, int first_layer, int n_layers, float* w_aff, void* stream);

size_t excel_attn_select_workspace_bytes(int B, int n_layers);
int excel_attn_select_mean(const float* attn, int Lw, int B, int N, int first_layer, int n_layers, const float* seg_attn,
                           float* w_out, void* workspace, void* stream);

size_t excel_trans_mat_workspace_bytes(int B, int P);
int excel_compute_trans_mat(const float* w_aff, int B, int P, float* trans_out, void* workspace, void* stream);

int excel_cls_compact(const float* onehot, int B, int F, int Smax, int32_t* cls_idx, int32_t* ncls, int32_t* nchan, void* stream);

int excel_scoremap_box_mask(const float* attr, const int32_t* cls_idx, const int32_t* ncls, int B, int g, int F, int Smax,
                            double caa_thre, float* v_out, uint8_t* mask_out, void* stream);

size_t excel_refine_workspace_bytes(int B, int P, int Smax);
int excel_refine_cams_with_aff(const float* attr, const float* w_aff, const int32_t* cls_idx, const int32_t* ncls,
                               int B, int g, int F, int Smax, double caa_thre, float* refined, void* workspace, void* stream);

#define EXCEL_CAMS_ZERO_UNUSED 1
int excel_cam_upsample_bkg(const float* refined, const int32_t* ncls, int B, int g, int Smax, int H, int W, float* cams,
                           void* workspace, int flags, void* stream);


#define EXCEL_PAR_STREAM_AFFINITIES 1
size_t excel_par_workspace_bytes(int B, int Cmax, int H, int W, int ndil);
int excel_par_forward(const float* imgs, int h, int w, const float* masks, const int32_t* nchan, int B, int Cmax, int H, int W,
                      const int32_t* dilations , int ndil, int n_iter, float w1, float w2, float* out,
                      void* workspace, int flags, void* stream);

int excel_argmax_label(const float* cams, const int32_t* nchan, const int32_t* cls_idx, int B, int Smax, int Cmax,
                       long long HW, uint8_t* labels_u8, int64_t* labels_i64, void* stream);

int excel_confusion_accumulate(const uint8_t* gt, const uint8_t* pred, long long n, int num_classes, int64_t* hist, void* stream);

typedef struct {
    int32_t B, total_tiles;
    int64_t total_pix;
    int64_t total_label_pix;
    int64_t max_plane_pix;
    int64_t table_ints;
} excel_ragged_info;
int excel_ragged_plan(const int32_t* hw , int B, excel_ragged_info* info , int32_t* table );

int excel_normalize_resize_u8_ragged(const uint8_t* hwc, const int32_t* table, int B, int S, const double* mean3 ,
                                     const double* std3 , float* out, void* stream);

int excel_normalize_resize_u8_ragged_mirror(const uint8_t* hwc, const int32_t* table, int B, int S, const double* mean3 ,
                                            const double* std3 , float* out, void* stream);

int excel_cam_upsample_bkg_ragged(const float* refined, const int32_t* ncls, const int32_t* table, const excel_ragged_info* info, int g,
                                  int Smax, float* cams, void* workspace, int flags, void* stream);

size_t excel_par_ragged_workspace_bytes(long long total_pix, int Cmax);
int excel_par_forward_ragged(const float* imgs, int h, int w, const float* masks, const int32_t* nchan, const int32_t* table,
                             const excel_ragged_info* info, int Cmax, const int32_t* dilations , int ndil, int n_iter, float w1,
                             float w2, float* out, void* workspace, void* stream);

int excel_argmax_label_ragged(const float* cams, const int32_t* nchan, const int32_t* cls_idx, const int32_t* table,
                              const excel_ragged_info* info, int Smax, int Cmax, uint8_t* labels_u8, void* stream);

int excel_seg_msc_fuse_ragged(const float* const* segs , const int32_t* g , const int32_t* flip_mean ,
                              int ns, int nc, const int32_t* table, const excel_ragged_info* info, float* planes, uint8_t* labels_u8,
                              void* stream);

int excel_seg_resize_argmax_ragged(const float* planes, const int32_t* src_table, const excel_ragged_info* src_info, const int32_t* dst_table,
                                   const excel_ragged_info* dst_info, int nc, uint8_t* labels_u8, void* stream);

int excel_seg_resize_argmax_uniform(const float* segs, int B, int h, int w, int nc, const int32_t* dst_table, const excel_ragged_info* dst_info,
                                    uint8_t* labels_u8, void* stream);

int excel_seg_softmax_resize(const float* planes, int h, int w, int nc, int H, int W, float* prob, void* stream);

int excel_seg_softmax_resize_ragged(const float* planes, const int32_t* src_table, const excel_ragged_info* src_info, const int32_t* dst_table,
                                    const excel_ragged_info* dst_info, int nc, float* prob, void* stream);

int excel_dcrf_ragged_workspace_bytes(long long total_label_pix, int C, size_t* bytes );
int excel_dcrf_inference_ragged(const uint8_t* hwc, const float* unary, int unary_is_energy, const int32_t* table,
                                const excel_ragged_info* info, int C, int iters, float pos_w, float pos_xy_std, float bi_w,
                                float bi_xy_std, float bi_rgb_std, uint8_t* labels_u8, float* q_out, void* workspace, void* stream);

int excel_dcrf_lam_ragged_workspace_bytes(const int32_t* hw , const int32_t* nchan , int B, size_t* bytes );
int excel_dcrf_lam_ragged(const uint8_t* hwc, const float* cams, const int32_t* nchan , const int32_t* nchan_host ,
                          const int32_t* cls_idx , const int32_t* table, const excel_ragged_info* info, int smax,
                          int Cmax, int iters, float pos_w, float pos_xy_std, float bi_w, float bi_xy_std, float bi_rgb_std,
                          uint8_t* labels_u8, float* q_out, void* workspace, void* stream);

#define EXCEL_CAM_OVERLAY_MAX 0
#define EXCEL_CAM_OVERLAY_PER_CLASS 1
int excel_cam_overlay_ragged(const uint8_t* hwc, const float* cams, int Cmax, const int32_t* ncls, const int64_t* out_off,
                             const int32_t* table, const excel_ragged_info* info, int mode, const double* tables, uint8_t* out, void* stream);
int excel_cam_overlay(const uint8_t* hwc, const float* cams, int k, int H, int W, int mode, const double* tables, uint8_t* out, void* stream);

#define EXCEL_TRAIN_PANELS 6
#define EXCEL_TRAIN_PANEL_IMG1 0
#define EXCEL_TRAIN_PANEL_CAM1 1
#define EXCEL_TRAIN_PANEL_PSEU_AFF 2
#define EXCEL_TRAIN_PANEL_PSEU_MID 3
#define EXCEL_TRAIN_PANEL_SEG_GT 4
#define EXCEL_TRAIN_PANEL_SEG_PRED 5
#define EXCEL_TRAIN_PANELS_PLAN_INTS (3 * EXCEL_TRAIN_PANELS + 1)
int excel_train_panels_plan(int B, int nrow, int S, int g, int panel_mask, int64_t* out );
int excel_train_panels(const float* img, const float* attr, const float* cls_label, const uint8_t* pseu_aff, const uint8_t* pseu_mid,
                       const uint8_t* seg_gt, const uint8_t* seg_pred, int B, int F, int P, int g, int S, int nrow, int panel_mask,
                       const float* mean , const float* std , const double* jet, const uint8_t* palette, uint8_t* out,
                       size_t out_bytes, void* stream);

size_t excel_png_labels_bound_bytes(int H, int W);
size_t excel_png_labels_workspace_bytes(int B, int max_h);
int excel_png_encode_labels_ragged(const uint8_t* labels, const int32_t* table, const excel_ragged_info* info, const int32_t* hw ,
                                   const uint8_t* palette, uint8_t* arena, size_t arena_bytes, int64_t* out_table, void* workspace,
                                   size_t workspace_bytes, void* stream);

#define EXCEL_AUG_CANDIDATES 10
typedef struct {
    double ratio;
    int32_t flip;
    int32_t h_pad, w_pad;
    int32_t cand_h[EXCEL_AUG_CANDIDATES];
    int32_t cand_w[EXCEL_AUG_CANDIDATES];
} excel_aug_params;
typedef struct {
    int32_t B, S, max_h, max_w2;
    int64_t table_ints;
    int64_t workspace_bytes;
    int64_t total_label_pix;
} excel_train_aug_info;
#define EXCEL_AUG_REC 40
int excel_train_aug_plan(const int32_t* hw , const excel_aug_params* params , int B, int S,
                         excel_train_aug_info* info , int32_t* table );
size_t excel_train_augment_workspace_bytes(const excel_train_aug_info* info);
int excel_train_augment(const uint8_t* hwc, const uint8_t* labels, const int32_t* table, const excel_train_aug_info* info,
                        const double* mean3 , const double* std3 , float* img, uint8_t* label, int32_t* img_box,
                        void* workspace, void* stream);
int excel_train_augment_image(const uint8_t* hwc, const int32_t* table, const excel_train_aug_info* info, const double* mean3 ,
                              const double* std3 , float* img, int32_t* img_box, void* workspace, void* stream);


int excel_attr_aggregate(const float* text, const float* bank, int F, int T, int C, int K, double topK, float* out, void* stream);

int excel_bilinear_resize(const float* in, float* out, long long planes, int h, int w, int H, int W, int align_corners, void* stream);

int excel_pos_embed_resize(const float* pos, int side, int g, int D, float* out, void* stream);

int excel_flip_max_normalize(const float* attr, float* out, int B, int g, int F, void* stream);

int excel_lam_scale_accumulate(const float* maps, float* acc, int B, int g, int F, int H, int W, int init, void* stream);
int excel_plane_minmax_normalize(float* lam, long long planes, long long HW, void* stream);


int excel_prof_enable(int on);
int excel_prof_set_mask(unsigned long long category_mask);
int excel_prof_set_sampling(int every);
int excel_prof_num_categories(void);
const char* excel_prof_category_name(int cat);
int excel_prof_collect(double* ms , long long* launches , double* work );

#ifdef __cplusplus
}
#endif
#endif
```

Before: 1492.

## Add 32-row tall tiles with triple-buffered LDS staging to PAR iterate kernel

Adds a 32-row tile variant of the PAR guided-iterate kernel using 1024-thread blocks, dynamic LDS and a three-slot load pipeline with graded vmcnt waits. Each block then loads proportionally less of the 24-row halo, cutting redundant global-to-LDS traffic per output pixel. A heuristic picks tall tiles when there are enough of them to fill the CUs. The ragged plan now records per-image tall-tile offsets. The cost is fewer, larger blocks (lower occupancy and fewer blocks for tail balancing) and more complex synchronisation.

```diff
diff --git a/excel_amd/_lib.py b/excel_amd/_lib.py
--- a/excel_amd/_lib.py
+++ b/excel_amd/_lib.py
@@ -55,7 +55,7 @@
 
 class RaggedInfo(C.Structure):
     _fields_ = [("B", C.c_int32), ("total_tiles", C.c_int32), ("total_pix", C.c_int64), ("total_label_pix", C.c_int64),
-                ("max_plane_pix", C.c_int64), ("table_ints", C.c_int64)]
+                ("max_plane_pix", C.c_int64), ("table_ints", C.c_int64), ("total_tall_tiles", C.c_int64)]
 
 
 class AugParams(C.Structure):
@@ -138,6 +138,7 @@
     "excel_refine_cams_with_aff": (c_i, [c_f, c_f, c_f, c_f, c_i, c_i, c_i, c_i, C.c_double, c_f, c_f, c_f]),
     "excel_cam_upsample_bkg": (c_i, [c_f, c_f, c_i, c_i, c_i, c_i, c_i, c_f, c_f, c_i, c_f]),
     "excel_par_workspace_bytes": (c_sz, [c_i, c_i, c_i, c_i, c_i]),
+    "excel_par_tile_rows": (c_i, [c_i, c_ll, c_i]),
     "excel_par_forward": (c_i, [c_f, c_i, c_i, c_f, c_f, c_i, c_i, c_i, c_i, C.POINTER(C.c_int32), c_i, c_i,
                                 C.c_float, C.c_float, c_f, c_f, c_i, c_f]),
     "excel_ragged_plan": (c_i, [C.POINTER(C.c_int32), c_i, C.POINTER(RaggedInfo), C.POINTER(C.c_int32)]),
@@ -146,7 +147,7 @@
     "excel_cam_upsample_bkg_ragged": (c_i, [c_f, c_f, c_f, C.POINTER(RaggedInfo), c_i, c_i, c_f, c_f, c_i, c_f]),
     "excel_par_ragged_workspace_bytes": (c_sz, [c_ll, c_i]),
     "excel_par_forward_ragged": (c_i, [c_f, c_i, c_i, c_f, c_f, c_f, C.POINTER(RaggedInfo), c_i, C.POINTER(C.c_int32), c_i, c_i,
-                                       C.c_float, C.c_float, c_f, c_f, c_f]),
+                                       C.c_float, C.c_float, c_f, c_f, c_i, c_f]),
     "excel_argmax_label_ragged": (c_i, [c_f, c_f, c_f, c_f, C.POINTER(RaggedInfo), c_i, c_i, c_f, c_f]),
     "excel_seg_msc_fuse_ragged": (c_i, [C.POINTER(C.c_void_p), C.POINTER(C.c_int32), C.POINTER(C.c_int32), c_i, c_i, c_f, C.POINTER(RaggedInfo),
                                         c_f, c_f, c_f]),
diff --git a/excel_amd/csrc/abi.hip b/excel_amd/csrc/abi.hip
--- a/excel_amd/csrc/abi.hip
+++ b/excel_amd/csrc/abi.hip
@@ -16,7 +16,7 @@
 }
 
 extern "C" const char* excel_last_error(void) { return g_err; }
-extern "C" int excel_abi_version(void) { return 4; }
+extern "C" int excel_abi_version(void) { return 5; }
 #ifndef EXCEL_BUILD_ID
 #define EXCEL_BUILD_ID "unstamped"
 #endif
@@ -660,24 +660,25 @@
 
 extern "C" int excel_ragged_plan(const int32_t* hw, int B, excel_ragged_info* info, int32_t* table) {
     EXCEL_CHECK_ARG(hw && info && B >= 1, "ragged_plan: bad argument");
-    long long pix = 0, lab = 0, tiles = 0, max_plane = 0;
+    long long pix = 0, lab = 0, tiles = 0, tall = 0, max_plane = 0;
     for (int b = 0; b < B; ++b) {
         const long long H = hw[2 * b], W = hw[2 * b + 1];
         EXCEL_CHECK_ARG(H >= 1 && W >= 1, "ragged_plan: image %d has size %lld x %lld", b, H, W);
-        const long long Wp = (W + 3) / 4 * 4, plane = H * Wp, nt = ((W + 63) / 64) * ((H + 15) / 16);
+        const long long Wp = (W + 3) / 4 * 4, plane = H * Wp, nt = ((W + 63) / 64) * ((H + 15) / 16), nt32 = ((W + 63) / 64) * ((H + 31) / 32);
         if (table) {
             int32_t* rec = table + EXCEL_RAG_REC * b;
-            rec[0] = (int32_t)H; rec[1] = (int32_t)W; rec[2] = (int32_t)pix; rec[3] = (int32_t)tiles; rec[4] = (int32_t)lab; rec[5] = rec[6] = rec[7] = 0;
+            rec[0] = (int32_t)H; rec[1] = (int32_t)W; rec[2] = (int32_t)pix; rec[3] = (int32_t)tiles; rec[4] = (int32_t)lab; rec[5] = (int32_t)tall; rec[6] = rec[7] = 0;
             for (long long t = 0; t < nt; ++t) table[EXCEL_RAG_REC * (B + 1) + tiles + t] = b;
         }
-        pix += plane; lab += H * W; tiles += nt;
+        pix += plane; lab += H * W; tiles += nt; tall += nt32;
         if (plane > max_plane) max_plane = plane;
         EXCEL_CHECK_ARG(pix < (1LL << 31) && 3 * lab < (1LL << 31) && tiles < (1LL << 31), "ragged_plan: batch too large for 32-bit offsets");
     }
     if (table) {
         int32_t* rec = table + EXCEL_RAG_REC * B;
-        rec[0] = rec[1] = 0; rec[2] = (int32_t)pix; rec[3] = (int32_t)tiles; rec[4] = (int32_t)lab; rec[5] = rec[6] = rec[7] = 0;
-    }
+        rec[0] = rec[1] = 0; rec[2] = (int32_t)pix; rec[3] = (int32_t)tiles; rec[4] = (int32_t)lab; rec[5] = (int32_t)tall; rec[6] = rec[7] = 0;
+    }
+    info->total_tall_tiles = tall;
     info->B = B; info->total_tiles = (int32_t)tiles; info->total_pix = pix; info->total_label_pix = lab; info->max_plane_pix = max_plane;
     info->table_ints = EXCEL_RAG_REC * (long long)(B + 1) + tiles;
     return EXCEL_OK;
@@ -749,6 +750,10 @@
     const size_t hw = (size_t)H * W;
     return align_up((size_t)B * 8 * ndil * hw * sizeof(float), 256) + align_up((size_t)B * Cmax * hw * sizeof(float), 256) +
            align_up((size_t)B * 3 * hw * sizeof(float), 256);
+}
+
+extern "C" int excel_par_tile_rows(int uniform_H, long long tall_tiles, int flags) {
+    return excel_par_pick_tile_rows(uniform_H, tall_tiles, (flags & EXCEL_PAR_TILE_ROWS_16) ? 16 : (flags & EXCEL_PAR_TILE_ROWS_32) ? 32 : 0);
 }
 
 template <class Step>
@@ -787,10 +792,12 @@
         hipMemcpyAsync(out, masks, sizeof(float) * (size_t)B * Cmax * hw, hipMemcpyDeviceToDevice, st);
         return EXCEL_OK;
     }
-    if (recompute)
+    if (recompute) {
+        const int rows = excel_par_tile_rows(H, (long long)B * cdiv(W, 64) * cdiv(H, 32), flags);
         return par_jacobi(masks, out, pp, n_iter, [&](const float* cur, float* dst) {
-            return excel_launch_par_iterate_guide(gimg, aff, cur, dst, nchan, Cmax, geo, 0, dilations, ndil, w1, w2, st);
+            return excel_launch_par_iterate_guide(gimg, aff, cur, dst, nchan, Cmax, geo, 0, rows, dilations, ndil, w1, w2, st);
         });
+    }
     return par_jacobi(masks, out, pp, n_iter, [&](const float* cur, float* dst) {
         return excel_launch_par_iterate(aff, cur, dst, nchan, B, Cmax, H, W, dilations, ndil, st);
     });
@@ -803,7 +810,7 @@
 
 extern "C" int excel_par_forward_ragged(const float* imgs, int h, int w, const float* masks, const int32_t* nchan, const int32_t* table,
                                         const excel_ragged_info* info, int Cmax, const int32_t* dilations, int ndil, int n_iter, float w1,
-                                        float w2, float* out, void* workspace, void* stream) {
+                                        float w2, float* out, void* workspace, int flags, void* stream) {
     EXCEL_CHECK_ARG(imgs && masks && out && workspace && dilations && table && info, "par_forward_ragged: null argument");
     EXCEL_CHECK_ARG(n_iter >= 1 && Cmax > 0 && h > 0 && w > 0 && info->B > 0, "par_forward_ragged: bad n_iter / shape");
     const size_t tp = (size_t)info->total_pix;
@@ -818,8 +825,10 @@
                     "(Wp = W rounded up to 4)");
     TRY(excel_launch_bilinear_ac_ragged(imgs, guide, h, w, geo, info->total_tiles, st));
     TRY(excel_launch_par_affinity(guide, stats, geo, info->total_tiles, dilations, ndil, w1, w2, st, 1));
+    const int rows = excel_par_tile_rows(0, info->total_tall_tiles, flags);
+    const int tiles = rows == 32 ? (int)info->total_tall_tiles : info->total_tiles;
     return par_jacobi(masks, out, pp, n_iter, [&](const float* cur, float* dst) {
-        return excel_launch_par_iterate_guide(guide, stats, cur, dst, nchan, Cmax, geo, info->total_tiles, dilations, ndil, w1, w2, st);
+        return excel_launch_par_iterate_guide(guide, stats, cur, dst, nchan, Cmax, geo, tiles, rows, dilations, ndil, w1, w2, st);
     });
 }
 
diff --git a/excel_amd/csrc/common.h b/excel_amd/csrc/common.h
--- a/excel_amd/csrc/common.h
+++ b/excel_amd/csrc/common.h
@@ -111,13 +111,35 @@
     t.HW = (long long)t.H * t.Wp;
     return t;
 }
-template <bool RAGGED>
+__device__ __forceinline__ Tile tile_of_ragged_tall(const TileGeo& g, int tile) {
+    Tile t;
+    const int* __restrict__ tab = g.tab;
+    int lo = 0, hi = g.B - 1;
+    while (lo < hi) {
+        const int mid = (lo + hi + 1) >> 1;
+        if (tab[EXCEL_RAG_REC * mid + 5] <= tile) lo = mid; else hi = mid - 1;
+    }
+    t.b = lo;
+    const int* rec = tab + EXCEL_RAG_REC * t.b;
+    t.H = rec[0]; t.W = rec[1];
+    t.Wp = (t.W + 3) & ~3;
+    t.base = rec[2];
+    t.lab = rec[4];
+    const int loc = tile - rec[5];
+    const int ntx = (t.W + 63) >> 6;
+    const int ty = loc / ntx;
+    t.x0 = (loc - ty * ntx) * 64;
+    t.y0 = ty * 32;
+    t.HW = (long long)t.H * t.Wp;
+    return t;
+}
+template <bool RAGGED, int TH = 16>
 __device__ __forceinline__ Tile tile_of(const TileGeo& g) {
     Tile t;
     if (RAGGED) {
-        t = tile_of_ragged(g, blockIdx.x);
+        t = (TH == 16) ? tile_of_ragged(g, blockIdx.x) : tile_of_ragged_tall(g, blockIdx.x);
     } else {
-        t.b = blockIdx.z; t.x0 = blockIdx.x * 64; t.y0 = blockIdx.y * 16;
+        t.b = blockIdx.z; t.x0 = blockIdx.x * 64; t.y0 = blockIdx.y * TH;
         t.H = g.H; t.W = g.W; t.Wp = g.W;
         t.HW = (long long)g.H * g.W;
         t.base = (long long)t.b * t.HW;
diff --git a/excel_amd/csrc/excel_internal.h b/excel_amd/csrc/excel_internal.h
--- a/excel_amd/csrc/excel_internal.h
+++ b/excel_amd/csrc/excel_internal.h
@@ -92,7 +92,8 @@
 int excel_par_guide_supported(const void* guide, const void* stats, const void* in, const void* out, int Cmax, long long max_plane, int Wp,
                               const int* dil, int ndil);
 int excel_launch_par_iterate_guide(const float* guide, const float* stats, const float* in, float* out, const int* nchan, int Cmax,
-                                   const TileGeo& geo, int total_tiles, const int* dil, int ndil, float w1, float w2, hipStream_t st);
+                                   const TileGeo& geo, int total_tiles, int tile_rows, const int* dil, int ndil, float w1, float w2, hipStream_t st);
+int excel_par_pick_tile_rows(int uniform_H, long long tall_tiles, int force);
 int excel_launch_par_iterate(const float* aff, const float* in, float* out, const int* nchan, int B, int Cmax, int H, int W,
                              const int* dil, int ndil, hipStream_t st);
 int excel_launch_bilinear_ac_ragged(const float* in, float* out, int h, int w, const TileGeo& geo, int total_tiles, hipStream_t st);
diff --git a/excel_amd/csrc/par.hip b/excel_amd/csrc/par.hip
--- a/excel_amd/csrc/par.hip
+++ b/excel_amd/csrc/par.hip
@@ -145,22 +145,37 @@
     return v;
 }
 
-template <bool RAGGED>
-__global__ __launch_bounds__(512, 4) void par_iterate_guide_kernel(const float* __restrict__ guide, const float* __restrict__ stats,
-                                                                    const float* __restrict__ in, float* __restrict__ out,
-                                                                    const int* __restrict__ nchan, ParDil dl, int Cmax, TileGeo geo, int dbg) {
-    constexpr int ND = 6, HALO = 24, TR = 16 + 2 * HALO, TP = PG_TP, NG = 3 * ND;
-    __shared__ __attribute__((aligned(1024))) float tile[2 * TR * TP];
+#define PAR_TALL_LDS_BYTES (3 * (32 + 48) * PG_TP * 4)
+extern __shared__ __attribute__((aligned(1024))) float par_tall_tile[];
+__device__ __forceinline__ void par_wait_vm(int k) {
+#define PAR_W(N) asm volatile("s_waitcnt vmcnt(" #N ")" ::: "memory")
+    if (k >= 10) { if (k >= 12) PAR_W(12); else if (k == 11) PAR_W(11); else PAR_W(10); }
+    else if (k >= 3) { if (k >= 5) PAR_W(5); else if (k == 4) PAR_W(4); else PAR_W(3); }
+    else if (k == 2) PAR_W(2);
+    else if (k == 1) PAR_W(1);
+    else PAR_W(0);
+#undef PAR_W
+}
+
+template <bool RAGGED, int TH>
+__global__ __launch_bounds__(TH * 32, 4) void par_iterate_guide_kernel(const float* __restrict__ guide, const float* __restrict__ stats,
+                                                                        const float* __restrict__ in, float* __restrict__ out,
+                                                                        const int* __restrict__ nchan, ParDil dl, int Cmax, TileGeo geo, int dbg) {
+    static_assert(TH == 16 || TH == 32, "tile height");
+    constexpr int ND = 6, HALO = 24, TR = TH + 2 * HALO, TP = PG_TP, NG = 3 * ND, NW = TH / 2, NSLOT = TH == 16 ? 2 : 3;
+    __shared__ __attribute__((aligned(1024))) float tile_s[TH == 16 ? 2 * TR * TP : 1];
+    float* const tile = TH == 16 ? tile_s : par_tall_tile;
     Tile tg;
     if (RAGGED) {
-        tg = tile_of_ragged(geo, (EXCEL_DBG(dbg) & 32) ? (int)blockIdx.x : xcd_remap(blockIdx.x, gridDim.x));
+        const int tn = (EXCEL_DBG(dbg) & 32) ? (int)blockIdx.x : xcd_remap(blockIdx.x, gridDim.x);
+        tg = TH == 16 ? tile_of_ragged(geo, tn) : tile_of_ragged_tall(geo, tn);
     } else {
-        tg = tile_of<false>(geo);
+        tg = tile_of<false, TH>(geo);
         if (!(EXCEL_DBG(dbg) & 32)) {
             const int nx = gridDim.x, ny = gridDim.y, per = nx * ny;
             const int id = xcd_remap(blockIdx.x + nx * (blockIdx.y + ny * blockIdx.z), per * (int)gridDim.z);
             const int bb = id / per, rem = id - bb * per, tyy = rem / nx;
-            tg.b = bb; tg.x0 = (rem - tyy * nx) * 64; tg.y0 = tyy * 16; tg.base = (long long)bb * tg.HW; tg.lab = tg.base;
+            tg.b = bb; tg.x0 = (rem - tyy * nx) * 64; tg.y0 = tyy * TH; tg.base = (long long)bb * tg.HW; tg.lab = tg.base;
         }
     }
     const int b = tg.b, x0 = tg.x0, y0 = tg.y0, H = tg.H, W = tg.W, Wp = tg.Wp;
@@ -177,7 +192,8 @@
     const __amdgpu_buffer_rsrc_t rs_m = __builtin_amdgcn_make_buffer_rsrc((void*)(in + (long long)Cmax * tg.base), 0, (int)((long long)Cmax * HW * 4), 0x00020000);
     const int xoffA = min(max(x0 - HALO + lane, 0), W - 1) * 4, xoffB = min(max(x0 - HALO + 64 + lane, 0), W - 1) * 4;
     const unsigned tile_b = lds_addr(tile);
-    constexpr int RPW = TR / 8;
+    constexpr int RPW = TR / NW;
+    static_assert(RPW * NW == TR, "rows per wave");
 #ifdef PAR_ALL_INTERIOR
     const bool interior = true;
 #else
@@ -189,16 +205,31 @@
         const int plane_off = (is_g ? p : p - 3) * (int)(HW * 4);
         unsigned dst = tile_b + (buf * TR + wave * RPW) * (TP * 4);
         asm volatile("" : "+s"(dst));
-        if ((EXCEL_DBG(dbg) & 8) && (wave == 0 || wave == 7)) return;
+        int xA = xoffA, xB = xoffB, x4 = x4off;
+        if constexpr (TH == 32) {
+            int ln = lane;
+            asm volatile("" : "+v"(ln));
+            xA = min(max(x0 - HALO + ln, 0), W - 1) * 4; xB = min(max(x0 - HALO + 64 + ln, 0), W - 1) * 4;
+            x4 = min(x0 - HALO + 4 * (ln & 31), Wp - 4) * 4;
+        }
+        if ((EXCEL_DBG(dbg) & 8) && (wave == 0 || wave == NW - 1)) return;
         if (interior) {
             int half = lane >> 5;
             asm volatile("" : "+v"(half));
 #pragma unroll
             for (int j = 0; j < RPW / 2; ++j) {
                 const int gy = min(max(y0 - HALO + wave * RPW + 2 * j + half, 0), H - 1);
-                const int voff = gy * Wp * 4 + x4off;
+                const int voff = gy * Wp * 4 + x4;
                 if (is_g) __builtin_amdgcn_raw_ptr_buffer_load_lds(rs_g, (lds_bptr)(unsigned long long)(dst + j * (2 * TP * 4)), 16, voff, plane_off, 0, 0);
                 else __builtin_amdgcn_raw_ptr_buffer_load_lds(rs_m, (lds_bptr)(unsigned long long)(dst + j * (2 * TP * 4)), 16, voff, plane_off, 0, 0);
+            }
+            if constexpr (RPW & 1) {
+                if (half == 0) {
+                    const int gy = min(max(y0 - HALO + wave * RPW + RPW - 1, 0), H - 1);
+                    const int voff = gy * Wp * 4 + x4;
+                    if (is_g) __builtin_amdgcn_raw_ptr_buffer_load_lds(rs_g, (lds_bptr)(unsigned long long)(dst + (RPW - 1) * (TP * 4)), 16, voff, plane_off, 0, 0);
+                    else __builtin_amdgcn_raw_ptr_buffer_load_lds(rs_m, (lds_bptr)(unsigned long long)(dst + (RPW - 1) * (TP * 4)), 16, voff, plane_off, 0, 0);
+                }
             }
             return;
         }
@@ -207,11 +238,11 @@
             const int gy = min(max(y0 - HALO + wave * RPW + rr, 0), H - 1);
             const int soff = plane_off + gy * Wp * 4;
             if (is_g) {
-                __builtin_amdgcn_raw_ptr_buffer_load_lds(rs_g, (lds_bptr)(unsigned long long)(dst + rr * (TP * 4)), 4, xoffA, soff, 0, 0);
-                __builtin_amdgcn_raw_ptr_buffer_load_lds(rs_g, (lds_bptr)(unsigned long long)(dst + rr * (TP * 4) + 256), 4, xoffB, soff, 0, 0);
+                __builtin_amdgcn_raw_ptr_buffer_load_lds(rs_g, (lds_bptr)(unsigned long long)(dst + rr * (TP * 4)), 4, xA, soff, 0, 0);
+                __builtin_amdgcn_raw_ptr_buffer_load_lds(rs_g, (lds_bptr)(unsigned long long)(dst + rr * (TP * 4) + 256), 4, xB, soff, 0, 0);
             } else {
-                __builtin_amdgcn_raw_ptr_buffer_load_lds(rs_m, (lds_bptr)(unsigned long long)(dst + rr * (TP * 4)), 4, xoffA, soff, 0, 0);
-                __builtin_amdgcn_raw_ptr_buffer_load_lds(rs_m, (lds_bptr)(unsigned long long)(dst + rr * (TP * 4) + 256), 4, xoffB, soff, 0, 0);
+                __builtin_amdgcn_raw_ptr_buffer_load_lds(rs_m, (lds_bptr)(unsigned long long)(dst + rr * (TP * 4)), 4, xA, soff, 0, 0);
+                __builtin_amdgcn_raw_ptr_buffer_load_lds(rs_m, (lds_bptr)(unsigned long long)(dst + rr * (TP * 4) + 256), 4, xB, soff, 0, 0);
             }
         }
     };
@@ -280,6 +311,7 @@
     f32x2 st_nxt = stat_load(0), st_nx2 = f32x2{0.f, 0.f};
     __builtin_amdgcn_sched_barrier(0);
     stage(0, 0);
+    const int NPC = __builtin_amdgcn_readfirstlane(interior ? RPW / 2 + (RPW & 1) : 2 * RPW);
 #pragma unroll 1
     for (int p = 0; p < 3; ++p) {
         asm volatile("s_waitcnt vmcnt(0)" : "+v"(st_nxt) :: "memory");
@@ -288,15 +320,19 @@
         st_nxt = stat_load(p + 1);
         if (p == 2) st_nx2 = stat_load(4);
         f32x2 ctr;
-        asm volatile("ds_read_b64 %0, %1 offset:%2" : "=v"(ctr) : "v"(org + (p & 1) * (TR * TP * 4)), "n"((HALO * TP + HALO) * 4) : "memory");
+        asm volatile("ds_read_b64 %0, %1 offset:%2" : "=v"(ctr) : "v"(org + (NSLOT == 2 ? (p & 1) : p) * (TR * TP * 4)), "n"((HALO * TP + HALO) * 4) : "memory");
         __builtin_amdgcn_sched_barrier(0);
-        stage(p + 1, (p + 1) & 1);
+        if constexpr (NSLOT == 2) stage(p + 1, (p + 1) & 1);
+        else {
+            if (p == 0) stage(1, 1);
+            if (p + 2 < np) stage(p + 2, p == 0 ? 2 : p - 1);
+        }
         asm volatile("s_waitcnt lgkmcnt(0)" : "+v"(ctr) :: "memory");
         if (EXCEL_DBG(dbg) & 1) continue;
         f32x2 nctr = -ctr;
         if (EXCEL_DBG(dbg) & 16) nctr += 1e-30f * far_taps(guide + 3 * tg.base + (long long)p * HW);
         asm volatile("" : "+v"(nctr));
-        taps(std::integral_constant<int, 1>{}, p & 1, [&](int di, int k, const f32x2 nb) {
+        taps(std::integral_constant<int, 1>{}, NSLOT == 2 ? (p & 1) : p, [&](int di, int k, const f32x2 nb) {
             const f32x2 dv = nb + nctr;
             wall[di][k] = __builtin_elementwise_fma(dv * dv, nk2, wall[di][k]);
         }, [] {});
@@ -321,17 +357,26 @@
 #define PAR_STORE_WAIT 1
 #endif
     const bool wstore = PAR_STORE_WAIT && __builtin_amdgcn_ballot_w64(valid) != 0 && !EXCEL_DBG(dbg);
+    int slot = NSLOT == 2 ? 1 : 0;
+    const int nst = __builtin_amdgcn_readfirstlane(wstore ? 1 : 0);
     for (int p = 3; p < np; ++p) {
-        if (p > 3 && wstore) asm volatile("s_waitcnt vmcnt(1)" ::: "memory");
-        else asm volatile("s_waitcnt vmcnt(0)" ::: "memory");
-        __builtin_amdgcn_s_barrier();
-        if (p + 1 < np) stage(p + 1, (p + 1) & 1);
+        if constexpr (NSLOT == 2) {
+            if (p > 3 && wstore) asm volatile("s_waitcnt vmcnt(1)" ::: "memory");
+            else asm volatile("s_waitcnt vmcnt(0)" ::: "memory");
+            __builtin_amdgcn_s_barrier();
+            if (p + 1 < np) stage(p + 1, (p + 1) & 1);
+        } else {
+            par_wait_vm((p + 1 < np ? NPC : 0) + nst * min(p - 3, 2));
+            __builtin_amdgcn_s_barrier();
+            if (p + 2 < np) stage(p + 2, slot == 0 ? 2 : slot - 1);
+        }
         if (EXCEL_DBG(dbg) & 4) continue;
         f32x2 acc = {0.f, 0.f};
         if (EXCEL_DBG(dbg) & 16) acc = 1e-30f * far_taps(in + (long long)Cmax * tg.base + (long long)(p - 3) * HW);
-        taps(std::integral_constant<int, PAR_MASK_DEPTH>{}, p & 1, [&](int di, int k, const f32x2 nb) { acc = __builtin_elementwise_fma(nb, wall[di][k], acc); },
+        taps(std::integral_constant<int, PAR_MASK_DEPTH>{}, NSLOT == 2 ? (p & 1) : slot, [&](int di, int k, const f32x2 nb) { acc = __builtin_elementwise_fma(nb, wall[di][k], acc); },
              [&] { asm volatile("" : "+v"(acc)); });
         if (valid) *reinterpret_cast<f32x2*>(out_px + (long long)(p - 3) * HW) = acc;
+        if constexpr (NSLOT == 3) slot = slot == 2 ? 0 : slot + 1;
     }
 }
 
@@ -679,9 +724,31 @@
     return (vec && par_dil_ok(dil, ndil) && planes * max_plane * 4 < (1LL << 31)) ? 1 : 0;
 }
 
+#define PAR_TALL_MIN_PER_CU 4
+int excel_par_pick_tile_rows(int uniform_H, long long tall_tiles, int force) {
+    if (force == 16 || force == 32) return force;
+    if (uniform_H > 0 && uniform_H < 32) return 16;
+    return tall_tiles >= 256LL * PAR_TALL_MIN_PER_CU ? 32 : 16;
+}
+
+static int par_tall_init() {
+    static bool done[64];
+    int dev = 0;
+    if (hipGetDevice(&dev) != hipSuccess || dev < 0 || dev >= 64) return EXCEL_ERR_LAUNCH;
+    if (done[dev]) return EXCEL_OK;
+    if (hipFuncSetAttribute((const void*)par_iterate_guide_kernel<true, 32>, hipFuncAttributeMaxDynamicSharedMemorySize, PAR_TALL_LDS_BYTES) != hipSuccess ||
+        hipFuncSetAttribute((const void*)par_iterate_guide_kernel<false, 32>, hipFuncAttributeMaxDynamicSharedMemorySize, PAR_TALL_LDS_BYTES) != hipSuccess) {
+        (void)hipGetLastError();
+        return EXCEL_ERR_LAUNCH;
+    }
+    done[dev] = true;
+    return EXCEL_OK;
+}
+
 int excel_launch_par_iterate_guide(const float* guide, const float* stats, const float* in, float* out, const int* nchan, int Cmax,
-                                   const TileGeo& geo, int total_tiles, const int* dil, int ndil, float w1, float w2, hipStream_t st) {
+                                   const TileGeo& geo, int total_tiles, int tile_rows, const int* dil, int ndil, float w1, float w2, hipStream_t st) {
     EXCEL_CHECK_ARG(par_dil_ok(dil, ndil), "par_iterate_guide: unsupported dilation set");
+    EXCEL_CHECK_ARG(tile_rows == 16 || tile_rows == 32, "par_iterate_guide: tile rows must be 16 or 32");
     ProfScope prof__(PROF_PAR_ITERATE, st);
     ParDil dl;
     int rc = make_dil(dil, ndil, w1, w2, &dl);
@@ -691,11 +758,21 @@
     static const int env_dbg = getenv("EXCEL_PAR_DBG") ? atoi(getenv("EXCEL_PAR_DBG")) : 0;
     dbg = env_dbg;
 #endif
-    if (geo.tab)
-        hipLaunchKernelGGL((par_iterate_guide_kernel<true>), dim3(total_tiles), dim3(512), 0, st, guide, stats, in, out, nchan, dl, Cmax, geo, dbg);
-    else
-        hipLaunchKernelGGL((par_iterate_guide_kernel<false>), dim3(cdiv(geo.W, 64), cdiv(geo.H, 16), geo.B), dim3(512), 0, st, guide, stats,
+    if (tile_rows == 32) {
+        rc = par_tall_init();
+        if (rc) return rc;
+        if (geo.tab)
+            hipLaunchKernelGGL((par_iterate_guide_kernel<true, 32>), dim3(total_tiles), dim3(1024), PAR_TALL_LDS_BYTES, st, guide, stats, in, out, nchan,
+                               dl, Cmax, geo, dbg);
+        else
+            hipLaunchKernelGGL((par_iterate_guide_kernel<false, 32>), dim3(cdiv(geo.W, 64), cdiv(geo.H, 32), geo.B), dim3(1024), PAR_TALL_LDS_BYTES, st,
+                               guide, stats, in, out, nchan, dl, Cmax, geo, dbg);
+    } else if (geo.tab) {
+        hipLaunchKernelGGL((par_iterate_guide_kernel<true, 16>), dim3(total_tiles), dim3(512), 0, st, guide, stats, in, out, nchan, dl, Cmax, geo, dbg);
+    } else {
+        hipLaunchKernelGGL((par_iterate_guide_kernel<false, 16>), dim3(cdiv(geo.W, 64), cdiv(geo.H, 16), geo.B), dim3(512), 0, st, guide, stats,
                            in, out, nchan, dl, Cmax, geo, dbg);
+    }
     EXCEL_CHECK_LAUNCH("par_iterate_guide");
     return EXCEL_OK;
 }
diff --git a/excel_amd/ops.py b/excel_amd/ops.py
--- a/excel_amd/ops.py
+++ b/excel_amd/ops.py
@@ -724,7 +724,21 @@
     return cams
 
 
-def par_forward(imgs, masks, dilations=PAR_DILATIONS, num_iter=20, nchan=None, w1=0.3, w2=0.01, stream_affinities=False, out=None, ws=None):
+def _par_flags(stream_affinities, tile_rows):
+    assert tile_rows in (None, 16, 32)
+    return (1 if stream_affinities else 0) | {None: 0, 16: 2, 32: 4}[tile_rows]
+
+
+def par_tile_rows(H, W, B, tile_rows=None):
+    return lib().excel_par_tile_rows(H, B * (-(-W // 64)) * (-(-H // 32)), _par_flags(False, tile_rows))
+
+
+def par_tile_rows_ragged(plan, tile_rows=None):
+    return lib().excel_par_tile_rows(0, int(plan.info.total_tall_tiles), _par_flags(False, tile_rows))
+
+
+def par_forward(imgs, masks, dilations=PAR_DILATIONS, num_iter=20, nchan=None, w1=0.3, w2=0.01, stream_affinities=False, out=None, ws=None,
+                tile_rows=None):
     imgs = f32c(imgs)
     masks = f32c(masks)
     B, Cmax, H, W = masks.shape
@@ -736,7 +750,7 @@
     if ws is None or ws.numel() < need:
         ws = _ws(need, masks.device)
     check(lib().excel_par_forward(_p(imgs), h, w, _p(masks), _p(nchan, torch.int32), B, Cmax, H, W, dil, len(dilations), num_iter,
-                                  w1, w2, _p(out), _p(ws, torch.uint8), 1 if stream_affinities else 0, _stream()), "excel_par_forward")
+                                  w1, w2, _p(out), _p(ws, torch.uint8), _par_flags(stream_affinities, tile_rows), _stream()), "excel_par_forward")
     return out
 
 
@@ -1103,7 +1117,8 @@
     return cams
 
 
-def par_forward_ragged(imgs, masks, plan, Cmax, dilations=PAR_DILATIONS, num_iter=20, nchan=None, w1=0.3, w2=0.01, out=None, ws=None):
+def par_forward_ragged(imgs, masks, plan, Cmax, dilations=PAR_DILATIONS, num_iter=20, nchan=None, w1=0.3, w2=0.01, out=None, ws=None,
+                       tile_rows=None):
     imgs = f32c(imgs)
     assert imgs.shape[0] == plan.B and imgs.shape[1] == 3 and masks.numel() == Cmax * plan.total_pix
     h, w = imgs.shape[-2:]
@@ -1113,7 +1128,8 @@
     if ws is None or ws.numel() < need:
         ws = _ws(need, masks.device)
     check(lib().excel_par_forward_ragged(_p(imgs), h, w, _p(masks), _p(nchan, torch.int32), _p(plan.table, torch.int32), C.byref(plan.info), Cmax,
-                                         dil, len(dilations), num_iter, w1, w2, _p(out), _p(ws, torch.uint8), _stream()), "excel_par_forward_ragged")
+                                         dil, len(dilations), num_iter, w1, w2, _p(out), _p(ws, torch.uint8), _par_flags(False, tile_rows), _stream()),
+          "excel_par_forward_ragged")
     return out
 
 
diff --git a/include/excel_hip.h b/include/excel_hip.h
--- a/include/excel_hip.h
+++ b/include/excel_hip.h
@@ -184,6 +184,9 @@
 
 
 #define EXCEL_PAR_STREAM_AFFINITIES 1
+#define EXCEL_PAR_TILE_ROWS_16 2
+#define EXCEL_PAR_TILE_ROWS_32 4
+int excel_par_tile_rows(int uniform_H, long long tall_tiles, int flags);
 size_t excel_par_workspace_bytes(int B, int Cmax, int H, int W, int ndil);
 int excel_par_forward(const float* imgs, int h, int w, const float* masks, const int32_t* nchan, int B, int Cmax, int H, int W,
                       const int32_t* dilations , int ndil, int n_iter, float w1, float w2, float* out,
@@ -200,6 +203,7 @@
     int64_t total_label_pix;
     int64_t max_plane_pix;
     int64_t table_ints;
+    int64_t total_tall_tiles;
 } excel_ragged_info;
 int excel_ragged_plan(const int32_t* hw , int B, excel_ragged_info* info , int32_t* table );
 
@@ -215,7 +219,7 @@
 size_t excel_par_ragged_workspace_bytes(long long total_pix, int Cmax);
 int excel_par_forward_ragged(const float* imgs, int h, int w, const float* masks, const int32_t* nchan, const int32_t* table,
                              const excel_ragged_info* info, int Cmax, const int32_t* dilations , int ndil, int n_iter, float w1,
-                             float w2, float* out, void* workspace, void* stream);
+                             float w2, float* out, void* workspace, int flags , void* stream);
 
 int excel_argmax_label_ragged(const float* cams, const int32_t* nchan, const int32_t* cls_idx, const int32_t* table,
                               const excel_ragged_info* info, int Smax, int Cmax, uint8_t* labels_u8, void* stream);
```

After: 1461. 0.979x the previous value.
